# saifahmadgit/go2-sim2real-locomotion-rl

Hardware: AMD Instinct MI355X
Metric: env-steps/sec (all envs) Go2 walk 4096 envs; 1/2/4/8-GPU scaling (higher is better)
Workload: dtype f32

## Files before the change

### go2_sim2real_locomotion_rl_amd/csrc/go2sim.hip

```cpp

#include <hip/hip_runtime.h>

#include <algorithm>
#include <cstddef>
#include <cstdint>
#include <cstdio>
#include <cstdlib>
#include <cstring>
#include <new>
#include <vector>

#include "../../include/go2sim.h"
#include "../../include/go2sim_detmath.h"

#define DEV __device__ __forceinline__
#define DEVN __device__ __noinline__

namespace {

constexpr int NL = GO2SIM_NL, ND = GO2SIM_ND, NQ = GO2SIM_NQ, NG = GO2SIM_NG, NJ = GO2SIM_NJ;
constexpr int NPAIR = GO2SIM_NPAIR_MAX, MAXC = GO2SIM_MAX_CONTACTS, MAXB = GO2SIM_MAX_BROAD, MAXR = GO2SIM_MAX_ROWS;
constexpr int JOINT_FIXED = 0, JOINT_REVOLUTE = 1, JOINT_FREE = 4;
constexpr int GEOM_PLANE = 0, GEOM_SPHERE = 1, GEOM_CYLINDER = 3, GEOM_BOX = 5, GEOM_TERRAIN = 7;
constexpr int TERRAIN_CB = 4;
// ... 303 lines not shown
      depth[i] = (par < 0) ? 0 : depth[par] + 1;
      if (depth[i] > max_depth) max_depth = depth[i];
    }
    m.n_levels = max_depth + 1;
    int k = 0;
    for (int lev = 0; lev <= max_depth; ++lev) {
      m.level_start[lev] = k;
      for (int i = 0; i < NL; ++i) if (depth[i] == lev) m.level_links[k++] = i;
    }
    for (int lev = max_depth + 1; lev <= NL; ++lev) m.level_start[lev] = k;
    k = 0;
    for (int par = 0; par < NL; ++par) {
      m.child_start[par] = k;
      for (int i = NL - 1; i > par; --i) if (m.links[i].parent == par) m.child_list[k++] = i;
    }
    m.child_start[NL] = k;
    for (int d = 0; d < ND; ++d) m.dof_link[d] = -1;
    for (int i = 0; i < NL; ++i) for (int d = m.links[i].dof_start; d < m.links[i].dof_end; ++d) m.dof_link[d] = i;
    for (int d = 0; d < ND; ++d) if (m.dof_link[d] < 0) return false;
  }
  int g_next = 0;
  for (int i = 0; i < NL; ++i) { if (m.links[i].geom_start != g_next) return false; g_next = m.links[i].geom_end; }
  return g_next == NG;
}


struct LinkS {
  int parent, entity, is_fixed, joint_start, joint_end, dof_start, dof_end, q_start, q_end, n_dofs;
  V3 pos; Q4 quat; V3 inertial_pos; Q4 inertial_quat; M3 inertial_i; float mass; float invweight[2];
};
struct GeomS { int type, link; V3 pos; Q4 quat; };
struct JLim { int q_start, dof_start; float lo, hi; };
constexpr int NTRI = ND * (ND + 1) / 2;
constexpr int LEG_K = 4, LEG_D = 3;
struct alignas(16) ModelS {
  int n_levels, iterations, ls_iterations, arrow_mode;
  float substep_dt; V3 gravity; float eps, tolerance, ls_tolerance, meaninertia;
  LinkS links[NL];
  unsigned char tri_i[NTRI + 1], tri_j[NTRI + 1];
  JLim jlim[NJ];
  Joint joints[NJ]; Dof dofs[ND]; GeomS geoms[NG]; Entity entities[2];
  float qpos0[NQ]; unsigned mass_mask_bits[ND];
  int level_start[NL + 1], level_links[NL], child_start[NL + 1], child_list[NL], dof_link[ND];
  unsigned char leg_links[LEG_K * LEG_D], leg_root, leg_form;
};
constexpr int SOLVER_BLOCK_BYTES = (int)(sizeof(LinkS) * NL + 2 * (NTRI + 1) + sizeof(JLim) * NJ);
static_assert(sizeof(ModelS) % 16 == 0 && (2 * (NTRI + 1)) % 4 == 0 && offsetof(ModelS, links) % 16 == 0 && offsetof(ModelS, jlim) == offsetof(ModelS, links) + sizeof(LinkS) * NL + 2 * (NTRI + 1), "ModelS is copied in 16-byte granules");

static bool build_leg_form(const Model& m, ModelS& o) {
  if (getenv("GO2SIM_NO_LEG_FORM") && atoi(getenv("GO2SIM_NO_LEG_FORM")) != 0) return false;
  if (NL > 255) return false;
  auto n_children = [&](int i) { return m.child_start[i + 1] - m.child_start[i]; };
  auto one_revolute = [&](const Link& L) {
    if (L.joint_end - L.joint_start != 1) return false;
    const Joint& J = m.joints[L.joint_start];
    return J.type == JOINT_REVOLUTE && J.dof_end - J.dof_start == 1 && L.dof_start == J.dof_start && L.dof_end == J.dof_end &&
           L.q_end - L.q_start == 1 && J.q_start == L.q_start;
  };
  int root = -1, n_links = 0;
  for (int i = 0; i < NL; ++i) {
    const Link& L = m.links[i];
    if (L.parent != -1) continue;
    const bool free_root = !L.is_fixed && L.joint_end - L.joint_start == 1 && m.joints[L.joint_start].type == JOINT_FREE && L.n_dofs == 6;
    if (free_root) {
      if (root >= 0) return false;
      root = i;
    } else if (!(L.is_fixed && L.joint_end == L.joint_start && L.n_dofs == 0 && n_children(i) == 0)) {
      return false;
    } else {
      n_links++;
    }
  }
  if (root < 0 || n_children(root) != LEG_K) return false;
  n_links++;
  for (int l = 0; l < LEG_K; ++l) {
    int i = m.child_list[m.child_start[root] + l];
    for (int d = 0; d < LEG_D; ++d) {
      if (!one_revolute(m.links[i]) || n_children(i) != (d + 1 < LEG_D ? 1 : 0)) return false;
      o.leg_links[LEG_D * l + d] = (unsigned char)i;
      n_links++;
      if (d + 1 < LEG_D) i = m.child_list[m.child_start[i]];
    }
  }
  if (n_links != NL) return false;
  o.leg_root = (unsigned char)root;
  return true;
}
bool build_model_s(const Model& m, ModelS& o) {
  memset(&o, 0, sizeof(o));
  o.n_levels = m.n_levels; o.iterations = m.iterations; o.ls_iterations = m.ls_iterations; o.arrow_mode = m.arrow_mode;
  o.substep_dt = m.substep_dt; o.gravity = m.gravity; o.eps = m.eps; o.tolerance = m.tolerance; o.ls_tolerance = m.ls_tolerance; o.meaninertia = m.meaninertia;
  for (int i = 0; i < NL; ++i) {
    const Link& a = m.links[i]; LinkS& b = o.links[i];
    b.parent = a.parent; b.entity = a.entity; b.is_fixed = a.is_fixed; b.joint_start = a.joint_start; b.joint_end = a.joint_end; b.dof_start = a.dof_start;
    b.dof_end = a.dof_end; b.q_start = a.q_start; b.q_end = a.q_end; b.n_dofs = a.n_dofs; b.pos = a.pos; b.quat = a.quat; b.inertial_pos = a.inertial_pos;
    b.inertial_quat = a.inertial_quat; b.inertial_i = a.inertial_i; b.mass = a.mass; b.invweight[0] = a.invweight[0]; b.invweight[1] = a.invweight[1];
  }
  for (int i = 0; i < NJ; ++i) o.joints[i] = m.joints[i];
  for (int i = 0; i < ND; ++i) o.dofs[i] = m.dofs[i];
  for (int i = 0; i < NG; ++i) { o.geoms[i].type = m.geoms[i].type; o.geoms[i].link = m.geoms[i].link; o.geoms[i].pos = m.geoms[i].pos; o.geoms[i].quat = m.geoms[i].quat; }
  for (int i = 0; i < 2; ++i) o.entities[i] = m.entities[i];
  for (int i = 0; i < NQ; ++i) o.qpos0[i] = m.qpos0[i];
  for (int i = 0; i < ND; ++i) {
    unsigned bits = 0;
    for (int j = 0; j < ND; ++j) {
      float v = m.mass_parent_mask[i][j];
      if (v == 1.0f) bits |= 1u << j; else if (v != 0.0f) return false;
    }
    o.mass_mask_bits[i] = bits;
  }
  for (int i = 0; i <= NL; ++i) { o.level_start[i] = m.level_start[i]; o.child_start[i] = m.child_start[i]; }
  for (int i = 0; i < NL; ++i) { o.level_links[i] = m.level_links[i]; o.child_list[i] = m.child_list[i]; }
  for (int i = 0; i < ND; ++i) o.dof_link[i] = m.dof_link[i];
  int k = 0;
  for (int i = 0; i < ND; ++i) for (int j = 0; j <= i; ++j) { o.tri_i[k] = (unsigned char)i; o.tri_j[k] = (unsigned char)j; k++; }
  for (int i = 0; i < NJ; ++i) {
    const Joint& J = m.joints[i];
    bool rev = J.type == JOINT_REVOLUTE;
    o.jlim[i].q_start = rev ? J.q_start : -1; o.jlim[i].dof_start = J.dof_start;
    o.jlim[i].lo = rev ? m.dofs[J.dof_start].limit[0] : 0.0f; o.jlim[i].hi = rev ? m.dofs[J.dof_start].limit[1] : 0.0f;
  }
  o.leg_form = build_leg_form(m, o) ? 1 : 0;
  return true;
}
DEV float mass_mask(const ModelS& m, int i, int j) { return (float)((m.mass_mask_bits[i] >> j) & 1u); }
DEV void tri_index(const ModelS& m, int idx, int& i, int& j) { i = m.tri_i[idx]; j = m.tri_j[idx]; }

struct ModelView {
  int n_levels, iterations, ls_iterations, arrow_mode, leg_form; float substep_dt; V3 gravity; float eps, tolerance, ls_tolerance, meaninertia;
  const LinkS* links; const Joint* joints; const Dof* dofs; const GeomS* geoms; const Entity* entities; const float* qpos0;
  const unsigned* mass_mask_bits; const int *level_start, *level_links, *child_start, *child_list, *dof_link; const unsigned char *tri_i, *tri_j;
  const unsigned char* leg_links; int leg_root;
  DEV ModelView(const ModelS* t, const ModelS* __restrict__ g)
      : n_levels(g->n_levels), iterations(g->iterations), ls_iterations(g->ls_iterations), arrow_mode(g->arrow_mode), leg_form(g->leg_form), substep_dt(g->substep_dt), gravity(g->gravity), eps(g->eps),
        tolerance(g->tolerance), ls_tolerance(g->ls_tolerance), meaninertia(g->meaninertia), links(t->links), joints(t->joints), dofs(t->dofs),
        geoms(t->geoms), entities(t->entities), qpos0(t->qpos0), mass_mask_bits(t->mass_mask_bits), level_start(t->level_start),
        level_links(t->level_links), child_start(t->child_start), child_list(t->child_list), dof_link(t->dof_link), tri_i(t->tri_i), tri_j(t->tri_j),
        leg_links(t->leg_links), leg_root(g->leg_root) {}
  DEV ModelView(const LinkS* lds_links, const unsigned char* lds_tri_i, const unsigned char* lds_tri_j, const Model* __restrict__ g)
      : n_levels(g->n_levels), iterations(g->iterations), ls_iterations(g->ls_iterations), arrow_mode(g->arrow_mode), leg_form(0), substep_dt(g->substep_dt), gravity(g->gravity), eps(g->eps),
        tolerance(g->tolerance), ls_tolerance(g->ls_tolerance), meaninertia(g->meaninertia), links(lds_links), joints(g->joints), dofs(g->dofs),
        geoms(nullptr), entities(g->entities), qpos0(g->qpos0), mass_mask_bits(nullptr), level_start(nullptr), level_links(nullptr), child_start(nullptr),
        child_list(nullptr), dof_link(nullptr), tri_i(lds_tri_i), tri_j(lds_tri_j), leg_links(nullptr), leg_root(-1) {}
};
DEV float mass_mask(const ModelView& m, int i, int j) { return (float)((m.mass_mask_bits[i] >> j) & 1u); }
DEV void tri_index(const ModelView& m, int idx, int& i, int& j) { i = m.tri_i[idx]; j = m.tri_j[idx]; }
constexpr int lds_dma_bytes(int nbytes) { return (nbytes + 1023) / 1024 * 1024; }
template <int NBYTES>
DEV void wg_dma_to_lds(void* lds_dst, const void* __restrict__ src, int lane = (int)threadIdx.x) {
#pragma unroll
  for (int k = 0; k < lds_dma_bytes(NBYTES) / 1024; ++k)
    __builtin_amdgcn_global_load_lds((const __attribute__((address_space(1))) void*)((const char*)src + (k * 64 + lane) * 16),
                                     (__attribute__((address_space(3))) void*)((char*)lds_dst + k * 1024), 16, 0, 0);
}
constexpr int MODELS_LDS_BYTES = lds_dma_bytes((int)sizeof(ModelS));
constexpr int GEOMK_BYTES = NG * (int)sizeof(GeomK), GEOMK_LDS_BYTES = lds_dma_bytes(GEOMK_BYTES);

#define GO2SIM_FLOAT_FIELDS(X)                                                                                       \
  X(qpos, NQ) X(vel, ND) X(ctrl_force, ND) X(ext, NL * 6) X(mass_shift, NL) X(com_shift, NL * 3)                        \
  X(friction_ratio, NG) X(l_pos, NL * 3) X(l_quat, NL * 4) X(cd_vel, NL * 3) X(cd_ang, NL * 3) X(root_com, NL * 3)     \
  X(contact_force, NL * 3) X(geom_friction, NG) X(ctrl_pos, ND) X(ctrl_vel, ND) X(dof_pos, ND) \
                                                                                       \
  X(actions, NA) X(last_actions, NA) X(applied_actions, NA) X(action_history, GO2SIM_ACTION_RING_MAX * NA) X(target_dof_pos, NM)            \
  X(e_dof_pos, NM) X(e_dof_vel, NM) X(last_dof_vel, NM) X(torque, NM) X(base_pos, 3) X(base_quat, 4) X(base_lin_vel, 3) \
  X(base_ang_vel, 3) X(projected_gravity, 3) X(base_euler, 3) X(commands, 3) X(time_out, 1) X(kp_factors, NM)          \
  X(kd_factors, NM) X(motor_strength, NM) X(gravity_offset, 3) X(current_push_force, 3) X(push_stored_force, 3)       \
  X(feet_air_time, 4) X(base_vel_world, 3) X(last_base_pos_x, 1) X(episode_sums, NREW) X(rew_terms, NREW) X(rew, 1) X(obs, NOBS_MAX) X(priv, NPRIV_MAX) \
  X(base_kp, 1) X(base_kd, 1)

#define GO2SIM_INT_FIELDS(X)                                                                                         \
  X(n_contacts, 1) X(n_con, 1) X(err, 1) X(is_warmstart, 1) X(first_time, 1) X(n_broad, 1) X(solver_iters, 1) X(ctrl_mode, ND) \
  X(gjk_fallback, 1) X(delay_steps, 1) X(episode_length, 1) X(reset_buf, 1) X(push_remaining, 1) X(foot_contact, 4)    \
  X(last_foot_contact, 4) X(terrain_row, 1) X(terrain_key, 1)

#define GO2SIM_AOS_FLOAT_FIELDS(X)                                                                                   \
  X(acc, ND) X(qacc_ws, ND) X(force, ND) X(qf_smooth, ND) X(acc_smooth, ND) X(qfrc_constraint, ND) X(mass_mat, NTRI)  \
  X(cdof_ang, ND * 3) X(cdof_vel, ND * 3) X(cdofd_ang, ND * 3) X(cdofd_vel, ND * 3) X(cinr_inertial, NL * 9)            \
  X(cinr_pos, NL * 3) X(cinr_mass, NL) X(i_pos, NL * 3) X(i_quat, NL * 4) X(g_pos, NG * 3) X(g_quat, NG * 4)              \
  X(sort_value, 2 * NG) X(c_pos, MAXC * 3) X(c_normal, MAXC * 3) X(c_pen, MAXC) X(c_friction, MAXC) X(c_sol, MAXC * 7)    \
  X(c_force, MAXC * 3) X(efc_force, MAXR) X(normal_cache, NPAIR * 3)

constexpr int NCV = (NPAIR + 31) / 32;
#define GO2SIM_AOS_INT_FIELDS(X) X(sort_ig, 2 * NG) X(broad, MAXB * 2) X(c_geom, 2 * MAXC) X(c_link, 2 * MAXC) X(ncache_valid, NCV)

enum FOff : int {
#define X(n, c) FO_##n##_, FO_##n##_end = FO_##n##_ + (c) - 1,
  GO2SIM_FLOAT_FIELDS(X)
#undef X
  FO_TOTAL
};
enum IOff : int {
#define X(n, c) IO_##n##_, IO_##n##_end = IO_##n##_ + (c) - 1,
  GO2SIM_INT_FIELDS(X)
#undef X
  IO_TOTAL
};
enum AOff : int {
#define X(n, c) AO_##n##_, AO_##n##_end = AO_##n##_ + (c) - 1,
  GO2SIM_AOS_FLOAT_FIELDS(X)
#undef X
  AO_TOTAL
};
enum AIOff : int {
#define X(n, c) AIO_##n##_, AIO_##n##_end = AIO_##n##_ + (c) - 1,
  GO2SIM_AOS_INT_FIELDS(X)
#undef X
  AIO_TOTAL
};
#define FO(n) FO_##n##_
#define IO(n) IO_##n##_
#define AO(n) AO_##n##_
#define AIO(n) AIO_##n##_
constexpr int ASTRIDE = (AO_TOTAL + 15) / 16 * 16;
constexpr int AISTRIDE = (AIO_TOTAL + 15) / 16 * 16;

template <typename T>
struct Arr {
  T* p; int B;
  DEV T& operator[](int i) const { return p[(size_t)i * B]; }
};
struct V3Ref {
  float* p; int B;
  DEV operator V3() const { return v3(p[0], p[B], p[2 * (size_t)B]); }
  DEV const V3Ref& operator=(V3 v) const { p[0] = v.x; p[B] = v.y; p[2 * (size_t)B] = v.z; return *this; }
  DEV const V3Ref& operator=(const V3Ref& o) const { V3 v = o; return *this = v; }
};
struct Q4Ref {
  float* p; int B;
  DEV operator Q4() const { return q4(p[0], p[B], p[2 * (size_t)B], p[3 * (size_t)B]); }
  DEV const Q4Ref& operator=(Q4 q) const { p[0] = q.w; p[B] = q.x; p[2 * (size_t)B] = q.y; p[3 * (size_t)B] = q.z; return *this; }
  DEV const Q4Ref& operator=(const Q4Ref& o) const { Q4 v = o; return *this = v; }
};
struct M3Ref {
  float* p; int B;
  DEV operator M3() const { M3 r;
#pragma unroll
    for (int i = 0; i < 9; ++i) r.m[i / 3][i % 3] = p[(size_t)i * B];
    return r; }
  DEV const M3Ref& operator=(const M3& r) const {
#pragma unroll
    for (int i = 0; i < 9; ++i) p[(size_t)i * B] = r.m[i / 3][i % 3];
    return *this; }
  DEV const M3Ref& operator=(const M3Ref& o) const { M3 v = o; return *this = v; }
};
struct Arr3 { float* p; int B; DEV V3Ref operator[](int i) const { return V3Ref{p + (size_t)(3 * i) * B, B}; } };
struct Arr4 { float* p; int B; DEV Q4Ref operator[](int i) const { return Q4Ref{p + (size_t)(4 * i) * B, B}; } };
struct Arr9 { float* p; int B; DEV M3Ref operator[](int i) const { return M3Ref{p + (size_t)(9 * i) * B, B}; } };
template <int W>
struct Arr2 {
  float* p; int B;
  DEV Arr<float> operator[](int i) const { return Arr<float>{p + (size_t)(W * i) * B, B}; }
};

struct Pool { float* f; int* i; int B; float* fa; int* ia; };

struct E {
  float* f; int* i; int B; int b; float* fa; int* ia;
  DEV E(const Pool& P, int b_) : f(P.f + b_), i(P.i + b_), B(P.B), b(b_), fa(P.fa + (size_t)b_ * ASTRIDE), ia(P.ia + (size_t)b_ * AISTRIDE) {}
#define FA(name) DEV Arr<float> name() const { return Arr<float>{f + (size_t)FO(name) * B, B}; }
#define FA3(name) DEV Arr3 name() const { return Arr3{f + (size_t)FO(name) * B, B}; }
#define FA4(name) DEV Arr4 name() const { return Arr4{f + (size_t)FO(name) * B, B}; }
#define FA2(name, W) DEV Arr2<W> name() const { return Arr2<W>{f + (size_t)FO(name) * B, B}; }
#define IA(name) DEV Arr<int> name() const { return Arr<int>{i + (size_t)IO(name) * B, B}; }
#define AA(name) DEV Arr<float> name() const { return Arr<float>{fa + AO(name), 1}; }
#define AA3(name) DEV Arr3 name() const { return Arr3{fa + AO(name), 1}; }
#define AA4(name) DEV Arr4 name() const { return Arr4{fa + AO(name), 1}; }
#define AA9(name) DEV Arr9 name() const { return Arr9{fa + AO(name), 1}; }
#define AA2(name, W) DEV Arr2<W> name() const { return Arr2<W>{fa + AO(name), 1}; }
#define AIA(name) DEV Arr<int> name() const { return Arr<int>{ia + AIO(name), 1}; }
  FA(qpos) FA(vel) FA(ctrl_force) FA(ctrl_pos) FA(ctrl_vel) FA(ext) FA(mass_shift) FA3(com_shift) FA(friction_ratio)
  FA(geom_friction) FA3(l_pos) FA4(l_quat) FA3(root_com) FA(dof_pos) FA3(cd_vel) FA3(cd_ang) FA3(contact_force)
  FA(actions) FA(last_actions) FA(applied_actions) FA2(action_history, NA) FA(target_dof_pos) FA(e_dof_pos) FA(e_dof_vel) FA(last_dof_vel)
  FA(torque) FA(base_pos) FA(base_quat) FA(base_lin_vel) FA(base_ang_vel) FA(projected_gravity) FA(base_euler) FA(commands) FA(time_out)
  FA(kp_factors) FA(kd_factors) FA(motor_strength) FA(gravity_offset) FA(current_push_force) FA(push_stored_force) FA(feet_air_time) FA(base_vel_world) FA(last_base_pos_x)
  FA(episode_sums) FA(rew_terms) FA(rew) FA(obs) FA(priv) FA(base_kp) FA(base_kd)
  IA(n_contacts) IA(n_con) IA(err) IA(is_warmstart) IA(first_time) IA(n_broad) IA(solver_iters) IA(ctrl_mode)
  IA(gjk_fallback) IA(delay_steps) IA(episode_length) IA(reset_buf) IA(push_remaining) IA(foot_contact) IA(last_foot_contact) IA(terrain_row) IA(terrain_key)
  AA(acc) AA(qacc_ws) AA(force) AA(qf_smooth) AA(acc_smooth) AA(qfrc_constraint) AA3(cdof_ang) AA3(cdof_vel) AA3(cdofd_ang)
  AA3(cdofd_vel) AA9(cinr_inertial) AA3(cinr_pos) AA(cinr_mass) AA3(i_pos) AA4(i_quat) AA3(g_pos) AA4(g_quat) AA(sort_value) AA3(c_pos) AA3(c_normal)
  AA(c_pen) AA(c_friction) AA2(c_sol, 7) AA3(c_force) AA(efc_force) AA3(normal_cache)
  AIA(sort_ig) AIA(broad) AIA(c_geom) AIA(c_link) AIA(ncache_valid)
#undef FA
#undef FA3
#undef FA4
#undef FA2
#undef IA
#undef AA
#undef AA3
#undef AA4
#undef AA9
#undef AA2
#undef AIA
};
DEV void team_sync() {
  __builtin_amdgcn_fence(__ATOMIC_RELEASE, "workgroup");
  __builtin_amdgcn_wave_barrier();
  __builtin_amdgcn_fence(__ATOMIC_ACQUIRE, "workgroup");
}
DEV void team_sync_lds() {
  __builtin_amdgcn_fence(__ATOMIC_RELEASE, "workgroup", "local");
  __builtin_amdgcn_wave_barrier();
  __builtin_amdgcn_fence(__ATOMIC_ACQUIRE, "workgroup", "local");
}
DEV float gload(const E& e, int off, int k) { return e.f[(size_t)(off + k) * e.B]; }
DEV void gstore(const E& e, int off, int k, float v) { e.f[(size_t)(off + k) * e.B] = v; }
DEV float aload(const E& e, int off, int k) { return e.fa[off + k]; }
DEV void astore(const E& e, int off, int k, float v) { e.fa[off + k] = v; }


template <int N, int T, class F>
DEV void team_for(int tl, F f) {
#pragma unroll
  for (int k0 = 0; k0 < N; k0 += T) { int k = k0 + tl; if (k < N) f(k); }
}
template <int N, int STRIDE, int R, class FL, class FS>
DEV void team_stage_r(int k0, FL& ld, FS& st) {
  if constexpr (R * STRIDE < N) {
    int k = R * STRIDE + k0;
    k = k < N ? k : N - 1;
    const float v = ld(k);
    team_stage_r<N, STRIDE, R + 1>(k0, ld, st);
    st(k, v);
  }
}
template <int N, int T, class FL, class FS>
DEV void team_stage(int tl, FL ld, FS st) { team_stage_r<N, T, 0>(tl, ld, st); }
template <int EPW, int COUNT, class F>
DEV void wg_load(const Pool& P, int b0, int off, F put) {
  const int ev = threadIdx.x % EPW, k0 = threadIdx.x / EPW;
  const int b = (b0 + ev < P.B) ? b0 + ev : P.B - 1;
  auto ld = [&](int k) { return P.f[(size_t)(off + k) * P.B + b]; };
  auto st = [&](int k, float v) { put(ev, k, v); };
  team_stage_r<COUNT, 64 / EPW, 0>(k0, ld, st);
}

#ifdef GO2SIM_PHASE_PROFILE
constexpr int PH_MAX_WG = 8192;
__device__ unsigned long long g_phase_cycles[PH_MAX_WG * 64];
#define PH_BEGIN unsigned long long ph_t = __builtin_readcyclecounter();
#define PH(i) { __builtin_amdgcn_s_waitcnt(0); unsigned long long ph_n = __builtin_readcyclecounter(); if (threadIdx.x == 0 && blockIdx.x < PH_MAX_WG / 2) g_phase_cycles[blockIdx.x * 64 + (i)] += ph_n - ph_t; ph_t = __builtin_readcyclecounter(); }
#define PHD_BEGIN unsigned long long phd_t = __builtin_readcyclecounter();
#define PHD(i) { unsigned long long phd_n = __builtin_readcyclecounter(); const unsigned long long phd_a = __ballot(1); if ((int)threadIdx.x == __ffsll((long long)phd_a) - 1 && blockIdx.x < PH_MAX_WG / 2) { atomicAdd(&g_phase_cycles[blockIdx.x * 64 + (i)], phd_n - phd_t); atomicAdd(&g_phase_cycles[blockIdx.x * 64 + (i) + 1], 1ull); } phd_t = __builtin_readcyclecounter(); }
#define PHC(i, n) { if (threadIdx.x == 0 && blockIdx.x < PH_MAX_WG / 2) g_phase_cycles[blockIdx.x * 64 + (i)] += (unsigned long long)(n); }
#define PHB(i) { __builtin_amdgcn_s_waitcnt(0); unsigned long long ph_n = __builtin_readcyclecounter(); if (threadIdx.x == 0 && blockIdx.x < PH_MAX_WG / 2) g_phase_cycles[(PH_MAX_WG / 2 + blockIdx.x) * 64 + (i)] += ph_n - ph_t; ph_t = __builtin_readcyclecounter(); }
#else
#define PH_BEGIN
#define PH(i)
#define PHD_BEGIN
#define PHD(i)
#define PHC(i, n)
#define PHB(i)
#endif

#ifdef GO2SIM_STAMP
constexpr int ST_KINDS = 8, ST_MAX_WG = 4096, ST_DEPTH = 4;
__device__ unsigned long long g_stamp[ST_KINDS * ST_MAX_WG * ST_DEPTH * 2];
__device__ unsigned g_stamp_cnt[ST_KINDS * ST_MAX_WG];
struct StampScope {
  int kind; unsigned long long t0;
  DEV StampScope(int k) : kind(k) { t0 = __builtin_amdgcn_s_memrealtime(); }
  DEV ~StampScope() {
    __builtin_amdgcn_s_waitcnt(0);
    const unsigned long long t1 = __builtin_amdgcn_s_memrealtime();
    if (threadIdx.x == 0 && blockIdx.x < ST_MAX_WG) {
      const int w = kind * ST_MAX_WG + (int)blockIdx.x;
      const unsigned c = g_stamp_cnt[w];
      g_stamp[(w * ST_DEPTH + (int)(c % ST_DEPTH)) * 2] = t0; g_stamp[(w * ST_DEPTH + (int)(c % ST_DEPTH)) * 2 + 1] = t1;
      g_stamp_cnt[w] = c + 1;
    }
  }
};
#define STAMP(kind) StampScope stamp_scope_(kind);
#else
#define STAMP(kind)
#endif
enum { STK_PRE_DYN = 0, STK_COLLIDE, STK_SOLVE, STK_INT_FK_DYN, STK_INT_FK, STK_POST_A, STK_POST_B, STK_OTHER };

enum { SV_COST = 0, SV_PREV_COST, SV_GAUSS, SV_QG0, SV_QG1, SV_QG2, SV_GTOL };
enum { SI_LS_IT = 0, SI_LS_RESULT, SI_IMPROVED };

DEV V3 ld3(const float* p, int i) { return v3(p[3 * i], p[3 * i + 1], p[3 * i + 2]); }
DEV void st3(float* p, int i, V3 v) { p[3 * i] = v.x; p[3 * i + 1] = v.y; p[3 * i + 2] = v.z; }
DEV Q4 ld4(const float* p, int i) { return q4(p[4 * i], p[4 * i + 1], p[4 * i + 2], p[4 * i + 3]); }
DEV void st4(float* p, int i, Q4 q) { p[4 * i] = q.w; p[4 * i + 1] = q.x; p[4 * i + 2] = q.y; p[4 * i + 3] = q.z; }
DEV M3 ld9(const float* p, int i) { M3 r;
#pragma unroll
  for (int k = 0; k < 9; ++k) r.m[k / 3][k % 3] = p[9 * i + k];
  return r; }
DEV void st9(float* p, int i, const M3& r) {
#pragma unroll
  for (int k = 0; k < 9; ++k) p[9 * i + k] = r.m[k / 3][k % 3]; }

DEV int xcd_block() {
  const int n = (int)gridDim.x, q = n >> 3, r = n & 7, x = (int)blockIdx.x & 7, i = (int)blockIdx.x >> 3;
  return (x < r ? x * (q + 1) : r * (q + 1) + (x - r) * q) + i;
}

constexpr int LPT_CLS = 32;
DEV int lpt_solver_xcd(int b, int B, int epw_s) {
  const int n = (B + epw_s - 1) / epw_s, q = n >> 3, r = n & 7, L = b / epw_s;
  if (L < r * (q + 1)) return L / (q + 1);
  return r + (L - r * (q + 1)) / (q > 0 ? q : 1);
}
DEV void lpt_file(int* __restrict__ rec, int cap, int L, int B, int epw_s, int nc) {
  const int x = lpt_solver_xcd(L * epw_s, B, epw_s), cls = LPT_CLS - 1 - imn(LPT_CLS - 1, nc);
  const int pos = atomicAdd(&rec[x * LPT_CLS + cls], 1);
  if (pos < cap) rec[8 * LPT_CLS + (x * LPT_CLS + cls) * cap + pos] = L;
}
DEV int lpt_take(const int* __restrict__ rec, int cap, int B, int epw, int slot) {
  const int ident = xcd_block() * epw + slot;
  if (rec == nullptr) return ident;
  const int n = (int)gridDim.x, q = n >> 3, r = n & 7, x = (int)blockIdx.x & 7;
  const int expected = q + (x < r ? 1 : 0);
  const int local = (int)blockIdx.x >> 3;
  int total = 0, cls = -1, off = 0;
#pragma unroll
  for (int c = 0; c < LPT_CLS; ++c) {
    const int k = rec[x * LPT_CLS + c];
    if (cls < 0 && local < total + k) { cls = c; off = local - total; }
    total += k;
  }
  if (total != expected) return ident;
  if (cls < 0 || off >= cap) return B;
  return rec[8 * LPT_CLS + (x * LPT_CLS + cls) * cap + off] * epw + slot;
}

struct KinData {
  float qpos[NQ], vel[ND], qpos_next[NQ], vel_next[ND];
  float l_pos[NL * 3], l_quat[NL * 4], i_pos[NL * 3], i_quat[NL * 4];
  float xanchor[NJ * 3], xaxis[NJ * 3];
  float cdof_ang[ND * 3], cdof_vel[ND * 3];
  float cd_vel[NL * 3], cd_ang[NL * 3];
  float mass[NL];
  int valid;
};

#ifndef GO2SIM_FAST_ORDER
#define GO2SIM_FAST_ORDER 1
#endif
template <int CTRL>
DEV float dpp_perm(float x) { return __int_as_float(__builtin_amdgcn_update_dpp(0, __float_as_int(x), CTRL, 0xf, 0xf, true)); }
#if GO2SIM_FAST_ORDER
constexpr bool ARROW_SHAPE = (ND == 18);
DEV float leg_sum4(float x) {
  const auto r = __builtin_amdgcn_permlane16_swap(__float_as_uint(x), __float_as_uint(x), false, false);
  const float p = __uint_as_float(r[0]) + __uint_as_float(r[1]);
  return p + dpp_perm<0x128>(p);
}
DEV float4 lds4(const float* p) { return *(const float4*)p; }
template <int T, int STRIDE>
DEV void arrow_factor(const int mode, const float eps, const float* A, float* F, int tl) {
  static_assert(T == 32 || T == 64, "four groups of eight lanes");
  const int leg = (tl >> 3) & 3, u = tl & 7, ub = u < 6 ? u : 5;
  const int p0 = dm_arrow_dof(mode, leg, 0), p1 = dm_arrow_dof(mode, leg, 1), p2 = dm_arrow_dof(mode, leg, 2);
  const bool w_lane = tl < 32 && u < 6;
  const float a00 = A[p0 * STRIDE + p0], a10 = A[p1 * STRIDE + p0], a11 = A[p1 * STRIDE + p1];
  const float a20 = A[p2 * STRIDE + p0], a21 = A[p2 * STRIDE + p1], a22 = A[p2 * STRIDE + p2];
  const float c0 = A[p0 * STRIDE + ub], c1 = A[p1 * STRIDE + ub], c2 = A[p2 * STRIDE + ub];
  float br[6];
#pragma unroll
  for (int j = 0; j < 6; ++j) br[j] = A[ub * STRIDE + j];
  team_sync();
  const float e0 = fmx(a00, eps), i0 = dm_sqrt(e0) * (1.0f / e0);
  const float l10 = a10 * i0, l20 = a20 * i0;
  const float e1 = fmx(__builtin_fmaf(-l10, l10, a11), eps), i1 = dm_sqrt(e1) * (1.0f / e1);
  const float l21 = __builtin_fmaf(-l20, l10, a21) * i1;
  const float e2 = fmx(__builtin_fmaf(-l21, l21, __builtin_fmaf(-l20, l20, a22)), eps), i2 = dm_sqrt(e2) * (1.0f / e2);
  const float w0 = c0 * i0, w1 = __builtin_fmaf(-w0, l10, c1) * i1, w2 = __builtin_fmaf(-w1, l21, __builtin_fmaf(-w0, l20, c2)) * i2;
  if (w_lane) *(float4*)&F[32 * leg + 8 + 4 * u] = make_float4(w0, w1, w2, 0.0f);
  if (tl < 32 && u == 0) { *(float4*)&F[32 * leg] = make_float4(i0, i1, i2, 0.0f); *(float4*)&F[32 * leg + 4] = make_float4(l10, l20, l21, 0.0f); }
  team_sync();
  float sc[6];
#pragma unroll
  for (int j = 0; j < 6; ++j) {
    const float4 wj = lds4(&F[32 * leg + 8 + 4 * j]);
    sc[j] = __builtin_fmaf(w2, wj.z, __builtin_fmaf(w1, wj.y, w0 * wj.x));
  }
#pragma unroll
  for (int j = 0; j < 6; ++j) sc[j] = leg_sum4(sc[j]);
  const float bp[6] = {br[0] - sc[0], br[1] - sc[1], br[2] - sc[2], br[3] - sc[3], br[4] - sc[4], br[5] - sc[5]};
  if (tl < 6) { *(float4*)&F[128 + 8 * tl] = make_float4(bp[0], bp[1], bp[2], bp[3]); *(float4*)&F[128 + 8 * tl + 4] = make_float4(bp[4], bp[5], 0.0f, 0.0f); }
  team_sync();
  float a[6][6];
#pragma unroll
  for (int k = 0; k < 6; ++k) {
    const float4 lo = lds4(&F[128 + 8 * k]); const float2 hi = *(const float2*)&F[128 + 8 * k + 4];
    a[k][0] = lo.x; a[k][1] = lo.y; a[k][2] = lo.z; a[k][3] = lo.w; a[k][4] = hi.x; a[k][5] = hi.y;
  }
  team_sync();
#pragma unroll
  for (int k = 0; k < 6; ++k) {
    const float e = fmx(a[k][k], eps), ik = dm_sqrt(e) * (1.0f / e);
    a[k][k] = ik;
#pragma unroll
    for (int j = k + 1; j < 6; ++j) a[j][k] = a[j][k] * ik;
#pragma unroll
    for (int j = k + 1; j < 6; ++j)
#pragma unroll
      for (int i = k + 1; i <= j; ++i) a[j][i] = __builtin_fmaf(-a[j][k], a[i][k], a[j][i]);
  }
  if (tl == 0) {
#pragma unroll
    for (int k = 0; k < 6; ++k) {
      *(float4*)&F[128 + 8 * k] = make_float4(a[k][0], k >= 1 ? a[k][1] : 0.0f, k >= 2 ? a[k][2] : 0.0f, k >= 3 ? a[k][3] : 0.0f);
      *(float2*)&F[128 + 8 * k + 4] = make_float2(k >= 4 ? a[k][4] : 0.0f, k >= 5 ? a[k][5] : 0.0f);
    }
  }
  team_sync();
}
template <int T>
DEV void arrow_solve(const float* F, float gl0, float gl1, float gl2, float gb, float* x6, int tl, float (&xb)[6], float& xl0, float& xl1, float& xl2) {
  static_assert(T == 32 || T == 64, "four groups of eight lanes");
  const int leg = (tl >> 3) & 3, u = tl & 7, ub = u < 6 ? u : 5;
  const float4 iv = lds4(&F[32 * leg]), lv = lds4(&F[32 * leg + 4]), wo = lds4(&F[32 * leg + 8 + 4 * ub]);
  float4 W[6];
#pragma unroll
  for (int b = 0; b < 6; ++b) W[b] = lds4(&F[32 * leg + 8 + 4 * b]);
  float L[6][6];
#pragma unroll
  for (int k = 0; k < 6; ++k) {
    const float4 lo = lds4(&F[128 + 8 * k]); const float2 hi = *(const float2*)&F[128 + 8 * k + 4];
    L[k][0] = lo.x; L[k][1] = lo.y; L[k][2] = lo.z; L[k][3] = lo.w; L[k][4] = hi.x; L[k][5] = hi.y;
  }
  const float y0 = gl0 * iv.x, y1 = __builtin_fmaf(-lv.x, y0, gl1) * iv.y, y2 = __builtin_fmaf(-lv.z, y1, __builtin_fmaf(-lv.y, y0, gl2)) * iv.z;
  const float z = leg_sum4(__builtin_fmaf(wo.z, y2, __builtin_fmaf(wo.y, y1, wo.x * y0)));
  if (tl < 6) x6[tl] = gb - z;
  team_sync();
  const float2 r0 = *(const float2*)&x6[0], r1 = *(const float2*)&x6[2], r2 = *(const float2*)&x6[4];
  float x[6] = {r0.x, r0.y, r1.x, r1.y, r2.x, r2.y};
  team_sync();
#pragma unroll
  for (int k = 0; k < 6; ++k) {
    float acc = x[k];
#pragma unroll
    for (int j = 0; j < k; ++j) acc = __builtin_fmaf(-L[k][j], x[j], acc);
    x[k] = acc * L[k][k];
  }
#pragma unroll
  for (int k_ = 0; k_ < 6; ++k_) {
    const int k = 5 - k_;
    float acc = x[k];
#pragma unroll
    for (int j_ = 0; j_ < 5 - k; ++j_) { const int j = 5 - j_; acc = __builtin_fmaf(-L[j][k], x[j], acc); }
    x[k] = acc * L[k][k];
  }
  float v0 = y0, v1 = y1, v2 = y2;
#pragma unroll
  for (int b = 0; b < 6; ++b) { v0 = __builtin_fmaf(-W[b].x, x[b], v0); v1 = __builtin_fmaf(-W[b].y, x[b], v1); v2 = __builtin_fmaf(-W[b].z, x[b], v2); }
  xl2 = v2 * iv.z; xl1 = __builtin_fmaf(-lv.z, xl2, v1) * iv.y; xl0 = __builtin_fmaf(-lv.x, xl1, __builtin_fmaf(-lv.y, xl2, v0)) * iv.x;
#pragma unroll
  for (int k = 0; k < 6; ++k) xb[k] = x[k];
}
#endif
struct DynData {
  float cinr_I[NL * 9], cinr_pos[NL * 3], cinr_mass[NL];
  float crb_I[NL * 9], crb_pos[NL * 3], crb_mass[NL];
  float cdof_ang[ND * 3], cdof_vel[ND * 3], cdofd_ang[ND * 3], cdofd_vel[ND * 3];
  float cd_vel[NL * 3], cd_ang[NL * 3], cdd_vel[NL * 3], cdd_ang[NL * 3], cfrc_vel[NL * 3], cfrc_ang[NL * 3];
  float f_ang[ND * 3], f_vel[ND * 3];
  float vel[ND], qf_applied[ND], qf_passive[ND], force[ND], out[ND], Dinv[ND];
  float M[ND * ND], L[ND * ND];
  int ctrl_mode[ND];
};
#if GO2SIM_FAST_ORDER
static_assert(!ARROW_SHAPE || (offsetof(DynData, Dinv) % 8 == 0 && sizeof(DynData) % 8 == 0), "arrow_solve reads DynData::Dinv with 8-byte LDS loads");
#endif

template <int T>
DEV void tk_stage_links(const E& e, KinData* s, int tl) {
  team_for<NL, T>(tl, [&](int i_l) { st3(s->l_pos, i_l, e.l_pos()[i_l]); st4(s->l_quat, i_l, e.l_quat()[i_l]); });
}
template <int T, class MT>
DEV void tk_kinematics(const MT& m, const E& e, KinData* s, int tl, bool force_update_fixed, DynData* dk = nullptr) {
  PH_BEGIN
  const bool legs = (T == 32 || T == 64) && m.leg_form;
  if (legs) {
    const int r = m.leg_root;
    const int rq = m.joints[m.links[r].joint_start].q_start;
    const V3 rpos = v3(s->qpos[rq], s->qpos[rq + 1], s->qpos[rq + 2]);
    Q4 rquat = q4(s->qpos[rq + 3], s->qpos[rq + 4], s->qpos[rq + 5], s->qpos[rq + 6]);
    const float rn = dm_sqrt(norm_sqr(rquat));
    rquat = q4(rquat.w / rn, rquat.x / rn, rquat.y / rn, rquat.z / rn);
    if (tl == 0) {
      const auto& L = m.links[r];
      const int i_j = L.joint_start, ds = m.joints[i_j].dof_start;
      st3(s->xanchor, i_j, rpos);
      st3(s->xaxis, i_j, v3(0, 0, 1));
      gstore(e, FO(dof_pos), ds + 0, rpos.x); gstore(e, FO(dof_pos), ds + 1, rpos.y); gstore(e, FO(dof_pos), ds + 2, rpos.z);
      if (dk) { dk->out[ds] = rpos.x; dk->out[ds + 1] = rpos.y; dk->out[ds + 2] = rpos.z; }
      st3(s->l_pos, r, rpos); st4(s->l_quat, r, rquat); e.l_pos()[r] = rpos; e.l_quat()[r] = rquat;
    }
    Q4 ql = q4(0, 0, 0, 0);
    if (tl < LEG_K * LEG_D) {
      const Joint& J = m.joints[m.links[m.leg_links[tl]].joint_start];
      const float dp = s->qpos[J.q_start] - m.qpos0[J.q_start];
      gstore(e, FO(dof_pos), J.dof_start, dp);
      if (dk) dk->out[J.dof_start] = dp;
      ql = rotvec_to_quat(m.dofs[J.dof_start].motion_ang * dp, m.eps);
    }
    Q4 qloc[LEG_D];
#pragma unroll
    for (int d = 0; d < LEG_D; ++d) {
      const int src = tl < LEG_K ? LEG_D * tl + d : 0;
      qloc[d] = q4(__shfl(ql.w, src, T), __shfl(ql.x, src, T), __shfl(ql.y, src, T), __shfl(ql.z, src, T));
    }
    if (tl < LEG_K) {
      int lk[LEG_D], jk[LEG_D];
      V3 lpos[LEG_D], jpos[LEG_D], axis[LEG_D]; Q4 lquat[LEG_D];
#pragma unroll
      for (int d = 0; d < LEG_D; ++d) {
        lk[d] = m.leg_links[LEG_D * tl + d];
        const auto& L = m.links[lk[d]];
        jk[d] = L.joint_start;
        const Joint& J = m.joints[jk[d]];
        lpos[d] = L.pos; lquat[d] = L.quat; jpos[d] = J.pos; axis[d] = m.dofs[J.dof_start].motion_ang;
      }
      V3 pos = rpos; Q4 quat = rquat;
#pragma unroll
      for (int d = 0; d < LEG_D; ++d) {
        const Q4 pq = quat;
        pos = pos + transform_by_quat(lpos[d], pq);
        quat = transform_quat_by_quat(lquat[d], pq);
        const V3 anchor = transform_by_quat(jpos[d], quat) + pos;
        st3(s->xanchor, jk[d], anchor);
        st3(s->xaxis, jk[d], transform_by_quat(axis[d], quat));
        quat = transform_quat_by_quat(qloc[d], quat);
        pos = anchor - transform_by_quat(jpos[d], quat);
        st3(s->l_pos, lk[d], pos); st4(s->l_quat, lk[d], quat); e.l_pos()[lk[d]] = pos; e.l_quat()[lk[d]] = quat;
      }
    }
    team_sync();
  }
  for (int lev = 0; lev < (legs ? 0 : m.n_levels); ++lev) {
    for (int k = m.level_start[lev] + tl; k < m.level_start[lev + 1]; k += T) {
      int i_l = m.level_links[k];
      const auto& L = m.links[i_l];
      V3 pos = L.pos; Q4 quat = L.quat;
      if (L.parent != -1) {
        Q4 pq = ld4(s->l_quat, L.parent);
        pos = ld3(s->l_pos, L.parent) + transform_by_quat(L.pos, pq);
        quat = transform_quat_by_quat(L.quat, pq);
      }
      for (int i_j = L.joint_start; i_j < L.joint_end; ++i_j) {
        const Joint& J = m.joints[i_j];
        int q_start = J.q_start, dof_start = J.dof_start;
        if (J.type == JOINT_FREE) {
          V3 pos_ = v3(s->qpos[q_start], s->qpos[q_start + 1], s->qpos[q_start + 2]);
          st3(s->xanchor, i_j, pos_);
          st3(s->xaxis, i_j, v3(0, 0, 1));
          Q4 quat_ = q4(s->qpos[q_start + 3], s->qpos[q_start + 4], s->qpos[q_start + 5], s->qpos[q_start + 6]);
          float n = dm_sqrt(norm_sqr(quat_));
          quat_ = q4(quat_.w / n, quat_.x / n, quat_.y / n, quat_.z / n);
          pos = pos_; quat = quat_;
          gstore(e, FO(dof_pos), dof_start + 0, pos.x); gstore(e, FO(dof_pos), dof_start + 1, pos.y); gstore(e, FO(dof_pos), dof_start + 2, pos.z);
          if (dk) { dk->out[dof_start] = pos.x; dk->out[dof_start + 1] = pos.y; dk->out[dof_start + 2] = pos.z; }
        } else if (J.type == JOINT_REVOLUTE) {
          V3 axis = m.dofs[dof_start].motion_ang;
          V3 anchor = transform_by_quat(J.pos, quat) + pos;
          st3(s->xanchor, i_j, anchor);
          st3(s->xaxis, i_j, transform_by_quat(axis, quat));
          float dp = s->qpos[q_start] - m.qpos0[q_start];
          gstore(e, FO(dof_pos), dof_start, dp);
          if (dk) dk->out[dof_start] = dp;
          Q4 qloc = rotvec_to_quat(axis * dp, m.eps);
          quat = transform_quat_by_quat(qloc, quat);
          pos = anchor - transform_by_quat(J.pos, quat);
        }
      }
      if (!(L.parent == -1 && L.is_fixed)) { st3(s->l_pos, i_l, pos); st4(s->l_quat, i_l, quat); e.l_pos()[i_l] = pos; e.l_quat()[i_l] = quat; }
    }
    team_sync();
  }
  PH(18)
  for (int i_l = tl; i_l < NL; i_l += T) {
    const auto& L = m.links[i_l];
    s->mass[i_l] = L.mass + gload(e, FO(mass_shift), i_l);
    V3 ipbw; Q4 iq;
    transform_pos_quat_by_trans_quat(L.inertial_pos + (V3)e.com_shift()[i_l], L.inertial_quat, ld3(s->l_pos, i_l), ld4(s->l_quat, i_l), ipbw, iq);
    st3(s->i_pos, i_l, ipbw); st4(s->i_quat, i_l, iq);
  }
  team_sync();
  V3 rc[2];
#pragma unroll
  for (int i_e = 0; i_e < 2; ++i_e) {
    const Entity& en = m.entities[i_e];
    V3 root_com_bw = v3(0, 0, 0); float mass_sum = 0.0f;
    for (int i_l = en.link_start; i_l < en.link_end; ++i_l) {
      float mass = s->mass[i_l];
      mass_sum = mass_sum + mass;
      root_com_bw = root_com_bw + mass * ld3(s->i_pos, i_l);
    }
    rc[i_e] = root_com_bw / mass_sum;
  }
  team_sync();
  for (int i_l = tl; i_l < NL; i_l += T) {
    const auto& L = m.links[i_l];
    V3 r = (L.entity == 0) ? rc[0] : rc[1];
    e.root_com()[i_l] = r;
    V3 ip = ld3(s->i_pos, i_l) - r;
    Q4 iq = ld4(s->i_quat, i_l);
    if (!dk) e.i_pos()[i_l] = ip;
    e.i_quat()[i_l] = iq;
    float i_mass = s->mass[i_l];
    M3 oI; V3 op;
    transform_inertia_by_trans_quat(L.inertial_i, i_mass, ip, iq, m.eps, oI, op);
    if (!dk) { e.cinr_inertial()[i_l] = oI; e.cinr_pos()[i_l] = op; e.cinr_mass()[i_l] = i_mass; }
    if (dk) { st9(dk->cinr_I, i_l, oI); st9(dk->crb_I, i_l, oI); st3(dk->cinr_pos, i_l, op); st3(dk->crb_pos, i_l, op); dk->cinr_mass[i_l] = i_mass; dk->crb_mass[i_l] = i_mass; }
  }
  for (int i_j = tl; i_j < NJ; i_j += T) {
    const Joint& J = m.joints[i_j];
    const auto& L = m.links[J.link];
    if (L.n_dofs == 0) continue;
    V3 r = (L.entity == 0) ? rc[0] : rc[1];
    V3 offset_pos = r - ld3(s->xanchor, i_j);
    int ds = J.dof_start;
    if (J.type == JOINT_REVOLUTE) {
      V3 ax = ld3(s->xaxis, i_j);
      V3 cv = cross(ax, offset_pos);
      st3(s->cdof_ang, ds, ax); st3(s->cdof_vel, ds, cv);
      e.cdof_ang()[ds] = ax; e.cdof_vel()[ds] = cv;
      if (dk) { st3(dk->cdof_ang, ds, ax); st3(dk->cdof_vel, ds, cv); }
    } else if (J.type == JOINT_FREE) {
      for (int i = 0; i < 3; ++i) {
        V3 cv = v3(0, 0, 0);
        vset(cv, i, 1.0f);
        st3(s->cdof_ang, i + ds, v3(0, 0, 0)); st3(s->cdof_vel, i + ds, cv);
        e.cdof_ang()[i + ds] = v3(0, 0, 0); e.cdof_vel()[i + ds] = cv;
        if (dk) { st3(dk->cdof_ang, i + ds, v3(0, 0, 0)); st3(dk->cdof_vel, i + ds, cv); }
      }
      M3 xmat_T = transpose(quat_to_R(ld4(s->l_quat, J.link), m.eps));
#pragma unroll
      for (int i = 0; i < 3; ++i) {
        V3 row = v3(xmat_T.m[i][0], xmat_T.m[i][1], xmat_T.m[i][2]);
        V3 cv = cross(row, offset_pos);
        st3(s->cdof_ang, i + ds + 3, row); st3(s->cdof_vel, i + ds + 3, cv);
        e.cdof_ang()[i + ds + 3] = row; e.cdof_vel()[i + ds + 3] = cv;
        if (dk) { st3(dk->cdof_ang, i + ds + 3, row); st3(dk->cdof_vel, i + ds + 3, cv); }
      }
    }
  }
  for (int i_g = tl; i_g < NG; i_g += T) {
    const auto& G = m.geoms[i_g];
    bool is_fixed = m.links[G.link].is_fixed;
    if (force_update_fixed || !is_fixed) {
      V3 p; Q4 q;
      transform_pos_quat_by_trans_quat(G.pos, G.quat, ld3(s->l_pos, G.link), ld4(s->l_quat, G.link), p, q);
      e.g_pos()[i_g] = p; e.g_quat()[i_g] = q;
    }
  }
  team_sync();
  PH(19)
  if (legs) {
    const int r = m.leg_root, ds = m.links[r].dof_start;
    float v[6]; V3 ca[6], cv[6];
#pragma unroll
    for (int i = 0; i < 6; ++i) { v[i] = s->vel[ds + i]; ca[i] = ld3(s->cdof_ang, ds + i); cv[i] = ld3(s->cdof_vel, ds + i); }
    V3 cvel_vel = v3(0, 0, 0), cvel_ang = v3(0, 0, 0);
#pragma unroll
    for (int i = 0; i < 3; ++i) { cvel_vel = cvel_vel + cv[i] * v[i]; cvel_ang = cvel_ang + ca[i] * v[i]; }
    if (tl == 0) {
#pragma unroll
      for (int i = 0; i < 3; ++i) {
        if (!dk) { e.cdofd_ang()[ds + i] = v3(0, 0, 0); e.cdofd_vel()[ds + i] = v3(0, 0, 0); }
        if (dk) { st3(dk->cdofd_ang, ds + i, v3(0, 0, 0)); st3(dk->cdofd_vel, ds + i, v3(0, 0, 0)); }
        V3 oa, ov;
        motion_cross_motion(cvel_ang, cvel_vel, ca[i + 3], cv[i + 3], oa, ov);
        if (!dk) { e.cdofd_ang()[ds + i + 3] = oa; e.cdofd_vel()[ds + i + 3] = ov; }
        if (dk) { st3(dk->cdofd_ang, ds + i + 3, oa); st3(dk->cdofd_vel, ds + i + 3, ov); }
      }
    }
#pragma unroll
    for (int i = 0; i < 3; ++i) { cvel_vel = cvel_vel + cv[i + 3] * v[i + 3]; cvel_ang = cvel_ang + ca[i + 3] * v[i + 3]; }
    if (tl == 0) {
      st3(s->cd_vel, r, cvel_vel); st3(s->cd_ang, r, cvel_ang);
      if (!dk) { e.cd_vel()[r] = cvel_vel; e.cd_ang()[r] = cvel_ang; }
      if (dk) { st3(dk->cd_vel, r, cvel_vel); st3(dk->cd_ang, r, cvel_ang); }
    }
    for (int i_l = tl; i_l < NL; i_l += T) {
      if (m.links[i_l].parent != -1 || i_l == r) continue;
      st3(s->cd_vel, i_l, v3(0, 0, 0)); st3(s->cd_ang, i_l, v3(0, 0, 0));
      if (!dk) { e.cd_vel()[i_l] = v3(0, 0, 0); e.cd_ang()[i_l] = v3(0, 0, 0); }
      if (dk) { st3(dk->cd_vel, i_l, v3(0, 0, 0)); st3(dk->cd_ang, i_l, v3(0, 0, 0)); }
    }
    if (tl < LEG_K) {
      int lk[LEG_D], dd[LEG_D]; float lv[LEG_D]; V3 la[LEG_D], lc[LEG_D];
#pragma unroll
      for (int d = 0; d < LEG_D; ++d) {
        lk[d] = m.leg_links[LEG_D * tl + d];
        dd[d] = m.links[lk[d]].dof_start;
        lv[d] = s->vel[dd[d]]; la[d] = ld3(s->cdof_ang, dd[d]); lc[d] = ld3(s->cdof_vel, dd[d]);
      }
#pragma unroll
      for (int d = 0; d < LEG_D; ++d) {
        V3 oa, ov;
        motion_cross_motion(cvel_ang, cvel_vel, la[d], lc[d], oa, ov);
        if (!dk) { e.cdofd_ang()[dd[d]] = oa; e.cdofd_vel()[dd[d]] = ov; }
        if (dk) { st3(dk->cdofd_ang, dd[d], oa); st3(dk->cdofd_vel, dd[d], ov); }
        cvel_vel = cvel_vel + lc[d] * lv[d];
        cvel_ang = cvel_ang + la[d] * lv[d];
        st3(s->cd_vel, lk[d], cvel_vel); st3(s->cd_ang, lk[d], cvel_ang);
        if (!dk) { e.cd_vel()[lk[d]] = cvel_vel; e.cd_ang()[lk[d]] = cvel_ang; }
        if (dk) { st3(dk->cd_vel, lk[d], cvel_vel); st3(dk->cd_ang, lk[d], cvel_ang); }
      }
    }
    team_sync();
  }
  for (int lev = 0; lev < (legs ? 0 : m.n_levels); ++lev) {
    for (int k = m.level_start[lev] + tl; k < m.level_start[lev + 1]; k += T) {
      int i_l = m.level_links[k];
      const auto& L = m.links[i_l];
      V3 cvel_vel = v3(0, 0, 0), cvel_ang = v3(0, 0, 0);
      if (L.parent != -1) { cvel_vel = ld3(s->cd_vel, L.parent); cvel_ang = ld3(s->cd_ang, L.parent); }
      for (int i_j = L.joint_start; i_j < L.joint_end; ++i_j) {
        const Joint& J = m.joints[i_j];
        int ds = J.dof_start;
        if (J.type == JOINT_FREE) {
          for (int i = 0; i < 3; ++i) {
            float v = s->vel[ds + i];
            cvel_vel = cvel_vel + ld3(s->cdof_vel, ds + i) * v;
            cvel_ang = cvel_ang + ld3(s->cdof_ang, ds + i) * v;
          }
          for (int i = 0; i < 3; ++i) {
            if (!dk) { e.cdofd_ang()[ds + i] = v3(0, 0, 0); e.cdofd_vel()[ds + i] = v3(0, 0, 0); }
            if (dk) { st3(dk->cdofd_ang, ds + i, v3(0, 0, 0)); st3(dk->cdofd_vel, ds + i, v3(0, 0, 0)); }
            V3 oa, ov;
            motion_cross_motion(cvel_ang, cvel_vel, ld3(s->cdof_ang, ds + i + 3), ld3(s->cdof_vel, ds + i + 3), oa, ov);
            if (!dk) { e.cdofd_ang()[ds + i + 3] = oa; e.cdofd_vel()[ds + i + 3] = ov; }
            if (dk) { st3(dk->cdofd_ang, ds + i + 3, oa); st3(dk->cdofd_vel, ds + i + 3, ov); }
          }
          for (int i = 0; i < 3; ++i) {
            float v = s->vel[ds + i + 3];
            cvel_vel = cvel_vel + ld3(s->cdof_vel, ds + i + 3) * v;
            cvel_ang = cvel_ang + ld3(s->cdof_ang, ds + i + 3) * v;
          }
        } else {
          for (int i_d = ds; i_d < J.dof_end; ++i_d) {
            V3 oa, ov;
            motion_cross_motion(cvel_ang, cvel_vel, ld3(s->cdof_ang, i_d), ld3(s->cdof_vel, i_d), oa, ov);
            if (!dk) { e.cdofd_ang()[i_d] = oa; e.cdofd_vel()[i_d] = ov; }
            if (dk) { st3(dk->cdofd_ang, i_d, oa); st3(dk->cdofd_vel, i_d, ov); }
          }
          for (int i_d = ds; i_d < J.dof_end; ++i_d) {
            float v = s->vel[i_d];
            cvel_vel = cvel_vel + ld3(s->cdof_vel, i_d) * v;
            cvel_ang = cvel_ang + ld3(s->cdof_ang, i_d) * v;
          }
        }
      }
      st3(s->cd_vel, i_l, cvel_vel); st3(s->cd_ang, i_l, cvel_ang);
      if (!dk) { e.cd_vel()[i_l] = cvel_vel; e.cd_ang()[i_l] = cvel_ang; }
      if (dk) { st3(dk->cd_vel, i_l, cvel_vel); st3(dk->cd_ang, i_l, cvel_ang); }
    }
    team_sync();
  }
  PH(55)
}

template <int T, class MT>
DEV void tk_integrate(const MT& m, const E& e, KinData* s, int tl) {
  for (int i_l = tl; i_l < NL; i_l += T) {
    const auto& L = m.links[i_l];
    if (L.n_dofs == 0) continue;
    int ds = L.dof_start, qs = L.q_start;
    int joint_type = m.joints[L.joint_start].type;
    if (joint_type == JOINT_FREE) {
      V3 pos = v3(s->qpos[qs], s->qpos[qs + 1], s->qpos[qs + 2]);
      V3 v = v3(s->vel_next[ds], s->vel_next[ds + 1], s->vel_next[ds + 2]);
      pos = pos + v * m.substep_dt;
      s->qpos_next[qs] = pos.x; s->qpos_next[qs + 1] = pos.y; s->qpos_next[qs + 2] = pos.z;
      Q4 rot0 = q4(s->qpos[qs + 3], s->qpos[qs + 4], s->qpos[qs + 5], s->qpos[qs + 6]);
      V3 ang = v3(s->vel_next[ds + 3], s->vel_next[ds + 4], s->vel_next[ds + 5]) * m.substep_dt;
      Q4 qrot = rotvec_to_quat(ang, m.eps);
      Q4 rot = transform_quat_by_quat(qrot, rot0);
      s->qpos_next[qs + 3] = rot.w; s->qpos_next[qs + 4] = rot.x; s->qpos_next[qs + 5] = rot.y; s->qpos_next[qs + 6] = rot.z;
    } else {
      for (int j_ = 0; j_ < L.q_end - qs; ++j_) s->qpos_next[qs + j_] = s->qpos[qs + j_] + s->vel_next[ds + j_] * m.substep_dt;
    }
  }
  team_sync();
  bool bad = false;
  for (int d = tl; d < ND; d += T) bad |= isnan_(s->vel_next[d]);
  for (int q = tl; q < NQ; q += T) bad |= isnan_(s->qpos_next[q]);
  if (bad) s->valid = 0;
  team_sync();
  if (s->valid) {
    for (int d = tl; d < ND; d += T) { float v = s->vel_next[d]; s->vel[d] = v; gstore(e, FO(vel), d, v); }
    for (int q = tl; q < NQ; q += T) { float v = s->qpos_next[q]; s->qpos[q] = v; gstore(e, FO(qpos), q, v); }
  } else if (tl == 0) {
    atomicOr(&e.err()[0], GO2SIM_ERR_INVALID_ACC_NAN);
  }
  team_sync();
}

template <int T>
DEV void integrate_fk_body(const Pool& P, const ModelS* __restrict__ mp, int b, KinData* lds, char* ms_raw, bool pre, float pre_vel, float pre_acc) {
  const ModelS& ms = *(const ModelS*)ms_raw;
  wg_dma_to_lds<(int)sizeof(ModelS)>(ms_raw, mp);
  const int tl = threadIdx.x % T, slot = threadIdx.x / T;
  const ModelView m(&ms, mp);
  E e(P, b < P.B ? b : P.B - 1);
  KinData* s = &lds[slot];
  PH_BEGIN
  if (pre) { if (tl < ND) { s->vel[tl] = pre_vel; s->vel_next[tl] = pre_acc; } }
  else {
    team_stage<ND, T>(tl, [&](int d) { return gload(e, FO(vel), d); }, [&](int d, float v) { s->vel[d] = v; });
    team_stage<ND, T>(tl, [&](int d) { return aload(e, AO(acc), d); }, [&](int d, float a) { s->vel_next[d] = a; });
  }
  team_stage<NQ, T>(tl, [&](int q) { return gload(e, FO(qpos), q); }, [&](int q, float v) { s->qpos[q] = v; });
  team_for<ND, T>(tl, [&](int d) { s->vel_next[d] = s->vel[d] + s->vel_next[d] * m.substep_dt; });
  if (tl == 0) s->valid = 1;
  tk_stage_links<T>(e, s, tl);
  team_sync();
  if (b >= P.B) return;
  tk_integrate<T>(m, e, s, tl);
  PH(40)
  tk_kinematics<T>(m, e, s, tl, false);
  PH(41)
}
template <int T>
__global__ __launch_bounds__(64) void k_integrate_fk_team(Pool P, const ModelS* __restrict__ mp) {
  STAMP(STK_INT_FK)
  constexpr int EPW = 64 / T;
  __shared__ KinData lds[EPW];
  __shared__ alignas(16) char ms_raw[MODELS_LDS_BYTES];
  integrate_fk_body<T>(P, mp, xcd_block() * EPW + (int)threadIdx.x / T, lds, ms_raw, false, 0.0f, 0.0f);
}

template <int T>
__global__ __launch_bounds__(64) void k_fk_team(Pool P, const ModelS* __restrict__ mp, int force_update_fixed, const int* __restrict__ cond) {
  constexpr int EPW = 64 / T;
  __shared__ KinData lds[EPW];
  __shared__ alignas(16) char ms_raw[MODELS_LDS_BYTES];
  const ModelS& ms = *(const ModelS*)ms_raw;
  if (cond && *cond <= 0) return;
  wg_dma_to_lds<(int)sizeof(ModelS)>(ms_raw, mp);
  const int tl = threadIdx.x % T, slot = threadIdx.x / T;
  const int b = xcd_block() * EPW + slot;
  const ModelView m(&ms, mp);
  E e(P, b < P.B ? b : P.B - 1);
  KinData* s = &lds[slot];
  team_stage<ND, T>(tl, [&](int d) { return gload(e, FO(vel), d); }, [&](int d, float v) { s->vel[d] = v; });
  team_stage<NQ, T>(tl, [&](int q) { return gload(e, FO(qpos), q); }, [&](int q, float v) { s->qpos[q] = v; });
  tk_stage_links<T>(e, s, tl);
  team_sync();
  if (b >= P.B) return;
  tk_kinematics<T>(m, e, s, tl, force_update_fixed != 0);
}

template <int T, class MT>
DEV void tk_dynamics(const MT& m, const E& e, DynData* s, int tl, bool env_valid) {
  PH_BEGIN
  const bool legs = (T == 32 || T == 64) && m.leg_form;
  if (legs) {
    for (int c = tl; c < 13; c += T) {
      auto at = [&](int i_l) -> float* { return (c < 9) ? &s->crb_I[9 * i_l + c] : ((c < 12) ? &s->crb_pos[3 * i_l + c - 9] : &s->crb_mass[i_l]); };
      const int r = m.leg_root;
      float x[LEG_K][LEG_D];
#pragma unroll
      for (int l = 0; l < LEG_K; ++l)
#pragma unroll
        for (int d = 0; d < LEG_D; ++d) x[l][d] = *at(m.leg_links[LEG_D * l + d]);
      float a = *at(r);
#pragma unroll
      for (int l = 0; l < LEG_K; ++l) {
#pragma unroll
        for (int d = LEG_D - 2; d >= 0; --d) { x[l][d] = x[l][d] + x[l][d + 1]; *at(m.leg_links[LEG_D * l + d]) = x[l][d]; }
      }
#pragma unroll
      for (int l = 0; l < LEG_K; ++l) a = a + x[l][0];
      *at(r) = a;
    }
    team_sync();
  }
  for (int lev = (legs ? -1 : m.n_levels - 2); lev >= 0; --lev) {
    int n_par = m.level_start[lev + 1] - m.level_start[lev];
    for (int w = tl; w < n_par * 13; w += T) {
      int i_p = m.level_links[m.level_start[lev] + w / 13], comp = w % 13;
      float* dst = (comp < 9) ? &s->crb_I[9 * i_p + comp] : ((comp < 12) ? &s->crb_pos[3 * i_p + comp - 9] : &s->crb_mass[i_p]);
      float a = *dst;
      for (int c = m.child_start[i_p]; c < m.child_start[i_p + 1]; ++c) {
        int i_l = m.child_list[c];
        float v = (comp < 9) ? s->crb_I[9 * i_l + comp] : ((comp < 12) ? s->crb_pos[3 * i_l + comp - 9] : s->crb_mass[i_l]);
        a = a + v;
      }
      *dst = a;
    }
    team_sync();
  }
  PH(21)
  for (int i_d = tl; i_d < ND; i_d += T) {
    int i_l = m.dof_link[i_d];
    V3 oa, ov;
    inertial_mul(ld3(s->crb_pos, i_l), ld9(s->crb_I, i_l), s->crb_mass[i_l], ld3(s->cdof_vel, i_d), ld3(s->cdof_ang, i_d), oa, ov);
    st3(s->f_ang, i_d, oa); st3(s->f_vel, i_d, ov);
  }
  team_sync();
  for (int idx = tl; idx < ND * (ND + 1) / 2; idx += T) {
    int i_d, j_d;
    tri_index(m, idx, i_d, j_d);
    float v = (dot(ld3(s->f_ang, i_d), ld3(s->cdof_ang, j_d)) + dot(ld3(s->f_vel, i_d), ld3(s->cdof_vel, j_d))) * mass_mask(m, i_d, j_d);
    if (i_d == j_d) {
      v = v + m.dofs[i_d].armature;
      v = v + m.dofs[i_d].damping * m.substep_dt;
      int cm = s->ctrl_mode[i_d];
      if (cm == CTRL_POSITION || cm == CTRL_VELOCITY) v = v + m.dofs[i_d].kv * m.substep_dt;
    }
    s->M[i_d * ND + j_d] = v; s->M[j_d * ND + i_d] = v;
    s->L[i_d * ND + j_d] = v;
  }
  team_sync();
  PH(22)
#if GO2SIM_FAST_ORDER
  const bool arrow = ARROW_SHAPE && (T == 32 || T == 64) && m.arrow_mode != 0;
  float* const AF = (float*)(((uintptr_t)s->L + 15) & ~(uintptr_t)15);
#else
  const bool arrow = false;
#endif
  if constexpr (T == 32 || T == 64) {
#if GO2SIM_FAST_ORDER
    if (arrow) arrow_factor<T, ND>(m.arrow_mode, m.eps, s->M, AF, tl);
#endif
  }
  if (arrow) {
  } else if constexpr (T >= ND) {
    const int row = tl < ND ? tl : ND - 1;
    float Lr[ND];
#pragma unroll
    for (int k = 0; k < ND; ++k) Lr[k] = s->L[row * ND + k];
    float dinv_own = 0.0f;
#pragma unroll
    for (int i_d_ = 0; i_d_ < ND; ++i_d_) {
      const int i_d = ND - i_d_ - 1;
      if (i_d_ > 0) {
        if (tl == i_d) {
#pragma unroll
          for (int k = 0; k <= i_d; ++k) s->L[i_d * ND + k] = Lr[k];
        }
        team_sync();
      }
      float ri[ND];
#pragma unroll
      for (int k = 0; k <= i_d; ++k) ri[k] = s->L[i_d * ND + k];
      const float lij = s->L[i_d * ND + (row < i_d ? row : 0)];
      const float D_inv = 1.0f / ri[i_d];
      if (row == i_d) dinv_own = D_inv;
      const bool act = row < i_d;
      const float a = lij * D_inv;
#pragma unroll
      for (int k = 0; k < i_d; ++k) { const float nv = Lr[k] - a * ri[k]; Lr[k] = act ? nv : Lr[k]; }
    }
    team_sync();
    if (tl < ND) {
#pragma unroll
      for (int k = 0; k < ND; ++k) if (k < row) s->L[row * ND + k] = Lr[k] * dinv_own;
      s->L[row * ND + row] = 1.0f;
      s->Dinv[row] = dinv_own;
    }
    team_sync();
  } else {
#pragma unroll
    for (int i_d_ = 0; i_d_ < ND; ++i_d_) {
      const int i_d = ND - i_d_ - 1;
      float D_inv = 1.0f / s->L[i_d * ND + i_d];
      for (int idx = tl; idx < i_d * (i_d + 1) / 2; idx += T) {
        int j_d, k_d;
        tri_index(m, idx, j_d, k_d);
        float a = s->L[i_d * ND + j_d] * D_inv;
        s->L[j_d * ND + k_d] -= a * s->L[i_d * ND + k_d];
      }
      team_sync();
      for (int j_d = tl; j_d < i_d; j_d += T) s->L[i_d * ND + j_d] = s->L[i_d * ND + j_d] * D_inv;
      if (tl == 0) { s->Dinv[i_d] = D_inv; s->L[i_d * ND + i_d] = 1.0f; }
      team_sync();
    }
  }
  PH(23)
  for (int i_d = tl; i_d < ND; i_d += T) {
    const Dof& D = m.dofs[i_d];
    const auto& L = m.links[m.dof_link[i_d]];
    int joint_type = m.joints[L.joint_start].type;
    float force = 0.0f;
    int cm = s->ctrl_mode[i_d];
    const float in_ctrl_force = s->qf_applied[i_d], in_ctrl_pos = s->qf_passive[i_d], in_ctrl_vel = s->force[i_d], in_dof_pos = s->out[i_d];
    if (cm == CTRL_FORCE) force = in_ctrl_force;
    else if (cm == CTRL_VELOCITY) force = D.kv * (in_ctrl_vel - s->vel[i_d]);
    else if (cm == CTRL_POSITION && !(joint_type == JOINT_FREE && i_d >= L.dof_start + 3))
      force = D.kp * (in_ctrl_pos - in_dof_pos) + D.kv * (in_ctrl_vel - s->vel[i_d]);
    s->qf_applied[i_d] = clampf(force, D.force_range[0], D.force_range[1]);
    float qp = -D.damping * s->vel[i_d];
    if (joint_type != JOINT_FREE && joint_type != JOINT_FIXED) qp = qp + (-in_dof_pos * D.stiffness);
    s->qf_passive[i_d] = qp;
  }
  if (legs) {
    const int r = m.leg_root;
    if (tl < 6 * LEG_K) {
      const int l = tl / 6, c = tl % 6;
      const float* src = (c < 3) ? s->cdofd_vel : s->cdofd_ang;
      const int cc = (c < 3) ? c : c - 3;
      const V3 g0 = -m.gravity * (1.0f - 0.0f);
      const int ds = m.links[r].dof_start;
      float vr[6], xr[6], vl[LEG_D], xl[LEG_D]; int lk[LEG_D];
#pragma unroll
      for (int i = 0; i < 6; ++i) { vr[i] = s->vel[ds + i]; xr[i] = src[3 * (ds + i) + cc]; }
#pragma unroll
      for (int d = 0; d < LEG_D; ++d) {
        lk[d] = m.leg_links[LEG_D * l + d];
        const int i_d = m.links[lk[d]].dof_start;
        vl[d] = s->vel[i_d]; xl[d] = src[3 * i_d + cc];
      }
      float* dst = (c < 3) ? s->cdd_vel : s->cdd_ang;
      float a = (c < 3) ? ((cc == 0) ? g0.x : ((cc == 1) ? g0.y : g0.z)) : 0.0f;
#pragma unroll
      for (int i = 0; i < 6; ++i) a = a + xr[i] * vr[i];
      if (l == 0) dst[3 * r + cc] = a;
#pragma unroll
      for (int d = 0; d < LEG_D; ++d) { a = a + xl[d] * vl[d]; dst[3 * lk[d] + cc] = a; }
    }
    for (int i_l = tl; i_l < NL; i_l += T) {
      if (m.links[i_l].parent != -1 || i_l == r) continue;
      st3(s->cdd_vel, i_l, -m.gravity * (1.0f - 0.0f)); st3(s->cdd_ang, i_l, v3(0, 0, 0));
    }
    team_sync();
  }
  for (int lev = 0; lev < (legs ? 0 : m.n_levels); ++lev) {
    for (int k = m.level_start[lev] + tl; k < m.level_start[lev + 1]; k += T) {
      int i_l = m.level_links[k];
      const auto& L = m.links[i_l];
      V3 cv, ca;
      if (L.parent == -1) { cv = -m.gravity * (1.0f - 0.0f); ca = v3(0, 0, 0); }
      else { cv = ld3(s->cdd_vel, L.parent); ca = ld3(s->cdd_ang, L.parent); }
      for (int i_d = L.dof_start; i_d < L.dof_end; ++i_d) {
        float v = s->vel[i_d];
        V3 local_cdd_vel = ld3(s->cdofd_vel, i_d) * v;
        V3 local_cdd_ang = ld3(s->cdofd_ang, i_d) * v;
        cv = cv + local_cdd_vel;
        ca = ca + local_cdd_ang;
      }
      st3(s->cdd_vel, i_l, cv); st3(s->cdd_ang, i_l, ca);
    }
    team_sync();
  }
  for (int i_l = tl; i_l < NL; i_l += T) {
    V3 f1_ang, f1_vel, f2_ang, f2_vel, f3_ang, f3_vel;
    M3 I = ld9(s->cinr_I, i_l); V3 cp = ld3(s->cinr_pos, i_l); float cm = s->cinr_mass[i_l];
    V3 cdv = ld3(s->cd_vel, i_l), cda = ld3(s->cd_ang, i_l);
    inertial_mul(cp, I, cm, ld3(s->cdd_vel, i_l), ld3(s->cdd_ang, i_l), f1_ang, f1_vel);
    inertial_mul(cp, I, cm, cdv, cda, f2_ang, f2_vel);
    motion_cross_force(cda, cdv, f2_ang, f2_vel, f3_ang, f3_vel);
    V3 ext_ang = ld3(s->cfrc_ang, i_l), ext_vel = ld3(s->cfrc_vel, i_l);
    st3(s->cfrc_vel, i_l, f1_vel + f3_vel + ext_vel + v3(0, 0, 0));
    st3(s->cfrc_ang, i_l, f1_ang + f3_ang + ext_ang + v3(0, 0, 0));
  }
  team_sync();
  if (legs) {
    for (int c = tl; c < 6; c += T) {
      auto at = [&](int i_l) -> float* { return (c < 3) ? &s->cfrc_vel[3 * i_l + c] : &s->cfrc_ang[3 * i_l + c - 3]; };
      const int r = m.leg_root;
      float x[LEG_K][LEG_D];
#pragma unroll
      for (int l = 0; l < LEG_K; ++l)
#pragma unroll
        for (int d = 0; d < LEG_D; ++d) x[l][d] = *at(m.leg_links[LEG_D * l + d]);
      float a = *at(r);
#pragma unroll
      for (int l = 0; l < LEG_K; ++l) {
#pragma unroll
        for (int d = LEG_D - 2; d >= 0; --d) { x[l][d] = x[l][d] + x[l][d + 1]; *at(m.leg_links[LEG_D * l + d]) = x[l][d]; }
      }
#pragma unroll
      for (int l = 0; l < LEG_K; ++l) a = a + x[l][0];
      *at(r) = a;
    }
    team_sync();
  }
  for (int lev = (legs ? -1 : m.n_levels - 2); lev >= 0; --lev) {
    int n_par = m.level_start[lev + 1] - m.level_start[lev];
    for (int w = tl; w < n_par * 6; w += T) {
      int i_p = m.level_links[m.level_start[lev] + w / 6], comp = w % 6;
      float* dst = (comp < 3) ? &s->cfrc_vel[3 * i_p + comp] : &s->cfrc_ang[3 * i_p + comp - 3];
      float a = *dst;
      for (int c = m.child_start[i_p]; c < m.child_start[i_p + 1]; ++c) {
        int i_l = m.child_list[c];
        a = a + ((comp < 3) ? s->cfrc_vel[3 * i_l + comp] : s->cfrc_ang[3 * i_l + comp - 3]);
      }
      *dst = a;
    }
    team_sync();
  }
  for (int i_d = tl; i_d < ND; i_d += T) {
    int i_l = m.dof_link[i_d];
    float qf_bias = dot(ld3(s->cdof_ang, i_d), ld3(s->cfrc_ang, i_l)) + dot(ld3(s->cdof_vel, i_d), ld3(s->cfrc_vel, i_l));
    float f = s->qf_passive[i_d] - qf_bias + s->qf_applied[i_d];
    s->force[i_d] = f;
    if (env_valid) { astore(e, AO(force), i_d, f); astore(e, AO(qf_smooth), i_d, f); }
  }
  team_sync();
  PH(24)
  bool solved = false;
#if GO2SIM_FAST_ORDER
  if constexpr (T == 32 || T == 64) {
    if (arrow) {
      const int leg = (tl >> 3) & 3, u = tl & 7, ub = u < 6 ? u : 5;
      const int p0 = dm_arrow_dof(m.arrow_mode, leg, 0), p1 = dm_arrow_dof(m.arrow_mode, leg, 1), p2 = dm_arrow_dof(m.arrow_mode, leg, 2);
      float xb[6], x0, x1, x2;
      arrow_solve<T>(AF, s->force[p0], s->force[p1], s->force[p2], s->force[ub], s->Dinv, tl, xb, x0, x1, x2);
      if (tl == 0) {
#pragma unroll
        for (int k = 0; k < 6; ++k) s->out[k] = xb[k];
      }
      if (tl < 32 && u == 0) { s->out[p0] = x0; s->out[p1] = x1; s->out[p2] = x2; }
      solved = true;
    }
  }
#endif
  if (!solved) {
    float y[ND];
#pragma unroll
    for (int i_d_ = 0; i_d_ < ND; ++i_d_) {
      const int i_d = ND - i_d_ - 1;
      float cur = s->force[i_d];
#pragma unroll
      for (int j_d = i_d + 1; j_d < ND; ++j_d) cur = cur - s->L[j_d * ND + i_d] * y[j_d];
      y[i_d] = cur;
    }
#pragma unroll
    for (int i_d = 0; i_d < ND; ++i_d) y[i_d] = y[i_d] * s->Dinv[i_d];
#pragma unroll
    for (int i_d = 0; i_d < ND; ++i_d) {
      float cur = y[i_d];
#pragma unroll
      for (int j_d = 0; j_d < i_d; ++j_d) cur = cur - s->L[i_d * ND + j_d] * y[j_d];
      y[i_d] = cur;
    }
    if (tl == 0) {
#pragma unroll
      for (int i_d = 0; i_d < ND; ++i_d) s->out[i_d] = y[i_d];
    }
  }
  team_sync();
  if (env_valid) for (int i_d = tl; i_d < ND; i_d += T) { float a = s->out[i_d]; astore(e, AO(acc_smooth), i_d, a); astore(e, AO(acc), i_d, a); }
  if (env_valid) for (int idx = tl; idx < NTRI; idx += T) { int i, j; tri_index(m, idx, i, j); astore(e, AO(mass_mat), idx, s->M[i * ND + j]); }
  PH(25)
}

template <int T> DEV unsigned long long team_ballot(bool p) {
  const unsigned long long b = __ballot(p);
  if constexpr (T == 64) return b;
  else return (b >> (threadIdx.x & (64 - T))) & ((1ull << T) - 1ull);
}
template <int T>
struct BroadData {
  alignas(16) float amin[NG * 4], amax[NG * 4];
  alignas(16) unsigned long long skey[2 * NG];
  alignas(8) int rank_mm[NG * 2];
  int cand_key[MAXB], cand_pair[MAXB];
  unsigned pair_sorted[MAXB];
};
static_assert(NPAIR <= (1 << 16) && NG <= (1 << 8), "broad_word: 8 bits per geom, 16 bits of pair index");
DEV unsigned broad_word(int packed, int pidx) { return (unsigned)packed | ((unsigned)pidx << 16); }
constexpr int BROAD_PAD = 12;
template <int T> constexpr bool BROAD_OVERLAY = sizeof(BroadData<T>) + BROAD_PAD <= sizeof(DynData);
template <bool OVERLAY, int T> struct BroadSeparate { BroadData<T> k[64 / T]; DEV BroadData<T>* at(int slot, DynData*) { return &k[slot]; } };
template <int T> struct BroadSeparate<true, T> {
  DEV BroadData<T>* at(int slot, DynData* d) {
    static_assert(sizeof(BroadData<T>) + BROAD_PAD <= sizeof(DynData) && sizeof(DynData) % 4 == 0 && alignof(BroadData<T>) == 16, "BroadData overlay");
    return (BroadData<T>*)((char*)d + (16 - (slot * (int)sizeof(DynData)) % 16) % 16);
  }
};
static_assert((BROAD_OVERLAY<16> && BROAD_OVERLAY<32> && BROAD_OVERLAY<64>) || NG != 28 || ND != 18, "the Go2 shape keeps the dynamics kernels' LDS size");

template <int T>
DEV void tk_broadphase(const Model& m, const E& e, BroadData<T>* s, int tl) {
  const float inf = dm_bits2f(0x7f800000u);
  PH_BEGIN
  const int nc_old = e.n_contacts()[0];
  const bool first = e.first_time()[0] != 0;
  const unsigned ncv_old = (unsigned)e.ncache_valid()[tl < NCV ? tl : NCV - 1];
  constexpr int n2 = 2 * NG, NK = (2 * NG + T - 1) / T, NPI = (NPAIR + T - 1) / T, NGR = (NG + T - 1) / T;
  int sig_[NK];
#pragma unroll
  for (int q = 0; q < NK; ++q) { const int i = tl + q * T; sig_[q] = e.sort_ig()[i < n2 ? i : n2 - 1]; }
  int packed_[NPI];
  {
    const int n_pairs = m.n_pairs;
#pragma unroll
    for (int it = 0; it < NPI; ++it) { int pidx = it * T + tl; int v = m.pair_list[pidx < NPAIR ? pidx : NPAIR - 1]; packed_[it] = (pidx < n_pairs) ? v : -1; }
  }
  V3 lower_[NGR], upper_[NGR];
#pragma unroll
  for (int g = 0; g < NGR; ++g) {
    const int i_g = (g * T + tl < NG) ? g * T + tl : NG - 1;
    V3 lower = v3(inf, inf, inf), upper = v3(-inf, -inf, -inf);
    V3 gp = e.g_pos()[i_g]; Q4 gq = e.g_quat()[i_g];
#pragma unroll
    for (int c = 0; c < 8; ++c) {
      V3 corner = transform_by_trans_quat(m.geoms[i_g].aabb[c], gp, gq);
      lower = vmin(lower, corner); upper = vmax(upper, corner);
    }
    lower_[g] = lower; upper_[g] = upper;
  }
  team_sync();
#pragma unroll
  for (int g = 0; g < NGR; ++g) {
    const int i_g = (g * T + tl < NG) ? g * T + tl : NG - 1;
    *(float4*)&s->amin[4 * i_g] = make_float4(lower_[g].x, lower_[g].y, lower_[g].z, 0.0f);
    *(float4*)&s->amax[4 * i_g] = make_float4(upper_[g].x, upper_[g].y, upper_[g].z, 0.0f);
  }
  team_sync();
  PH(30)
  int r[NK]; float sorted_v[NK]; int sorted_sg[NK];
  unsigned long long key[NK];
#pragma unroll
  for (int q = 0; q < NK; ++q) {
    const int i = (tl + q * T < n2) ? tl + q * T : n2 - 1;
    const int sg = first ? ((i >> 1) | ((i & 1) ? 0x100 : 0)) : sig_[q];
    const int g = sg & 0xff;
    const float v = (sg & 0x100) ? s->amax[4 * g] : s->amin[4 * g];
    unsigned u = (unsigned)__float_as_int(v + 0.0f);
    u = (u & 0x80000000u) ? ~u : (u | 0x80000000u);
    key[q] = ((unsigned long long)u << 8) | (unsigned long long)i;
    s->skey[i] = key[q];
    sorted_v[q] = v; sorted_sg[q] = sg; r[q] = 0;
  }
  team_sync();
#pragma unroll
  for (int j = 0; j < 2 * NG; ++j) {
    const unsigned long long kj = s->skey[j];
#pragma unroll
    for (int q = 0; q < NK; ++q) r[q] += (kj < key[q]) ? 1 : 0;
  }
#pragma unroll
  for (int q = 0; q < NK; ++q)
    if (tl + q * T < n2) s->rank_mm[2 * (sorted_sg[q] & 0xff) + ((sorted_sg[q] & 0x100) ? 1 : 0)] = r[q];
  team_sync();
  PH(31)
  int n_cand = 0;
  unsigned ncv_clear = 0u;
  static_assert(NCV <= T, "one lane per word of the normal-cache mask");
#pragma unroll
  for (int it = 0; it < NPI; ++it) {
    const int packed = packed_[it];
    const int a = (packed < 0) ? 0 : (packed & 0xff), bg = (packed < 0) ? 0 : (packed >> 8);
    const int2 rka = *(const int2*)&s->rank_mm[2 * a], rkb = *(const int2*)&s->rank_mm[2 * bg];
    const float4 amn = *(const float4*)&s->amin[4 * a], amx = *(const float4*)&s->amax[4 * a], bmn = *(const float4*)&s->amin[4 * bg], bmx = *(const float4*)&s->amax[4 * bg];
    const int ra = rka.x, rb = rkb.x;
    const int rs = (ra < rb) ? rb : ra, rf = (ra < rb) ? ra : rb;
    const int rmax_first = (ra < rb) ? rka.y : rkb.y;
    const bool swept = packed >= 0 && rs < rmax_first;
    const bool any1 = (amx.x <= bmn.x) || (amx.y <= bmn.y) || (amx.z <= bmn.z);
    const bool any2 = (amn.x >= bmx.x) || (amn.y >= bmx.y) || (amn.z >= bmx.z);
    const bool cand = swept && !(any1 || any2);
    const unsigned long long cb = team_ballot<T>(cand);
    if (cand) {
      const int pos = n_cand + __popcll(cb & ((1ull << tl) - 1ull));
      if (pos < MAXB) { s->cand_key[pos] = rs * 64 + rf; s->cand_pair[pos] = (int)broad_word(packed, it * T + tl); }
    }
    n_cand += __popcll(cb);
    const unsigned long long sep = team_ballot<T>(swept && (any1 || any2));
    if constexpr (T < 32) { if (tl == ((it * T) >> 5)) ncv_clear |= (unsigned)(sep << ((it * T) & 31)); }
    else if constexpr (T == 32) { if (tl == it) ncv_clear |= (unsigned)sep; }
    else { if (tl == 2 * it) ncv_clear |= (unsigned)sep; if (tl == 2 * it + 1) ncv_clear |= (unsigned)(sep >> 32); }
  }
  const bool overflow = n_cand > m.max_broad_pairs;
  n_cand = imn(n_cand, MAXB);
  team_sync();
  for (int c = tl; c < n_cand; c += T) {
    const int ck = s->cand_key[c]; int cr = 0;
    for (int j = 0; j < n_cand; ++j) cr += s->cand_key[j] < ck;
    s->pair_sorted[cr] = (unsigned)s->cand_pair[c];
  }
  const int n_broad = imn(n_cand, m.max_broad_pairs);
  team_sync();
  for (int c = tl; c < n_broad; c += T) e.broad()[c] = (int)s->pair_sorted[c];
#pragma unroll
  for (int q = 0; q < NK; ++q) if (tl + q * T < n2) { e.sort_value()[r[q]] = sorted_v[q]; e.sort_ig()[r[q]] = sorted_sg[q]; }
  if (tl < NCV && ncv_clear != 0u) e.ncache_valid()[tl] = (int)(ncv_old & ~ncv_clear);
  if (tl == 0) {
    e.n_broad()[0] = n_broad;
    if (first) e.first_time()[0] = 0;
    if (overflow) atomicOr(&e.err()[0], GO2SIM_ERR_OVERFLOW_CANDIDATE_CONTACTS);
  }
  for (int i_c = tl; i_c < nc_old; i_c += T) {
    e.c_link()[i_c] = -1; e.c_link()[MAXC + i_c] = -1; e.c_geom()[i_c] = -1; e.c_geom()[MAXC + i_c] = -1;
    e.c_pen()[i_c] = 0.0f; e.c_pos()[i_c] = v3(0, 0, 0); e.c_normal()[i_c] = v3(0, 0, 0); e.c_force()[i_c] = v3(0, 0, 0);
  }
  PH(32)
}

template <int T>
__global__ __launch_bounds__(64) void k_dynamics_team(Pool P, const ModelS* __restrict__ mp, const Model* __restrict__ gm) {
  constexpr int EPW = 64 / T;
  __shared__ alignas(16) DynData lds[EPW];
  __shared__ alignas(16) char ms_raw[MODELS_LDS_BYTES];
  __shared__ BroadSeparate<BROAD_OVERLAY<T>, T> lds_b;
  const ModelS& ms = *(const ModelS*)ms_raw;
  wg_dma_to_lds<(int)sizeof(ModelS)>(ms_raw, mp);
  {
    const int b0 = xcd_block() * EPW;
    wg_load<EPW, NL * 3>(P, b0, FO(cd_vel), [&](int ev, int k, float v) { lds[ev].cd_vel[k] = v; });
    wg_load<EPW, NL * 3>(P, b0, FO(cd_ang), [&](int ev, int k, float v) { lds[ev].cd_ang[k] = v; });
    wg_load<EPW, ND>(P, b0, FO(vel), [&](int ev, int k, float v) { lds[ev].vel[k] = v; });
  }
  const int tl = threadIdx.x % T, slot = threadIdx.x / T;
  const int b = xcd_block() * EPW + slot;
  const bool env_valid = b < P.B;
  const ModelView m(&ms, mp);
  E e(P, env_valid ? b : P.B - 1);
  DynData* s = &lds[slot];
  PH_BEGIN
  team_stage<NL * 9, T>(tl, [&](int k) { return aload(e, AO(cinr_inertial), k); }, [&](int k, float v) { s->cinr_I[k] = v; s->crb_I[k] = v; });
  team_stage<NL * 3, T>(tl, [&](int k) { return aload(e, AO(cinr_pos), k); }, [&](int k, float v) { s->cinr_pos[k] = v; s->crb_pos[k] = v; });
  team_stage<NL, T>(tl, [&](int k) { return aload(e, AO(cinr_mass), k); }, [&](int k, float v) { s->cinr_mass[k] = v; s->crb_mass[k] = v; });
  team_stage<ND, T>(tl, [&](int d) { return __int_as_float((int)e.ctrl_mode()[d]); }, [&](int d, float v) { s->ctrl_mode[d] = __float_as_int(v); });
  team_stage<ND * 3, T>(tl, [&](int k) { return aload(e, AO(cdof_ang), k); }, [&](int k, float v) { s->cdof_ang[k] = v; });
  team_stage<ND * 3, T>(tl, [&](int k) { return aload(e, AO(cdof_vel), k); }, [&](int k, float v) { s->cdof_vel[k] = v; });
  team_stage<ND * 3, T>(tl, [&](int k) { return aload(e, AO(cdofd_ang), k); }, [&](int k, float v) { s->cdofd_ang[k] = v; });
  team_stage<ND * 3, T>(tl, [&](int k) { return aload(e, AO(cdofd_vel), k); }, [&](int k, float v) { s->cdofd_vel[k] = v; });
  team_stage<ND, T>(tl, [&](int d) { return gload(e, FO(ctrl_force), d); }, [&](int d, float v) { s->qf_applied[d] = v; });
  team_stage<ND, T>(tl, [&](int d) { return gload(e, FO(ctrl_pos), d); }, [&](int d, float v) { s->qf_passive[d] = v; });
  team_stage<ND, T>(tl, [&](int d) { return gload(e, FO(ctrl_vel), d); }, [&](int d, float v) { s->force[d] = v; });
  team_stage<ND, T>(tl, [&](int d) { return gload(e, FO(dof_pos), d); }, [&](int d, float v) { s->out[d] = v; });
  team_stage<NL * 6, T>(tl, [&](int k) { return gload(e, FO(ext), k); },
                        [&](int k, float v) { int i_l = k / 6, c = k % 6; if (c < 3) s->cfrc_ang[3 * i_l + c] = v; else s->cfrc_vel[3 * i_l + c - 3] = v; });
  team_sync();
  PH(20)
  tk_dynamics<T>(m, e, s, tl, env_valid);
  if (env_valid) tk_broadphase<T>(*gm, e, lds_b.at(slot, s), tl);
}


template <bool OVERLAY, int EPW> struct KinSeparate { KinData k[EPW]; DEV KinData* at(int slot, void*) { return &k[slot]; } };
template <int EPW> struct KinSeparate<true, EPW> { DEV KinData* at(int, void* overlay) { return (KinData*)overlay; } };
constexpr bool KIN_OVERLAY = sizeof(KinData) <= 2 * sizeof(float) * ND * ND;
template <int T>
DEV void integrate_fk_dynamics_body(const Pool& P, const ModelS* __restrict__ mp, const Model* __restrict__ gm, int b, DynData* lds_d, char* ms_raw,
                                    KinSeparate<KIN_OVERLAY, 64 / T>& lds_k, BroadSeparate<BROAD_OVERLAY<T>, T>& lds_b, bool pre, float pre_vel, float pre_acc) {
  const ModelS& ms = *(const ModelS*)ms_raw;
  wg_dma_to_lds<(int)sizeof(ModelS)>(ms_raw, mp);
  const int tl = threadIdx.x % T, slot = threadIdx.x / T;
  const ModelView m(&ms, mp);
  asm volatile("" : "+v"(b));
  E e(P, b < P.B ? b : P.B - 1);
  DynData* d = &lds_d[slot];
  static_assert(offsetof(DynData, L) == offsetof(DynData, M) + sizeof(float) * ND * ND, "KinData overlay");
  KinData* s = lds_k.at(slot, d->M);
  PH_BEGIN
  if (pre) { if (tl < ND) { s->vel[tl] = pre_vel; s->vel_next[tl] = pre_acc; } }
  else {
    team_stage<ND, T>(tl, [&](int i) { return gload(e, FO(vel), i); }, [&](int i, float v) { s->vel[i] = v; });
    team_stage<ND, T>(tl, [&](int i) { return aload(e, AO(acc), i); }, [&](int i, float a) { s->vel_next[i] = a; });
  }
  team_stage<NQ, T>(tl, [&](int q) { return gload(e, FO(qpos), q); }, [&](int q, float v) { s->qpos[q] = v; });
  team_stage<ND, T>(tl, [&](int i) { return __int_as_float((int)e.ctrl_mode()[i]); }, [&](int i, float v) { d->ctrl_mode[i] = __float_as_int(v); });
  team_stage<ND, T>(tl, [&](int i) { return gload(e, FO(ctrl_force), i); }, [&](int i, float v) { d->qf_applied[i] = v; });
  team_stage<ND, T>(tl, [&](int i) { return gload(e, FO(ctrl_pos), i); }, [&](int i, float v) { d->qf_passive[i] = v; });
  team_stage<ND, T>(tl, [&](int i) { return gload(e, FO(ctrl_vel), i); }, [&](int i, float v) { d->force[i] = v; });
  team_stage<NL * 6, T>(tl, [&](int k) { return gload(e, FO(ext), k); },
                        [&](int k, float v) { int i_l = k / 6, c = k % 6; if (c < 3) d->cfrc_ang[3 * i_l + c] = v; else d->cfrc_vel[3 * i_l + c - 3] = v; });
  team_for<ND, T>(tl, [&](int i) { s->vel_next[i] = s->vel[i] + s->vel_next[i] * m.substep_dt; });
  if (tl == 0) s->valid = 1;
  tk_stage_links<T>(e, s, tl);
  team_sync();
  if (b >= P.B) return;
  tk_integrate<T>(m, e, s, tl);
  PH(40)
  tk_kinematics<T>(m, e, s, tl, false, d);
  team_for<ND, T>(tl, [&](int i) { d->vel[i] = s->vel[i]; });
  team_sync();
  PH(41)
  tk_dynamics<T>(m, e, d, tl, true);
  tk_broadphase<T>(*gm, e, lds_b.at(slot, d), tl);
}
template <int T>
__global__ __launch_bounds__(64) void k_integrate_fk_dynamics_team(Pool P, const ModelS* __restrict__ mp, const Model* __restrict__ gm) {
  STAMP(STK_INT_FK_DYN)
  constexpr int EPW = 64 / T;
  __shared__ alignas(16) DynData lds_d[EPW];
  __shared__ alignas(16) char ms_raw[MODELS_LDS_BYTES];
  __shared__ KinSeparate<KIN_OVERLAY, EPW> lds_k;
  __shared__ BroadSeparate<BROAD_OVERLAY<T>, T> lds_b;
  integrate_fk_dynamics_body<T>(P, mp, gm, xcd_block() * EPW + (int)threadIdx.x / T, lds_d, ms_raw, lds_k, lds_b, false, 0.0f, 0.0f);
}

DEV int wrap180(float x) {
  if (!(x >= 0.0f)) return 0;
  int i = (x >= 180.0f) ? (int)(x - 180.0f) : (int)x;
  return (i > 179) ? 179 : i;
}
DEV int clampidx(float x) {
  if (!(x >= 0.0f)) return 0;
  return (x >= 179.0f) ? 179 : (int)x;
}
DEV V3 support_cylinder_local(const Model& m, const Geom& G, V3 d_mesh, int* vid_out = nullptr) {
  const float PI = 3.14159265358979323846f;
  float theta = dm_atan2(d_mesh.y, d_mesh.x);
  float phi = dm_acos(d_mesh.z);
  const float support_res = 180.0f;
  float ii = (theta + PI) / PI / 2.0f * support_res;
  float jj = phi / PI * support_res;
  const int i_lo = wrap180(dm_floor(ii)), i_hi = wrap180(dm_ceil(ii));
  int j_lo = clampidx(dm_floor(jj)); if (j_lo == 0) j_lo = 1;
  int j_hi = clampidx(dm_ceil(jj)); if (j_hi == 179) j_hi = 178;
  const int k_lo = m.theta_to_ring[i_lo], k_hi = m.theta_to_ring[i_hi];
  const float rx_lo = G.rim[k_lo][0], ry_lo = G.rim[k_lo][1], rx_hi = G.rim[k_hi][0], ry_hi = G.rim[k_hi][1];
  const float half = 0.5f * G.data[1];
  float dot_max = -1e20f;
  V3 v = v3(0, 0, 0);
  int vid = 0;
#pragma unroll
  for (int i4 = 0; i4 < 4; ++i4) {
    const bool hi_i = (i4 % 2) != 0, hi_j = (i4 / 2) > 0;
    const int j = hi_j ? j_hi : j_lo, k = hi_i ? k_hi : k_lo;
    V3 pos = v3(hi_i ? rx_hi : rx_lo, hi_i ? ry_hi : ry_lo, (j <= 90) ? half : -half);
    float d = dot(pos, d_mesh);
    if (d > dot_max) { v = pos; dot_max = d; vid = k + ((j <= 90) ? 0 : 32); }
  }
  if (vid_out) *vid_out = vid;
  return v;
}
DEV V3 vsel(bool c, V3 a, V3 b) { return v3(c ? a.x : b.x, c ? a.y : b.y, c ? a.z : b.z); }
DEV V3 support_prism(const V3* prism, V3 d) {
  const bool bottom = d.z < 0;
  const V3 p0 = vsel(bottom, prism[0], prism[3]), p1 = vsel(bottom, prism[1], prism[4]), p2 = vsel(bottom, prism[2], prism[5]);
  float best = dot(p0, d);
  V3 v = p0;
  const float dt1 = dot(p1, d);
  const bool b1 = dt1 > best;
  v = vsel(b1, p1, v); best = b1 ? dt1 : best;
  const float dt2 = dot(p2, d);
  v = vsel(dt2 > best, p2, v);
  return v;
}
struct GeomLite { int type; float d0, d1, d2; };
DEV GeomLite geom_lite(const GeomK* gk, int i_g) { const GeomK& G = gk[i_g]; GeomLite r = {G.type, G.data[0], G.data[1], G.data[2]}; return r; }
DEV V3 support_driver(const Model& m, V3 direction, int i_g, const GeomLite& gl, V3 pos, const Rot& rot, const V3* prism = nullptr) {
  if (gl.type == GEOM_TERRAIN) return support_prism(prism, direction);
  if (gl.type == GEOM_SPHERE) {
    return pos + direction * gl.d0;
  } else if (gl.type == GEOM_BOX) {
    V3 d_box = rot_apply_inv(rot, direction);
    V3 v_ = v3((d_box.x < 0.0f ? -1.0f : 1.0f) * gl.d0 * 0.5f, (d_box.y < 0.0f ? -1.0f : 1.0f) * gl.d1 * 0.5f,
               (d_box.z < 0.0f ? -1.0f : 1.0f) * gl.d2 * 0.5f);
    return rot_apply(rot, v_) + pos;
  } else if (gl.type == GEOM_CYLINDER) {
    V3 d_mesh = rot_apply_inv(rot, direction);
    V3 v_ = support_cylinder_local(m, m.geoms[i_g], d_mesh);
    return rot_apply(rot, v_) + pos;
  }
  return pos;
}
struct Pair { int i_ga, i_gb; V3 pos_a; Q4 quat_a; V3 pos_b; Q4 quat_b; const V3* prism; GeomLite ga, gb; Rot ra, rb; };
DEV void pair_set_rots(Pair& pr) { pr.ra = make_rot(pr.quat_a); pr.rb = make_rot(pr.quat_b); }
DEV void compute_support(const Model& m, V3 direction, const Pair& pr, V3& v, V3& v1, V3& v2) {
  v1 = support_driver(m, direction, pr.i_ga, pr.ga, pr.pos_a, pr.ra);
  v2 = support_driver(m, -direction, pr.i_gb, pr.gb, pr.pos_b, pr.rb, pr.prism);
  v = v1 - v2;
}


DEV V3 gjk_support_driver(const Model& m, V3 direction, int i_g, const GeomLite& gl, V3 pos, const Rot& rot, int& vid) {
  if (gl.type == GEOM_SPHERE) {
    vid = -1;
    return pos + direction * gl.d0;
  } else if (gl.type == GEOM_BOX) {
    V3 d_box = rot_apply_inv(rot, direction);
    V3 v_ = v3((d_box.x < 0.0f ? -1.0f : 1.0f) * gl.d0 * 0.5f, (d_box.y < 0.0f ? -1.0f : 1.0f) * gl.d1 * 0.5f,
               (d_box.z < 0.0f ? -1.0f : 1.0f) * gl.d2 * 0.5f);
    vid = (v_.x > 0.0f) * 1 + (v_.y > 0.0f) * 2 + (v_.z > 0.0f) * 4 + 64 * i_g;
    return rot_apply(rot, v_) + pos;
  } else if (gl.type == GEOM_CYLINDER) {
    V3 d_mesh = rot_apply_inv(rot, direction);
    int k = 0;
    V3 v_ = support_cylinder_local(m, m.geoms[i_g], d_mesh, &k);
    vid = k + 64 * i_g;
    return rot_apply(rot, v_) + pos;
  }
  vid = -1;
  return pos;
}
#include "go2sim_gjk_dev.h"

DEVN DgResult gjk_query_global(const DgPair& dp, GjkStoreFull* full, float eps) { return dg_contact(dp, *full, eps); }
DEV DgResult gjk_query(const DgPair& dp, GjkStoreLds* slots, unsigned* slot_mask, GjkStoreFull* full, float eps) {
  int slot = -1;
  if (slots) {
    for (int i = 0; i < GJK_SLOTS_MAX && slot < 0; ++i) {
      const unsigned bit = 1u << i;
      if (!(atomicOr(slot_mask, bit) & bit)) slot = i;
    }
  }
  DgResult r; r.is_col = false; r.overflow = true; r.penetration = 0.0f; r.normal = v3(0, 0, 0); r.pos = v3(0, 0, 0);
  if (slot >= 0) {
    r = dg_contact(dp, slots[slot], eps);
    atomicAnd(slot_mask, ~(1u << slot));
  }
  if (r.overflow) r = gjk_query_global(dp, full, eps);
  return r;
}

struct Simplex { V3 v[4], v1[4], v2[4]; };
DEV V3 mpr_portal_dir(const Simplex& s) { return normalized(cross(s.v[2] - s.v[1], s.v[3] - s.v[1])); }
DEV bool mpr_portal_reach_tolerance(const Model& m, const Simplex& s, V3 v, V3 direction) {
  float dv1 = dot(s.v[1], direction), dv2 = dot(s.v[2], direction), dv3 = dot(s.v[3], direction), dv4 = dot(v, direction);
  float dot1 = fmn(fmn(dv4 - dv1, dv4 - dv2), dv4 - dv3);
  return dot1 < m.ccd_tolerance + m.ccd_eps * fmx(1.0f, dot1);
}
DEV void simplex_set(Simplex& s, int i, V3 v, V3 v1, V3 v2) {
  const bool c1 = i == 1, c2 = i == 2, c3 = !(c1 || c2);
  s.v[1] = vsel(c1, v, s.v[1]); s.v1[1] = vsel(c1, v1, s.v1[1]); s.v2[1] = vsel(c1, v2, s.v2[1]);
  s.v[2] = vsel(c2, v, s.v[2]); s.v1[2] = vsel(c2, v1, s.v1[2]); s.v2[2] = vsel(c2, v2, s.v2[2]);
  s.v[3] = vsel(c3, v, s.v[3]); s.v1[3] = vsel(c3, v1, s.v1[3]); s.v2[3] = vsel(c3, v2, s.v2[3]);
}
DEV void mpr_expand_portal(Simplex& s, V3 v, V3 v1, V3 v2) {
  V3 v4v0 = cross(v, s.v[0]);
  float d = dot(s.v[1], v4v0);
  int i_s;
  if (d > 0) { d = dot(s.v[2], v4v0); i_s = (d > 0) ? 1 : 3; }
  else { d = dot(s.v[3], v4v0); i_s = (d > 0) ? 2 : 1; }
  simplex_set(s, i_s, v, v1, v2);
}
DEV bool mpr_first_support_separates(const Model& m, const Pair& pr, V3 center_a, V3 center_b) {
  const float EPSC = m.ccd_eps;
  V3 v0 = center_a - center_b;
  if (dm_abs(v0.x) < EPSC && dm_abs(v0.y) < EPSC && dm_abs(v0.z) < EPSC) v0.x += 10.0f * EPSC;
  const V3 direction = -normalized(v0);
  V3 v, v1, v2;
  compute_support(m, direction, pr, v, v1, v2);
  return dot(v, direction) < EPSC;
}
DEV int mpr_discover_portal(const Model& m, Simplex& s, const Pair& pr, V3 center_a, V3 center_b) {
  const float EPSC = m.ccd_eps;
  s.v1[0] = center_a; s.v2[0] = center_b; s.v[0] = center_a - center_b;
  int simplex_size = 1;
  if (dm_abs(s.v[0].x) < EPSC && dm_abs(s.v[0].y) < EPSC && dm_abs(s.v[0].z) < EPSC) s.v[0].x += 10.0f * EPSC;
  V3 direction = -normalized(s.v[0]);
  V3 v, v1, v2;
  compute_support(m, direction, pr, v, v1, v2);
  s.v1[1] = v1; s.v2[1] = v2; s.v[1] = v;
  simplex_size = 2;
  float d = dot(v, direction);
  int ret = 0;
  if (d < EPSC) {
    ret = -1;
  } else {
    direction = cross(s.v[0], s.v[1]);
    if (dot(direction, direction) < EPSC) {
      if (dm_abs(s.v[1].x) < EPSC && dm_abs(s.v[1].y) < EPSC && dm_abs(s.v[1].z) < EPSC) ret = 1; else ret = 2;
    } else {
      direction = normalized(direction);
      compute_support(m, direction, pr, v, v1, v2);
      d = dot(v, direction);
      if (d < EPSC) {
        ret = -1;
      } else {
        s.v1[2] = v1; s.v2[2] = v2; s.v[2] = v;
        simplex_size = 3;
        V3 va = s.v[1] - s.v[0], vb = s.v[2] - s.v[0];
        direction = normalized(cross(va, vb));
        d = dot(direction, s.v[0]);
        if (d > 0) {
          V3 t;
          t = s.v[1]; s.v[1] = s.v[2]; s.v[2] = t; t = s.v1[1]; s.v1[1] = s.v1[2]; s.v1[2] = t; t = s.v2[1]; s.v2[1] = s.v2[2]; s.v2[2] = t;
          direction = -direction;
        }
        int num_trials = 0;
        while (simplex_size < 4) {
          compute_support(m, direction, pr, v, v1, v2);
          d = dot(v, direction);
          if (d < EPSC) { ret = -1; break; }
          bool cont = false;
          va = cross(s.v[1], v);
          d = dot(va, s.v[0]);
          if (d < -EPSC) { s.v1[2] = v1; s.v2[2] = v2; s.v[2] = v; cont = true; }
          if (!cont) {
            va = cross(v, s.v[2]);
            d = dot(va, s.v[0]);
            if (d < -EPSC) { s.v1[1] = v1; s.v2[1] = v2; s.v[1] = v; cont = true; }
          }
          if (cont) {
            va = s.v[1] - s.v[0]; vb = s.v[2] - s.v[0];
            direction = normalized(cross(va, vb));
            num_trials++;
            if (num_trials == 15) { ret = -1; break; }
          } else {
            s.v1[3] = v1; s.v2[3] = v2; s.v[3] = v;
            simplex_size = 4;
          }
        }
      }
    }
  }
  return ret;
}
DEV int mpr_refine_portal(const Model& m, Simplex& s, const Pair& pr) {
  int ret = 1;
  while (true) {
    V3 direction = mpr_portal_dir(s);
    if (dot(s.v[1], direction) > -m.ccd_eps) { ret = 0; break; }
    V3 v, v1, v2;
    compute_support(m, direction, pr, v, v1, v2);
    if (!(dot(v, direction) > -m.ccd_eps) || mpr_portal_reach_tolerance(m, s, v, direction)) { ret = -1; break; }
    mpr_expand_portal(s, v, v1, v2);
  }
  return ret;
}
DEV V3 mpr_find_pos(const Model& m, const Simplex& s) {
  float b0 = 0.0f, b1 = 0.0f, b2 = 0.0f, b3 = 0.0f;
  float sum_ = ((b0 + b1) + b2) + b3;
  if (sum_ < m.ccd_eps) {
    V3 direction = mpr_portal_dir(s);
    b0 = 0.0f;
    b1 = dot(cross(s.v[2], s.v[3]), direction);
    b2 = dot(cross(s.v[3], s.v[1]), direction);
    b3 = dot(cross(s.v[1], s.v[2]), direction);
    sum_ = ((b0 + b1) + b2) + b3;
  }
  V3 p1 = v3(0, 0, 0), p2 = v3(0, 0, 0);
  p1 = p1 + b0 * s.v1[0]; p2 = p2 + b0 * s.v2[0];
  p1 = p1 + b1 * s.v1[1]; p2 = p2 + b1 * s.v2[1];
  p1 = p1 + b2 * s.v1[2]; p2 = p2 + b2 * s.v2[2];
  p1 = p1 + b3 * s.v1[3]; p2 = p2 + b3 * s.v2[3];
  return (0.5f / sum_) * (p1 + p2);
}
DEV void mpr_find_penetration(const Model& m, Simplex& s, const Pair& pr, bool& is_col, V3& normal, float& penetration, V3& pos) {
  int iterations = 0;
  while (true) {
    V3 direction = mpr_portal_dir(s);
    V3 v, v1, v2;
    compute_support(m, direction, pr, v, v1, v2);
    if (mpr_portal_reach_tolerance(m, s, v, direction) || iterations > m.ccd_iterations) {
      penetration = dot(direction, s.v[1]);
      normal = -direction;
      is_col = true;
      pos = mpr_find_pos(m, s);
      break;
    }
    mpr_expand_portal(s, v, v1, v2);
    iterations++;
  }
}
DEV void guess_geoms_center(const Model& m, const GeomK* gk, const Pair& pr, V3 normal_ws, V3& center_a, V3& center_b) {
  const GeomK& A = gk[pr.i_ga]; const GeomK& Bg = gk[pr.i_gb];
  center_a = transform_by_trans_quat(A.center, pr.pos_a, pr.quat_a);
  center_b = transform_by_trans_quat(Bg.center, pr.pos_b, pr.quat_b);
  if (dm_abs(normal_ws.x) > m.ccd_eps || dm_abs(normal_ws.y) > m.ccd_eps || dm_abs(normal_ws.z) > m.ccd_eps) {
    V3 center_a_local = A.aabb_mid;
    center_a = transform_by_trans_quat(center_a_local, pr.pos_a, pr.quat_a);
    V3 center_b_local = Bg.aabb_mid;
    center_b = transform_by_trans_quat(center_b_local, pr.pos_b, pr.quat_b);
    V3 delta = center_a - center_b;
    V3 normal = normalized(delta);
    if (norm(cross(normal_ws, normal)) > 0.01f) {
      V3 offset = dot(delta, normal_ws) * normal_ws - delta;
      float offset_norm = norm(offset);
      if (offset_norm > m.eps) {
        V3 dir_offset = offset / offset_norm;
        V3 dla = inv_transform_by_quat(dir_offset, pr.quat_a), dlb = inv_transform_by_quat(dir_offset, pr.quat_b);
        V3 box_size_a = A.aabb_size, box_size_b = Bg.aabb_size;
        float length_a = dot(box_size_a, v3(dm_abs(dla.x), dm_abs(dla.y), dm_abs(dla.z)));
        float length_b = dot(box_size_b, v3(dm_abs(dlb.x), dm_abs(dlb.y), dm_abs(dlb.z)));
        float offset_ratio = fmn(offset_norm / (length_a + length_b), 0.5f);
        center_a = center_a + dir_offset * length_a * offset_ratio;
        center_b = center_b - dir_offset * length_b * offset_ratio;
      }
    }
  }
}
DEV void mpr_contact_from_centers(const Model& m, const Pair& pr, V3 center_a, V3 center_b, bool& is_col, V3& normal, float& penetration, V3& pos) {
  Simplex s;
  int res = mpr_discover_portal(m, s, pr, center_a, center_b);
  is_col = false; pos = v3(0, 0, 0); normal = v3(0, 0, 0); penetration = 0.0f;
  if (res == 1) {
    is_col = true; penetration = 0.0f; normal = -normalized(s.v[0]); pos = (s.v1[1] + s.v2[1]) * 0.5f;
  } else if (res == 2) {
// ... 2015 lines not shown
    dp.ga = geom_lite(m.gk, i_ga); dp.gb = geom_lite(m.gk, i_gb); dp.ra = make_rot(qa); dp.rb = make_rot(qb);
    dp.discrete = m.geoms[i_ga].type == GEOM_BOX && m.geoms[i_gb].type == GEOM_BOX;
    const DgResult r = (which == 1) ? gjk_query(dp, slots, &mask, full, m.eps) : gjk_query(dp, nullptr, &mask, full, m.eps);
    is_col = r.is_col; pen = r.penetration; normal = r.normal; pos = r.pos;
  }
  out8[0] = is_col ? 1.0f : 0.0f; out8[1] = pen; out8[2] = normal.x; out8[3] = normal.y; out8[4] = normal.z; out8[5] = pos.x; out8[6] = pos.y; out8[7] = pos.z;
}

__global__ __launch_bounds__(64) void k_build_geomk(const Model* __restrict__ mp, GeomK* __restrict__ gk) {
  for (int i_g = (int)threadIdx.x; i_g < NG; i_g += 64) {
    const Geom& G = mp->geoms[i_g];
    GeomK k;
    k.type = G.type; k.link = G.link;
    for (int q = 0; q < 3; ++q) k.data[q] = G.data[q];
    for (int q = 0; q < 7; ++q) k.sol_params[q] = G.sol_params[q];
    k.center = G.center; k.aabb7 = G.aabb[7];
    k.aabb_mid = 0.5f * (G.aabb[7] + G.aabb[0]);
    k.aabb_size = G.aabb[7] - G.aabb[0];
    k.aabb_diag = norm(G.aabb[7] - G.aabb[0]);
    gk[i_g] = k;
  }
}

__global__ __launch_bounds__(WG) void k_clear_ext(Pool P) {
  int b = blockIdx.x * WG + threadIdx.x;
  if (b >= P.B) return;
  E e(P, b);
  auto ext = e.ext();
  for (int i = 0; i < NL * 6; ++i) ext[i] = 0.0f;
}

struct DCfg { double d[GO2SIM_FC_N_HOST]; float f[GO2SIM_FC_COUNT]; int i[GO2SIM_IC_COUNT]; };
struct Acc { double timeouts, tracking, ep[NREW]; int n_reset_now; int done; };
typedef go2sim_env_globals_t Glob;

enum { RNG_ACTION_NOISE = 1, RNG_PUSH = 2, RNG_CMD = 3, RNG_OBS_NOISE = 4, RNG_RESET_DR = 5, RNG_GLOBAL_DR = 6, RNG_RESET_CMD = 7, RNG_RESET_POSE = 8, RNG_TERRAIN_ROW = 9, RNG_TERRAIN_PERM = 10, RNG_RESET_KPKD = 11 };
__host__ __device__ inline dm_u4 rng4(uint64_t seed, uint32_t purpose, uint32_t env, uint32_t step, uint32_t idx) {
#ifdef GO2SIM_RNG_CONST
  dm_u4 o; o.v[0] = o.v[1] = o.v[2] = o.v[3] = step; (void)purpose; (void)env; (void)idx; (void)seed; return o;
#else
  return dm_philox(env, step, purpose, idx, (uint32_t)seed, (uint32_t)(seed >> 32));
#endif
}
__host__ __device__ inline float rand_float(double lower, double upper, uint32_t r) { return (float)(upper - lower) * dm_u01(r) + (float)lower; }
#ifdef GO2SIM_RNG_CONST
DEV int rand_int(int lower, int upper, uint32_t r) { return lower + (int)(dm_rng_const_u(r) * (float)(upper - lower + 1)); }
#else
DEV int rand_int(int lower, int upper, uint32_t r) { return lower + (int)(r % (uint32_t)(upper - lower + 1)); }
#endif
__host__ __device__ inline double clamp01d(double x) { return x < 0.0 ? 0.0 : (x > 1.0 ? 1.0 : x); }
__host__ __device__ inline double lerpd(double a, double b, double t) { t = clamp01d(t); return a + (b - a) * t; }
__host__ __device__ inline double lerp_lo(const DCfg& c, int easy_lo, double t) { return lerpd(c.d[easy_lo], c.d[easy_lo + 2], t); }
__host__ __device__ inline double lerp_hi(const DCfg& c, int easy_lo, double t) { return lerpd(c.d[easy_lo + 1], c.d[easy_lo + 3], t); }
DEV void sample_commands(const DCfg& c, const Glob& g, const dm_u4& r, int b, float& cx, float& cy, float& cz) {
  cx = rand_float(g.cmd_x_lo, g.cmd_x_hi, r.v[0]); cy = rand_float(g.cmd_y_lo, g.cmd_y_hi, r.v[1]); cz = rand_float(g.cmd_yaw_lo, g.cmd_yaw_hi, r.v[2]);
  if (!c.i[GO2SIM_IC_COMPOUND_COMMANDS]) {
    const int choice = rand_int(0, 2, r.v[3]);
    if (choice != 0) cx = 0.0f;
    if (choice != 1) cy = 0.0f;
    if (choice != 2) cz = 0.0f;
  }
  if (b < c.i[GO2SIM_IC_N_STANDING]) { cx = 0.0f; cy = 0.0f; cz = 0.0f; }
}

DEV Q4 tc_quat_mul(Q4 u, Q4 v) {
  float w1 = u.w, x1 = u.x, y1 = u.y, z1 = u.z, w2 = v.w, x2 = v.x, y2 = v.y, z2 = v.z;
  float ww = (z1 + x1) * (x2 + y2), yy = (w1 - y1) * (w2 + z2), zz = (w1 + y1) * (w2 - z2);
  float xx = ww + yy + zz;
  float qq = 0.5f * (xx + (z1 - x1) * (x2 - y2));
  Q4 o = q4(qq - ww + (z1 - y1) * (y2 - z2), qq - xx + (x1 + w1) * (x2 + w2), qq - yy + (w1 - x1) * (y2 + z2), qq - zz + (z1 + y1) * (w2 - x2));
  float n = dm_sqrt(norm_sqr(o));
  return q4(o.w / n, o.x / n, o.y / n, o.z / n);
}
DEV V3 tc_transform_by_quat(V3 v, Q4 q) {
  float q_ww = q.w * q.w, q_wx = q.w * q.x, q_wy = q.w * q.y, q_wz = q.w * q.z;
  float q_xx = q.x * q.x, q_xy = q.x * q.y, q_xz = q.x * q.z, q_yy = q.y * q.y, q_yz = q.y * q.z, q_zz = q.z * q.z;
  float den = q_ww + q_xx + q_yy + q_zz;
  float vx = v.x / den, vy = v.y / den, vz = v.z / den;
  return v3(vx * (q_xx + q_ww - q_yy - q_zz) + vy * (2.0f * q_xy - 2.0f * q_wz) + vz * (2.0f * q_xz + 2.0f * q_wy),
            vx * (2.0f * q_wz + 2.0f * q_xy) + vy * (q_ww - q_xx + q_yy - q_zz) + vz * (2.0f * q_yz - 2.0f * q_wx),
            vx * (2.0f * q_xz - 2.0f * q_wy) + vy * (2.0f * q_wx + 2.0f * q_yz) + vz * (q_ww - q_xx - q_yy + q_zz));
}
DEV V3 tc_quat_to_xyz_rpy_deg(Q4 q, float eps) {
  float q_ww = q.w * q.w, q_wx = q.w * q.x, q_wy = q.w * q.y, q_wz = q.w * q.z;
  float q_xx = q.x * q.x, q_xy = q.x * q.y, q_xz = q.x * q.z, q_yy = q.y * q.y, q_yz = q.y * q.z, q_zz = q.z * q.z;
  float sinp = q_wy - q_xz, sinrcosp = q_wx + q_yz, sinycosp = q_wz + q_xy;
  float cosrcosp = (q_ww - q_xx - q_yy + q_zz) / 2.0f, cosycosp = (q_ww + q_xx - q_yy - q_zz) / 2.0f;
  float cosp = dm_sqrt(cosycosp * cosycosp + sinycosp * sinycosp);
  float x = dm_atan2(sinrcosp, cosrcosp), y = dm_atan2(sinp, cosp), z = dm_atan2(sinycosp, cosycosp);
  if (cosp < eps) { x = 0.0f; z = dm_atan2(q_wz - q_xy, (q_ww - q_xx + q_yy - q_zz) / 2.0f); }
  const float R2D = 57.29577951308232f;
  return v3(x * R2D, y * R2D, z * R2D);
}

__host__ __device__ inline double dr_level(const DCfg& c, double terrain_level) {
  if (!c.i[GO2SIM_IC_DR_SCHEDULE]) return terrain_level;
  double gate = c.d[GO2SIM_FC_DR_TERRAIN_GATE], p1 = c.d[GO2SIM_FC_DR_PHASE1_LEVEL];
  if (terrain_level < gate) return p1;
  double den = 1.0 - gate; if (den < 1e-6) den = 1e-6;
  double progress = clamp01d((terrain_level - gate) / den);
  return lerpd(p1, 1.0, progress);
}
DEV float terrain_height(const Model& m, const DCfg& c, float x, float y) {
  if (!c.i[GO2SIM_IC_USE_TERRAIN] || !m.terrain_enabled) return 0.0f;
  long long col = (long long)((x - c.f[GO2SIM_FC_TERRAIN_ORIGIN_X]) / c.f[GO2SIM_FC_TERRAIN_H_SCALE]);
  long long row = (long long)((y - c.f[GO2SIM_FC_TERRAIN_ORIGIN_Y]) / c.f[GO2SIM_FC_TERRAIN_H_SCALE]);
  col = col < 0 ? 0 : (col > m.terrain_rows - 1 ? m.terrain_rows - 1 : col);
  row = row < 0 ? 0 : (row > m.terrain_cols - 1 ? m.terrain_cols - 1 : row);
  return m.terrain_hf[(size_t)col * m.terrain_cols + row];
}
__host__ __device__ inline void apply_curriculum_level(const DCfg& c, Glob& g) {
  double lvl_terrain = c.i[GO2SIM_IC_CURR_ENABLED] ? g.level : 1.0;
  double lvl = dr_level(c, lvl_terrain);
  g.obs_noise_level_cur = lerpd(0.0, c.i[GO2SIM_IC_HAS_OBS_NOISE] ? c.d[GO2SIM_FC_OBS_NOISE_LEVEL_MAX] : 0.0, lvl);
  g.action_noise_std_cur = lerpd(0.0, c.d[GO2SIM_FC_ACTION_NOISE_STD_MAX], lvl);
  double dt = c.d[GO2SIM_FC_DT];
  if (!c.i[GO2SIM_IC_HAS_PUSH]) {
    g.push_enable = 0; g.push_force_lo = g.push_force_hi = 0.0; g.push_interval = 1000000000;
  } else {
    double push_start = c.d[GO2SIM_FC_PUSH_START];
    if (lvl < push_start) {
      g.push_enable = 0; g.push_force_lo = g.push_force_hi = 0.0;
      g.push_interval = (int)(c.d[GO2SIM_FC_PUSH_INTERVAL_S_EASY] / dt);
    } else {
      double den = 1.0 - push_start; if (den < 1e-6) den = 1e-6;
      double s = clamp01d((lvl - push_start) / den);
      g.push_force_lo = c.d[GO2SIM_FC_PUSH_FORCE_LO] * s;
      g.push_force_hi = c.d[GO2SIM_FC_PUSH_FORCE_HI] * s;
      double interval_s = lerpd(c.d[GO2SIM_FC_PUSH_INTERVAL_S_EASY], c.d[GO2SIM_FC_PUSH_INTERVAL_S_HARD], s);
      int iv = (int)(interval_s / dt);
      g.push_interval = iv < 1 ? 1 : iv;
      g.push_enable = 1;
    }
  }
  g.delay_max_cur = (int)rint(lerpd((double)c.i[GO2SIM_IC_DELAY_EASY_MAX], (double)c.i[GO2SIM_IC_MAX_DELAY], lvl));
  double frac = c.i[GO2SIM_IC_CMD_CURRICULUM] ? lerpd(c.d[GO2SIM_FC_CMD_START_FRAC], 1.0, lvl_terrain) : 1.0;
  {
    double lo = c.d[GO2SIM_FC_CMD_X_LO], hi = c.d[GO2SIM_FC_CMD_X_HI], center = (lo + hi) / 2.0, half = (hi - lo) / 2.0;
    g.cmd_x_lo = center - half * frac; g.cmd_x_hi = center + half * frac;
    lo = c.d[GO2SIM_FC_CMD_Y_LO]; hi = c.d[GO2SIM_FC_CMD_Y_HI]; center = (lo + hi) / 2.0; half = (hi - lo) / 2.0;
    g.cmd_y_lo = center - half * frac; g.cmd_y_hi = center + half * frac;
    lo = c.d[GO2SIM_FC_CMD_YAW_LO]; hi = c.d[GO2SIM_FC_CMD_YAW_HI]; center = (lo + hi) / 2.0; half = (hi - lo) / 2.0;
    g.cmd_yaw_lo = center - half * frac; g.cmd_yaw_hi = center + half * frac;
  }
}

__host__ __device__ inline bool curriculum_update(const DCfg& c, Glob& g, double timeout_rate, double tracking_per_sec, double fall_rate) {
  double a = c.d[GO2SIM_FC_CURR_EMA_ALPHA];
  if (!g.ema_valid) { g.timeout_rate_ema = timeout_rate; g.tracking_ema = tracking_per_sec; g.fall_rate_ema = fall_rate; g.ema_valid = 1; }
  else {
    g.timeout_rate_ema = (1.0 - a) * g.timeout_rate_ema + a * timeout_rate;
    g.tracking_ema = (1.0 - a) * g.tracking_ema + a * tracking_per_sec;
    g.fall_rate_ema = (1.0 - a) * g.fall_rate_ema + a * fall_rate;
  }
  if (g.cooldown > 0) g.cooldown -= 1;
  bool ready = g.timeout_rate_ema >= c.d[GO2SIM_FC_CURR_READY_TIMEOUT_RATE] && g.tracking_ema >= c.d[GO2SIM_FC_CURR_READY_TRACKING] &&
               g.fall_rate_ema <= c.d[GO2SIM_FC_CURR_READY_FALL_RATE];
  bool hard = g.fall_rate_ema >= c.d[GO2SIM_FC_CURR_HARD_FALL_RATE];
  g.ready_streak = ready ? g.ready_streak + 1 : 0;
  g.hard_streak = hard ? g.hard_streak + 1 : 0;
  double old_level = g.level;
  if (g.hard_streak >= c.i[GO2SIM_IC_CURR_HARD_STREAK]) {
    { double lo = c.d[GO2SIM_FC_CURR_LEVEL_MIN], v = g.level - c.d[GO2SIM_FC_CURR_STEP_DOWN]; g.level = (lo < v) ? v : lo; }
    g.hard_streak = 0; g.ready_streak = 0; g.cooldown = c.i[GO2SIM_IC_CURR_COOLDOWN];
  } else if (g.ready_streak >= c.i[GO2SIM_IC_CURR_READY_STREAK] && g.cooldown == 0) {
    { double hi = c.d[GO2SIM_FC_CURR_LEVEL_MAX], v = g.level + c.d[GO2SIM_FC_CURR_STEP_UP]; g.level = (v < hi) ? v : hi; }
    g.ready_streak = 0; g.cooldown = c.i[GO2SIM_IC_CURR_COOLDOWN];
  }
  g.level = clamp01d(g.level);
  return g.level != old_level;
}

__global__ __launch_bounds__(WG) void k_env_pre(Pool P, const Model* __restrict__ mp, const DCfg cv, const Glob* __restrict__ gp,
                                                const float* __restrict__ actions_in, uint64_t seed, uint32_t step_count, int write_idx) {
  int b = blockIdx.x * WG + threadIdx.x;
  if (b >= P.B) return;
  const DCfg& c = cv;  const Glob& g = *gp;
  E e(P, b);
  const int na = c.i[GO2SIM_IC_NUM_ACTIONS];
  float clip = c.f[GO2SIM_FC_CLIP_ACTIONS];
  auto actions = e.actions(); auto hist = e.action_history(); auto applied = e.applied_actions();
  auto target_dof_pos = e.target_dof_pos(); auto kp_factors = e.kp_factors(); auto kd_factors = e.kd_factors(); auto motor_strength = e.motor_strength();
  auto dof_pos = e.e_dof_pos(); auto dof_vel = e.e_dof_vel(); auto torque_ = e.torque(); auto ctrl_mode = e.ctrl_mode(); auto ctrl_force = e.ctrl_force();
  auto cpf = e.current_push_force(); auto psf = e.push_stored_force(); auto prem = e.push_remaining(); auto ext = e.ext();
  const bool manual_pd = c.i[GO2SIM_IC_MANUAL_PD] != 0, pls = c.i[GO2SIM_IC_PLS_ENABLE] != 0;
  const bool push_on = c.i[GO2SIM_IC_HAS_PUSH] && g.push_enable;
  const int pl = c.i[GO2SIM_IC_PUSH_LINK];
  int delay = e.delay_steps()[0];
  const bool base_env = c.i[GO2SIM_IC_ENV_KIND] == 1;
  const int depth = c.i[GO2SIM_IC_MAX_DELAY] + 1;
  const int read_idx = (((write_idx - delay) % depth) + depth) % depth;
  auto last_a = e.last_actions();
  float a_in[NA], h_[NA];
#pragma unroll
  for (int i = 0; i < NA; ++i) {
    a_in[i] = (i < na) ? actions_in[(size_t)b * na + i] : 0.0f;
    h_[i] = base_env ? last_a[i] : hist[read_idx][i];
  }
  float kpf[NM], kdf[NM], mst[NM], dp[NM], dv[NM];
#pragma unroll
  for (int i = 0; i < NM; ++i) { kpf[i] = kp_factors[i]; kdf[i] = kd_factors[i]; mst[i] = motor_strength[i]; dp[i] = dof_pos[i]; dv[i] = dof_vel[i]; }
  float bkp = c.f[GO2SIM_FC_KP], bkd = c.f[GO2SIM_FC_KD];
  if (manual_pd && !pls && c.i[GO2SIM_IC_HAS_KP_RANGE]) { bkp = e.base_kp()[0]; bkd = e.base_kd()[0]; }
  float psf_[3] = {psf[0], psf[1], psf[2]}; int rem0 = prem[0];
  V3 pl_pos = e.l_pos()[pl], pl_com = e.root_com()[pl];
  float ext_[6];
#pragma unroll
  for (int k = 0; k < 6; ++k) ext_[k] = ext[6 * pl + k];
  float delayed[NA];
#pragma unroll
  for (int i = 0; i < NA; ++i) {
    if (i < na) {
      float a = fmn(fmx(a_in[i], -clip), clip);
      actions[i] = a;
      float d;
      if (base_env) d = (depth > 1) ? h_[i] : a;
      else { hist[write_idx][i] = a; d = (read_idx == write_idx) ? a : h_[i]; }
      delayed[i] = d; applied[i] = d;
    } else {
      delayed[i] = 0.0f;
    }
  }
  float target[NM];
#pragma unroll
  for (int i = 0; i < NM; ++i) target[i] = delayed[i] * c.f[GO2SIM_FC_ACTION_SCALE] + c.f[GO2SIM_FC_DEFAULT_DOF_POS0 + i];
  if (g.action_noise_std_cur > 0.0) {
#pragma unroll
    for (int blk = 0; blk < 3; ++blk) {
      dm_u4 r = rng4(seed, RNG_ACTION_NOISE, b, step_count, blk);
      float n0, n1, n2, n3;
      dm_normal2(r.v[0], r.v[1], &n0, &n1); dm_normal2(r.v[2], r.v[3], &n2, &n3);
      target[4 * blk + 0] = target[4 * blk + 0] + n0 * (float)g.action_noise_std_cur;
      target[4 * blk + 1] = target[4 * blk + 1] + n1 * (float)g.action_noise_std_cur;
      target[4 * blk + 2] = target[4 * blk + 2] + n2 * (float)g.action_noise_std_cur;
      target[4 * blk + 3] = target[4 * blk + 3] + n3 * (float)g.action_noise_std_cur;
    }
  }
  if (!manual_pd) {
    auto ctrl_pos = e.ctrl_pos(); auto ctrl_vel = e.ctrl_vel();
#pragma unroll
    for (int i = 0; i < NM; ++i) {
      target_dof_pos[i] = target[i];
      int d = c.i[GO2SIM_IC_MOTOR_DOF0 + i];
      ctrl_mode[d] = CTRL_POSITION; ctrl_pos[d] = target[i]; ctrl_vel[d] = 0.0f; ctrl_force[d] = 0.0f;
      torque_[i] = 0.0f;
    }
  } else
#pragma unroll
  for (int i = 0; i < NM; ++i) {
    target_dof_pos[i] = target[i];
    float eff_kp, eff_kd;
    if (pls) {
      int leg = i / 3;
      float kp_leg = c.f[GO2SIM_FC_PLS_KP_DEFAULT] + delayed[NM + leg] * c.f[GO2SIM_FC_PLS_KP_ACTION_SCALE];
      kp_leg = fmn(fmx(kp_leg, c.f[GO2SIM_FC_PLS_KP_MIN]), c.f[GO2SIM_FC_PLS_KP_MAX]);
      float kd_j = 0.2f * dm_sqrt(kp_leg);
      eff_kp = kp_leg * kpf[i] * mst[i];
      eff_kd = kd_j * kdf[i];
    } else {
      eff_kp = bkp * kpf[i]; eff_kd = bkd * kdf[i];
    }
    float pos_error = target[i] - dp[i];
    float torque = eff_kp * pos_error - eff_kd * dv[i];
    float lim = c.f[GO2SIM_FC_TORQUE_LIMIT0 + i];
    torque = fmn(fmx(torque, -lim), lim);
    torque_[i] = torque;
    int d = c.i[GO2SIM_IC_MOTOR_DOF0 + i];
    ctrl_mode[d] = CTRL_FORCE; ctrl_force[d] = torque;
  }
  if (!push_on) {
    cpf[0] = 0.0f; cpf[1] = 0.0f; cpf[2] = 0.0f;
  } else {
    if (g.push_counter % g.push_interval == 0) {
      dm_u4 r = rng4(seed, RNG_PUSH, b, step_count, 0);
      psf_[0] = rand_float(g.push_force_lo, g.push_force_hi, r.v[0]);
      psf_[1] = rand_float(g.push_force_lo, g.push_force_hi, r.v[1]);
      psf_[2] = 0.0f;
      psf[0] = psf_[0]; psf[1] = psf_[1]; psf[2] = psf_[2];
      rem0 = rand_int(c.i[GO2SIM_IC_PUSH_DUR_LO], c.i[GO2SIM_IC_PUSH_DUR_HI], r.v[2]);
    }
    int rem = rem0;
    float active = (rem > 0) ? 1.0f : 0.0f;
    V3 force = v3(psf_[0] * active, psf_[1] * active, psf_[2] * active);
    cpf[0] = force.x; cpf[1] = force.y; cpf[2] = force.z;
    prem[0] = imx(rem - 1, 0);
    V3 tq = cross(pl_pos - pl_com, force);
    ext[6 * pl + 0] = ext_[0] - tq.x; ext[6 * pl + 1] = ext_[1] - tq.y; ext[6 * pl + 2] = ext_[2] - tq.z;
    ext[6 * pl + 3] = ext_[3] - force.x; ext[6 * pl + 4] = ext_[4] - force.y; ext[6 * pl + 5] = ext_[5] - force.z;
  }
}

template <int T>
__global__ __launch_bounds__(64) void k_pre_dynamics_team(Pool P, const ModelS* __restrict__ mp, const DCfg cv, const Glob* __restrict__ gp,
                                                          const float* __restrict__ actions_in, uint64_t seed, uint32_t step_count, int write_idx,
                                                          const Model* __restrict__ gm) {
  STAMP(STK_PRE_DYN)
  static_assert(T >= NA, "one lane per action");
  constexpr int EPW = 64 / T;
  __shared__ alignas(16) DynData lds[EPW];
  __shared__ alignas(16) char ms_raw[MODELS_LDS_BYTES];
  __shared__ BroadSeparate<BROAD_OVERLAY<T>, T> lds_b;
  const ModelS& ms = *(const ModelS*)ms_raw;
  wg_dma_to_lds<(int)sizeof(ModelS)>(ms_raw, mp);
  {
    const int b0 = xcd_block() * EPW;
    wg_load<EPW, NL * 3>(P, b0, FO(cd_vel), [&](int ev, int k, float v) { lds[ev].cd_vel[k] = v; });
    wg_load<EPW, NL * 3>(P, b0, FO(cd_ang), [&](int ev, int k, float v) { lds[ev].cd_ang[k] = v; });
    wg_load<EPW, ND>(P, b0, FO(vel), [&](int ev, int k, float v) { lds[ev].vel[k] = v; });
  }
  const int tl = threadIdx.x % T, slot = threadIdx.x / T;
  const int b = xcd_block() * EPW + slot;
  const bool env_valid = b < P.B;
  const ModelView m(&ms, mp);
  E e(P, env_valid ? b : P.B - 1);
  DynData* s = &lds[slot];
  const DCfg& c = cv; const Glob& g = *gp;
  PH_BEGIN
  const int na = c.i[GO2SIM_IC_NUM_ACTIONS];
  const int ia = tl < NA ? tl : NA - 1, im = tl < NM ? tl : NM - 1;
  const int eb = env_valid ? b : P.B - 1;
  auto hist = e.action_history();
  const int delay = e.delay_steps()[0];
  const float a_in = (ia < na) ? actions_in[(size_t)eb * na + ia] : 0.0f;
  const bool base_env = c.i[GO2SIM_IC_ENV_KIND] == 1;
  const int depth = c.i[GO2SIM_IC_MAX_DELAY] + 1;
  const int read_idx = (((write_idx - delay) % depth) + depth) % depth;
  const float h_ = base_env ? e.last_actions()[ia] : hist[read_idx][ia];
  const float kpf = e.kp_factors()[im], kdf = e.kd_factors()[im], mst = e.motor_strength()[im], dp = e.e_dof_pos()[im], dv = e.e_dof_vel()[im];
  const bool manual_pd = c.i[GO2SIM_IC_MANUAL_PD] != 0, pls = c.i[GO2SIM_IC_PLS_ENABLE] != 0;
  const bool base_gains = manual_pd && !pls && c.i[GO2SIM_IC_HAS_KP_RANGE];
  const float bkp = base_gains ? e.base_kp()[0] : c.f[GO2SIM_FC_KP], bkd = base_gains ? e.base_kd()[0] : c.f[GO2SIM_FC_KD];
  const bool push_on = c.i[GO2SIM_IC_HAS_PUSH] && g.push_enable;
  const int pl = c.i[GO2SIM_IC_PUSH_LINK];
  auto psf = e.push_stored_force(); auto prem = e.push_remaining(); auto cpf = e.current_push_force(); auto ext = e.ext();
  float psf_[3] = {psf[0], psf[1], psf[2]}; int rem0 = prem[0];
  const V3 pl_pos = e.l_pos()[pl], pl_com = e.root_com()[pl];
  float ext_[6];
#pragma unroll
  for (int k = 0; k < 6; ++k) ext_[k] = ext[6 * pl + k];
  team_stage<NL * 9, T>(tl, [&](int k) { return aload(e, AO(cinr_inertial), k); }, [&](int k, float v) { s->cinr_I[k] = v; s->crb_I[k] = v; });
  team_stage<NL * 3, T>(tl, [&](int k) { return aload(e, AO(cinr_pos), k); }, [&](int k, float v) { s->cinr_pos[k] = v; s->crb_pos[k] = v; });
  team_stage<NL, T>(tl, [&](int k) { return aload(e, AO(cinr_mass), k); }, [&](int k, float v) { s->cinr_mass[k] = v; s->crb_mass[k] = v; });
  team_stage<ND, T>(tl, [&](int d) { return __int_as_float((int)e.ctrl_mode()[d]); }, [&](int d, float v) { s->ctrl_mode[d] = __float_as_int(v); });
  team_stage<ND * 3, T>(tl, [&](int k) { return aload(e, AO(cdof_ang), k); }, [&](int k, float v) { s->cdof_ang[k] = v; });
  team_stage<ND * 3, T>(tl, [&](int k) { return aload(e, AO(cdof_vel), k); }, [&](int k, float v) { s->cdof_vel[k] = v; });
  team_stage<ND * 3, T>(tl, [&](int k) { return aload(e, AO(cdofd_ang), k); }, [&](int k, float v) { s->cdofd_ang[k] = v; });
  team_stage<ND * 3, T>(tl, [&](int k) { return aload(e, AO(cdofd_vel), k); }, [&](int k, float v) { s->cdofd_vel[k] = v; });
  team_stage<ND, T>(tl, [&](int d) { return gload(e, FO(ctrl_force), d); }, [&](int d, float v) { s->qf_applied[d] = v; });
  team_stage<ND, T>(tl, [&](int d) { return gload(e, FO(ctrl_pos), d); }, [&](int d, float v) { s->qf_passive[d] = v; });
  team_stage<ND, T>(tl, [&](int d) { return gload(e, FO(ctrl_vel), d); }, [&](int d, float v) { s->force[d] = v; });
  team_stage<ND, T>(tl, [&](int d) { return gload(e, FO(dof_pos), d); }, [&](int d, float v) { s->out[d] = v; });
  team_stage<NL * 6, T>(tl, [&](int k) { return gload(e, FO(ext), k); },
                        [&](int k, float v) { int i_l = k / 6, cc = k % 6; if (cc < 3) s->cfrc_ang[3 * i_l + cc] = v; else s->cfrc_vel[3 * i_l + cc - 3] = v; });
  team_sync();
  if (env_valid) {
    const float clip = c.f[GO2SIM_FC_CLIP_ACTIONS];
    float delayed = 0.0f;
    if (tl < NA && tl < na) {
      const float a = fmn(fmx(a_in, -clip), clip);
      e.actions()[tl] = a;
      if (base_env) delayed = (depth > 1) ? h_ : a;
      else { hist[write_idx][tl] = a; delayed = (read_idx == write_idx) ? a : h_; }
      e.applied_actions()[tl] = delayed;
    }
    const float delayed_leg = __shfl(delayed, NM + im / 3, T);
    if (tl < NM) {
      float target = delayed * c.f[GO2SIM_FC_ACTION_SCALE] + c.f[GO2SIM_FC_DEFAULT_DOF_POS0 + tl];
      if (g.action_noise_std_cur > 0.0) {
        dm_u4 r = rng4(seed, RNG_ACTION_NOISE, b, step_count, tl / 4);
        float n0, n1;
        if ((tl & 2) == 0) dm_normal2(r.v[0], r.v[1], &n0, &n1); else dm_normal2(r.v[2], r.v[3], &n0, &n1);
        target = target + ((tl & 1) ? n1 : n0) * (float)g.action_noise_std_cur;
      }
      e.target_dof_pos()[tl] = target;
      const int d = c.i[GO2SIM_IC_MOTOR_DOF0 + tl];
      if (!manual_pd) {
        e.ctrl_mode()[d] = CTRL_POSITION; e.ctrl_pos()[d] = target; e.ctrl_vel()[d] = 0.0f; e.ctrl_force()[d] = 0.0f;
        e.torque()[tl] = 0.0f;
        s->ctrl_mode[d] = CTRL_POSITION; s->qf_passive[d] = target; s->force[d] = 0.0f; s->qf_applied[d] = 0.0f;
      } else {
        float eff_kp, eff_kd;
        if (pls) {
          float kp_leg = c.f[GO2SIM_FC_PLS_KP_DEFAULT] + delayed_leg * c.f[GO2SIM_FC_PLS_KP_ACTION_SCALE];
          kp_leg = fmn(fmx(kp_leg, c.f[GO2SIM_FC_PLS_KP_MIN]), c.f[GO2SIM_FC_PLS_KP_MAX]);
          const float kd_j = 0.2f * dm_sqrt(kp_leg);
          eff_kp = kp_leg * kpf * mst;
          eff_kd = kd_j * kdf;
        } else {
          eff_kp = bkp * kpf; eff_kd = bkd * kdf;
        }
        const float pos_error = target - dp;
        float torque = eff_kp * pos_error - eff_kd * dv;
        const float lim = c.f[GO2SIM_FC_TORQUE_LIMIT0 + tl];
        torque = fmn(fmx(torque, -lim), lim);
        e.torque()[tl] = torque;
        e.ctrl_mode()[d] = CTRL_FORCE; e.ctrl_force()[d] = torque;
        s->ctrl_mode[d] = CTRL_FORCE; s->qf_applied[d] = torque;
      }
    }
    if (tl == T - 1) {
      if (!push_on) {
        cpf[0] = 0.0f; cpf[1] = 0.0f; cpf[2] = 0.0f;
      } else {
        if (g.push_counter % g.push_interval == 0) {
          dm_u4 r = rng4(seed, RNG_PUSH, b, step_count, 0);
          psf_[0] = rand_float(g.push_force_lo, g.push_force_hi, r.v[0]);
          psf_[1] = rand_float(g.push_force_lo, g.push_force_hi, r.v[1]);
          psf_[2] = 0.0f;
          psf[0] = psf_[0]; psf[1] = psf_[1]; psf[2] = psf_[2];
          rem0 = rand_int(c.i[GO2SIM_IC_PUSH_DUR_LO], c.i[GO2SIM_IC_PUSH_DUR_HI], r.v[2]);
        }
        const float active = (rem0 > 0) ? 1.0f : 0.0f;
        const V3 force = v3(psf_[0] * active, psf_[1] * active, psf_[2] * active);
        cpf[0] = force.x; cpf[1] = force.y; cpf[2] = force.z;
        prem[0] = imx(rem0 - 1, 0);
        const V3 tq = cross(pl_pos - pl_com, force);
        const float x0 = ext_[0] - tq.x, x1 = ext_[1] - tq.y, x2 = ext_[2] - tq.z, x3 = ext_[3] - force.x, x4 = ext_[4] - force.y, x5 = ext_[5] - force.z;
        ext[6 * pl + 0] = x0; ext[6 * pl + 1] = x1; ext[6 * pl + 2] = x2; ext[6 * pl + 3] = x3; ext[6 * pl + 4] = x4; ext[6 * pl + 5] = x5;
        s->cfrc_ang[3 * pl + 0] = x0; s->cfrc_ang[3 * pl + 1] = x1; s->cfrc_ang[3 * pl + 2] = x2;
        s->cfrc_vel[3 * pl + 0] = x3; s->cfrc_vel[3 * pl + 1] = x4; s->cfrc_vel[3 * pl + 2] = x5;
      }
    }
  }
  team_sync();
  PH(20)
  tk_dynamics<T>(m, e, s, tl, env_valid);
  if (env_valid) tk_broadphase<T>(*gm, e, lds_b.at(slot, s), tl);
}

struct RewCtx { float link_vel_xy[8], foot_z[4], foot_xy[8]; float vel_world[3]; int was_reset; };
struct RewState {
  float cmd[3], blv[3], bav[3], pg[3], base_pos[3];
  float dof_pos[NM], dof_vel[NM], last_dof_vel[NM], target[NM], ctrl_force[NM];
  float actions[NA], last_actions[NA];
  float fat[4]; int fc[4];
  float last_x;
  float ctrl_pos[NM], ctrl_vel[NM], s_vel[NM], s_dof_pos[NM]; int ctrl_mode[NM];
};
DEV void load_rew_state(const DCfg& c, const E& e, RewState& rs) {
  auto cmd = e.commands(); auto ldv = e.last_dof_vel(); auto t = e.target_dof_pos(); auto cf = e.ctrl_force(); auto a = e.actions(); auto la = e.last_actions();
  auto fat = e.feet_air_time();
#pragma unroll
  for (int i = 0; i < 3; ++i) rs.cmd[i] = cmd[i];
#pragma unroll
  for (int i = 0; i < NM; ++i) { rs.last_dof_vel[i] = ldv[i]; rs.target[i] = t[i]; rs.ctrl_force[i] = cf[c.i[GO2SIM_IC_MOTOR_DOF0 + i]]; }
#pragma unroll
  for (int i = 0; i < NA; ++i) { rs.actions[i] = a[i]; rs.last_actions[i] = la[i]; }
#pragma unroll
  for (int i = 0; i < 4; ++i) rs.fat[i] = fat[i];
  rs.last_x = e.last_base_pos_x()[0];
  if (c.i[GO2SIM_IC_ENV_KIND] == 1) {
    auto ctrl_mode = e.ctrl_mode(); auto cp = e.ctrl_pos(); auto cv = e.ctrl_vel(); auto vel = e.vel(); auto sdp = e.dof_pos();
#pragma unroll
    for (int i = 0; i < NM; ++i) {
      int d = c.i[GO2SIM_IC_MOTOR_DOF0 + i];
      rs.ctrl_mode[i] = ctrl_mode[d]; rs.ctrl_pos[i] = cp[d]; rs.ctrl_vel[i] = cv[d]; rs.s_vel[i] = vel[d]; rs.s_dof_pos[i] = sdp[d];
    }
  }
}
struct RewGates { float still, moving; };
DEV RewGates reward_gates(const RewState& rs) {
  const float c0 = rs.cmd[0], c1 = rs.cmd[1], c2 = rs.cmd[2];
  const float cmd_norm = dm_sqrt(c0 * c0 + c1 * c1 + c2 * c2);
  RewGates g;
  g.still = (cmd_norm < 0.1f) ? 1.0f : 0.0f;
  g.moving = (dm_sqrt(c0 * c0 + c1 * c1) > 0.1f) ? 1.0f : 0.0f;
  return g;
}
struct RewK { float dt, sigma, lin_vel_z_deadzone, base_height_target, feet_air_time_target, feet_height_target; float def[NM], force_lo[NM], force_hi[NM]; int na, use_terrain; };
DEV RewK load_rew_k(const Model& m, const DCfg& c) {
  RewK K;
  K.dt = c.f[GO2SIM_FC_DT]; K.sigma = c.f[GO2SIM_FC_TRACKING_SIGMA]; K.lin_vel_z_deadzone = c.f[GO2SIM_FC_LIN_VEL_Z_DEADZONE];
  K.base_height_target = c.f[GO2SIM_FC_BASE_HEIGHT_TARGET]; K.feet_air_time_target = c.f[GO2SIM_FC_FEET_AIR_TIME_TARGET]; K.feet_height_target = c.f[GO2SIM_FC_FEET_HEIGHT_TARGET];
  K.na = c.i[GO2SIM_IC_NUM_ACTIONS]; K.use_terrain = c.i[GO2SIM_IC_USE_TERRAIN];
#pragma unroll
  for (int i = 0; i < NM; ++i) {
    const int d = c.i[GO2SIM_IC_MOTOR_DOF0 + i];
    K.def[i] = c.f[GO2SIM_FC_DEFAULT_DOF_POS0 + i]; K.force_lo[i] = m.dofs[d].force_range[0]; K.force_hi[i] = m.dofs[d].force_range[1];
  }
  return K;
}
DEV float reward_term(const Model& m, const DCfg& c, const RewK& K, RewState& rs, int id, const RewCtx& rc, const RewGates& gt) {
  const float dt = K.dt;
  const float* cmd = rs.cmd; const float* blv = rs.blv; const float* bav = rs.bav; const float* dof_pos = rs.dof_pos; const float* dof_vel = rs.dof_vel;
  float c0 = cmd[0], c1 = cmd[1], c2 = cmd[2];
  const float still = gt.still, moving = gt.moving;
  switch (id) {
    case GO2SIM_R_TRACKING_LIN_VEL: { float d0 = c0 - blv[0], d1 = c1 - blv[1]; return dm_exp(-(d0 * d0 + d1 * d1) / K.sigma); }
    case GO2SIM_R_TRACKING_ANG_VEL: { float d = c2 - bav[2]; return dm_exp(-(d * d) / K.sigma); }
    case GO2SIM_R_LIN_VEL_Z: {
      float v = blv[2], dz = K.lin_vel_z_deadzone;
      if (dz > 0.0f) { float ex = fmx(dm_abs(v) - dz, 0.0f); return ex * ex; }
      return v * v;
    }
    case GO2SIM_R_ACTION_RATE: {
      float s = 0.0f; const int na = K.na;
#pragma unroll
      for (int i = 0; i < NA; ++i) if (i < na) { float d = rs.last_actions[i] - rs.actions[i]; s = s + d * d; }
      return s;
    }
    case GO2SIM_R_SIMILAR_TO_DEFAULT: {
      float s = 0.0f;
#pragma unroll
      for (int i = 0; i < NM; ++i) s = s + dm_abs(dof_pos[i] - K.def[i]);
      return s;
    }
    case GO2SIM_R_BASE_HEIGHT: {
      float hgt = rs.base_pos[2];
      if (K.use_terrain) hgt = rs.base_pos[2] - terrain_height(m, c, rs.base_pos[0], rs.base_pos[1]);
      float d = hgt - K.base_height_target; return d * d;
    }
    case GO2SIM_R_DOF_ACC: {
      float s = 0.0f;
#pragma unroll
      for (int i = 0; i < NM; ++i) { float a = (dof_vel[i] - rs.last_dof_vel[i]) / dt; s = s + a * a; }
      return s;
    }
    case GO2SIM_R_DOF_VEL: {
      float s = 0.0f;
#pragma unroll
      for (int i = 0; i < NM; ++i) { float v = dof_vel[i]; s = s + v * v; }
      return s;
    }
    case GO2SIM_R_ORIENTATION_PENALTY: { float a = rs.pg[0], b2 = rs.pg[1]; return a * a + b2 * b2; }
    case GO2SIM_R_ANG_VEL_XY: { float a = bav[0], b2 = bav[1]; return a * a + b2 * b2; }
    case GO2SIM_R_STAND_STILL: {
      float s = 0.0f;
#pragma unroll
      for (int i = 0; i < NM; ++i) s = s + dm_abs(dof_pos[i] - K.def[i]);
      return s * still;
    }
    case GO2SIM_R_STAND_STILL_VEL: { float a = blv[0], b2 = blv[1], w = bav[2]; float lin = a * a + b2 * b2; float ang = w * w; return (lin + 0.5f * ang) * still; }
    case GO2SIM_R_FEET_STANCE: {
      float sa = 0.0f, sn = 0.0f;
#pragma unroll
      for (int i = 0; i < 4; ++i) { sa = sa + rs.fat[i]; sn = sn + (rs.fc[i] ? 0.0f : 1.0f); }
      return (sa + sn) * still;
    }
    case GO2SIM_R_FEET_AIR_TIME: {
      float first[4], at[4];
#pragma unroll
      for (int i = 0; i < 4; ++i) { float a = rs.fat[i]; int ct = rs.fc[i]; first[i] = (a > 0.0f && ct) ? 1.0f : 0.0f; a = a + dt; a = a * (ct ? 0.0f : 1.0f); rs.fat[i] = a; at[i] = a; }
      float s = 0.0f;
#pragma unroll
      for (int i = 0; i < 4; ++i) s = s + (at[i] - K.feet_air_time_target) * first[i];
      return s * moving;
    }
    case GO2SIM_R_FOOT_SLIP: {
      float slip = 0.0f;
#pragma unroll
      for (int i = 0; i < 4; ++i) { float vx = rc.link_vel_xy[2 * i], vy = rc.link_vel_xy[2 * i + 1]; slip = slip + (rs.fc[i] ? 1.0f : 0.0f) * (vx * vx + vy * vy); }
      return slip;
    }
    case GO2SIM_R_FOOT_CLEARANCE: {
      float pen = 0.0f;
#pragma unroll
      for (int i = 0; i < 4; ++i) {
        float vx = rc.link_vel_xy[2 * i], vy = rc.link_vel_xy[2 * i + 1];
        float vn = dm_sqrt(vx * vx + vy * vy);
        float fz = rc.foot_z[i];
        if (K.use_terrain) fz = rc.foot_z[i] - terrain_height(m, c, rc.foot_xy[2 * i], rc.foot_xy[2 * i + 1]);
        float he = K.feet_height_target - fz; he = he * he;
        pen = pen + (rs.fc[i] ? 0.0f : 1.0f) * he * vn;
      }
      return pen * moving;
    }
    case GO2SIM_R_JOINT_TRACKING: {
      float s = 0.0f;
#pragma unroll
      for (int i = 0; i < NM; ++i) { float d = rs.target[i] - dof_pos[i]; s = s + d * d; }
      return s;
    }
    case GO2SIM_R_ENERGY: case GO2SIM_R_TORQUE_LOAD: {
      float s = 0.0f;
#pragma unroll
      for (int i = 0; i < NM; ++i) {
        float tau = clampf(rs.ctrl_force[i], K.force_lo[i], K.force_hi[i]);
        s = s + ((id == GO2SIM_R_ENERGY) ? dm_abs(tau * dof_vel[i]) : dm_abs(tau));
      }
      return s;
    }
    case GO2SIM_R_JUMP_IMPULSE: { float gate = (rs.base_pos[2] < 0.50f) ? 1.0f : 0.0f; return gate * fmx(blv[2], 0.0f); }
    case GO2SIM_R_JUMP_APEX: { float q = (rs.base_pos[2] - c.f[GO2SIM_FC_JUMP_APEX_HEIGHT]) / c.f[GO2SIM_FC_JUMP_APEX_SIGMA]; return dm_exp(-(q * q)); }
    case GO2SIM_R_XY_STABILITY: { float vx = rc.vel_world[0], vy = rc.vel_world[1]; return -(vx * vx + vy * vy); }
    case GO2SIM_R_ORIENTATION: return -rs.pg[2];
    case GO2SIM_R_NO_SHAKE: { float a = bav[0], b2 = bav[1], c3 = bav[2]; return -((a * a + b2 * b2) + c3 * c3) / 1.0f; }
    case GO2SIM_R_CROUCH: return (rs.base_pos[2] < 0.25f) ? 1.0f : 0.0f;
    case GO2SIM_R_CROUCH_2: { float z = rs.base_pos[2]; return (z <= 0.30f && z >= 0.20f) ? 1.0f : 0.0f; }
    case GO2SIM_R_GROUND_PENALTY: { float v = (0.15f - rs.base_pos[2]) / 0.1f; v = fmn(fmx(v, 0.0f), 1.0f); return -(v * v); }
    case GO2SIM_R_CROUCH_TARGET: { float q = (rs.base_pos[2] - 0.15f) / 0.03f; return dm_exp(-(q * q)); }
    case GO2SIM_R_NO_FALL: { float dn = fmx(-blv[2] - 0.5f, 0.0f); return -(dn * dn); }
    case GO2SIM_R_Y_STABILITY: { float vy = rc.vel_world[1]; return -(vy * vy); }
    case GO2SIM_R_TORQUE_LOAD_BASE: {
      float s = 0.0f;
#pragma unroll
      for (int i = 0; i < NM; ++i) {
        int d = c.i[GO2SIM_IC_MOTOR_DOF0 + i];
        const Dof& D = m.dofs[d];
        float pos_d = rc.was_reset ? ((m.qpos0[d + 1] + dof_pos[i]) - m.qpos0[d + 1]) : rs.s_dof_pos[i];
        float vel_d = rc.was_reset ? 0.0f : rs.s_vel[i];
        float force = 0.0f;
        int cm = rs.ctrl_mode[i];
        if (cm == CTRL_FORCE) force = rs.ctrl_force[i];
        else if (cm == CTRL_VELOCITY) force = D.kv * (rs.ctrl_vel[i] - vel_d);
        else if (cm == CTRL_POSITION) force = D.kp * (rs.ctrl_pos[i] - pos_d) + D.kv * (rs.ctrl_vel[i] - vel_d);
        s = s + dm_abs(clampf(force, D.force_range[0], D.force_range[1]));
      }
      return -0.001f * s;
    }
    case GO2SIM_R_CROUCH_PROGRESS: return fmx(0.35f - rs.base_pos[2], 0.0f);
    case GO2SIM_R_CROUCH_SPEED: return -(blv[2] * blv[2]);
    case GO2SIM_R_ORIENTATION_ROLL_ONLY: { float gy = rs.pg[1]; return gy * gy; }
    case GO2SIM_R_FORWARD_PROGRESS: { float bx = rs.base_pos[0]; float dx = bx - rs.last_x; rs.last_x = bx; return dx; }
  }
  return 0.0f;
}

DEV void env_globals_body(const DCfg& c, Glob& g, Acc* acc, uint64_t seed, int count_push);
constexpr int POST_A_NWAVES = 4;
struct TermDeal { uint32_t w[NREW / 8]; uint32_t tracking; };
static_assert(NREW == 32 && POST_A_NWAVES >= 2 && POST_A_NWAVES <= 16, "TermDeal holds four bits per term");
__global__ __launch_bounds__(WG * POST_A_NWAVES) void k_env_post_a(Pool P, const Model* __restrict__ mp, const DCfg cv, Glob* gp,
                                                   Acc* acc, uint64_t seed, uint32_t step_count, const TermDeal deal) {
  STAMP(STK_POST_A)
  __shared__ float s_es[NREW][WG], s_r[NREW][WG];
  const int ln = threadIdx.x % WG, wv = threadIdx.x / WG;
  const bool w0 = wv == 0;
  int b = blockIdx.x * WG + ln;
  if (b >= P.B) return;
  const Model& m = *mp; const DCfg& c = cv;  const Glob& g = *gp;
  E e(P, b);
  const int nrew = c.i[GO2SIM_IC_N_REWARDS];
  const bool base_env = c.i[GO2SIM_IC_ENV_KIND] == 1;
  PH_BEGIN
  int ep_len = e.episode_length()[0] + 1;
  int bl = c.i[GO2SIM_IC_BASE_LINK];
  V3 bp = e.l_pos()[bl]; Q4 bq = e.l_quat()[bl];
  V3 rcom = e.root_com()[bl];
  V3 cda = e.cd_ang()[bl], cdv = e.cd_vel()[bl];
  V3 f_cf[4], f_lp[4], f_cdv[4], f_cda[4]; int fc_old[4];
  {
    auto fc = e.foot_contact();
#pragma unroll
    for (int i = 0; i < 4; ++i) {
      int l = c.i[GO2SIM_IC_FOOT_LINK0 + i];
      fc_old[i] = fc[i];
      f_cf[i] = e.contact_force()[l]; f_lp[i] = e.l_pos()[l]; f_cdv[i] = e.cd_vel()[l]; f_cda[i] = e.cd_ang()[l];
    }
  }
  RewState rs;
  {
    auto sdof_pos = e.dof_pos(); auto vel = e.vel();
#pragma unroll
    for (int i = 0; i < NM; ++i) { int d = c.i[GO2SIM_IC_MOTOR_DOF0 + i]; rs.dof_pos[i] = sdof_pos[d]; rs.dof_vel[i] = vel[d]; }
  }
  if (!base_env) load_rew_state(c, e, rs);
  else { auto cmd = e.commands(); for (int i = 0; i < 3; ++i) rs.cmd[i] = cmd[i]; }
  {
    auto episode_sums = e.episode_sums();
    float es_[NREW];
#pragma unroll
    for (int k = 0; k < NREW; ++k) es_[k] = episode_sums[k];
    if (w0) {
#pragma unroll
      for (int k = 0; k < NREW; ++k) s_es[k][ln] = es_[k];
    }
  }
  PH(12)
  if (w0) {
    { auto ext = e.ext(); for (int i = 0; i < NL * 6; ++i) ext[i] = 0.0f; }
    e.episode_length()[0] = ep_len;
    auto base_pos = e.base_pos(); auto base_quat = e.base_quat();
    base_pos[0] = bp.x; base_pos[1] = bp.y; base_pos[2] = bp.z;
    base_quat[0] = bq.w; base_quat[1] = bq.x; base_quat[2] = bq.y; base_quat[3] = bq.z;
  }
  Q4 inv_init = inv_quat(q4(c.f[GO2SIM_FC_BASE_INIT_QUAT0], c.f[GO2SIM_FC_BASE_INIT_QUAT0 + 1], c.f[GO2SIM_FC_BASE_INIT_QUAT0 + 2], c.f[GO2SIM_FC_BASE_INIT_QUAT0 + 3]));
  V3 eul = tc_quat_to_xyz_rpy_deg(tc_quat_mul(bq, inv_init), m.eps);
  Q4 inv_bq = inv_quat(bq);
  V3 velw = cdv + cross(cda, bp - rcom);
  V3 blv = tc_transform_by_quat(velw, inv_bq), bav = tc_transform_by_quat(cda, inv_bq);
  V3 pg = tc_transform_by_quat(v3(0.0f, 0.0f, -1.0f), inv_bq);
  if (w0) {
    auto base_euler = e.base_euler();
    base_euler[0] = eul.x; base_euler[1] = eul.y; base_euler[2] = eul.z;
    { auto bvw = e.base_vel_world(); bvw[0] = velw.x; bvw[1] = velw.y; bvw[2] = velw.z; }
    auto o_blv = e.base_lin_vel(); auto o_bav = e.base_ang_vel(); auto o_pg = e.projected_gravity();
    o_blv[0] = blv.x; o_blv[1] = blv.y; o_blv[2] = blv.z;
    o_bav[0] = bav.x; o_bav[1] = bav.y; o_bav[2] = bav.z;
    o_pg[0] = pg.x; o_pg[1] = pg.y; o_pg[2] = pg.z;
  }
  rs.blv[0] = blv.x; rs.blv[1] = blv.y; rs.blv[2] = blv.z; rs.bav[0] = bav.x; rs.bav[1] = bav.y; rs.bav[2] = bav.z;
  rs.pg[0] = pg.x; rs.pg[1] = pg.y; rs.pg[2] = pg.z; rs.base_pos[0] = bp.x; rs.base_pos[1] = bp.y; rs.base_pos[2] = bp.z;
  if (w0) {
    auto dof_pos = e.e_dof_pos(); auto dof_vel = e.e_dof_vel();
#pragma unroll
    for (int i = 0; i < NM; ++i) { dof_pos[i] = rs.dof_pos[i]; dof_vel[i] = rs.dof_vel[i]; }
  }
  RewCtx rc; rc.was_reset = 0; rc.vel_world[0] = velw.x; rc.vel_world[1] = velw.y; rc.vel_world[2] = velw.z;
  auto fc = e.foot_contact(); auto lfc = e.last_foot_contact();
#pragma unroll
  for (int i = 0; i < 4; ++i) {
    int ct = dm_abs(f_cf[i].z) > c.f[GO2SIM_FC_FOOT_CONTACT_THRESHOLD];
    if (w0) { lfc[i] = fc_old[i]; fc[i] = ct; }
    rs.fc[i] = ct;
    V3 lp = f_lp[i];
    V3 lv = f_cdv[i] + cross(f_cda[i], lp - rcom);
    rc.link_vel_xy[2 * i] = lv.x; rc.link_vel_xy[2 * i + 1] = lv.y; rc.foot_z[i] = lp.z; rc.foot_xy[2 * i] = lp.x; rc.foot_xy[2 * i + 1] = lp.y;
  }
  if (ep_len % c.i[GO2SIM_IC_RESAMPLE_STEPS] == 0) {
    auto cmd = e.commands();
    dm_u4 r = rng4(seed, RNG_CMD, b, step_count, 0);
    float cx, cy, cz;
    sample_commands(c, g, r, b, cx, cy, cz);
    if (w0) { cmd[0] = cx; cmd[1] = cy; cmd[2] = cz; }
    rs.cmd[0] = cx; rs.cmd[1] = cy; rs.cmd[2] = cz;
  }
  int maxlen = c.i[GO2SIM_IC_MAX_EPISODE_LENGTH];
  int rst = ep_len > maxlen;
  rst |= dm_abs(eul.y) > c.f[GO2SIM_FC_TERM_PITCH_DEG];
  rst |= dm_abs(eul.x) > c.f[GO2SIM_FC_TERM_ROLL_DEG];
  rst |= dm_abs(blv.z) > c.f[GO2SIM_FC_TERM_ZVEL];
  rst |= dm_abs(blv.y) > c.f[GO2SIM_FC_TERM_YVEL];
  float time_out = (ep_len > maxlen) ? 1.0f : 0.0f;
  if (w0) { e.reset_buf()[0] = rst; e.time_out()[0] = time_out; }
  float rew = 0.0f;
  float tracking_int = 0.0f;
  PH(13)
  const float fat0[4] = {rs.fat[0], rs.fat[1], rs.fat[2], rs.fat[3]};
  const float last_x0 = rs.last_x;
  const RewGates gates = reward_gates(rs);
// ... 1697 lines not shown
```

Before: 18.25 million.

## Use LDS-only team syncs, keep geom poses in registers, defer dynamics stores into broadphase

Most team_sync calls between LDS-only phases become team_sync_lds, which fences only local memory so outstanding global stores need not drain at every barrier. Geom poses computed in kinematics are passed to the broadphase in registers instead of being re-read from global memory. Per-link mass and COM shifts are prefetched before the first barrier. The acc and mass-matrix global stores are moved into the broadphase so they overlap AABB computation. The control kernel hoists its global loads (action ring, gains) ahead of staging, with asm pins forcing early issue. The price is more register pressure and a subtle memory-ordering risk if any phase actually depends on global data that the narrower fence no longer orders.

```diff
diff --git a/go2_sim2real_locomotion_rl_amd/csrc/go2sim.hip b/go2_sim2real_locomotion_rl_amd/csrc/go2sim.hip
--- a/go2_sim2real_locomotion_rl_amd/csrc/go2sim.hip
+++ b/go2_sim2real_locomotion_rl_amd/csrc/go2sim.hip
@@ -629,6 +629,7 @@
   __builtin_amdgcn_wave_barrier();
   __builtin_amdgcn_fence(__ATOMIC_ACQUIRE, "workgroup", "local");
 }
+DEV void issued(float x) { asm volatile("" ::"v"(x)); }
 DEV float gload(const E& e, int off, int k) { return e.f[(size_t)(off + k) * e.B]; }
 DEV void gstore(const E& e, int off, int k, float v) { e.f[(size_t)(off + k) * e.B] = v; }
 DEV float aload(const E& e, int off, int k) { return e.fa[off + k]; }
@@ -893,12 +894,21 @@
 static_assert(!ARROW_SHAPE || (offsetof(DynData, Dinv) % 8 == 0 && sizeof(DynData) % 8 == 0), "arrow_solve reads DynData::Dinv with 8-byte LDS loads");
 #endif
 
+struct LinkShift { float mass; V3 com; };
+template <int T>
+DEV LinkShift tk_load_shift(const E& e, int tl) {
+  const int i_l = tl < NL ? tl : NL - 1;
+  LinkShift r; r.mass = gload(e, FO(mass_shift), i_l); r.com = e.com_shift()[i_l];
+  return r;
+}
+template <int T> struct GeomPose { V3 p[(NG + T - 1) / T]; Q4 q[(NG + T - 1) / T]; };
 template <int T>
 DEV void tk_stage_links(const E& e, KinData* s, int tl) {
   team_for<NL, T>(tl, [&](int i_l) { st3(s->l_pos, i_l, e.l_pos()[i_l]); st4(s->l_quat, i_l, e.l_quat()[i_l]); });
 }
 template <int T, class MT>
-DEV void tk_kinematics(const MT& m, const E& e, KinData* s, int tl, bool force_update_fixed, DynData* dk = nullptr) {
+DEV void tk_kinematics(const MT& m, const E& e, KinData* s, int tl, bool force_update_fixed, DynData* dk = nullptr, const LinkShift* ls = nullptr,
+                       GeomPose<T>* gout = nullptr) {
   PH_BEGIN
   const bool legs = (T == 32 || T == 64) && m.leg_form;
   if (legs) {
@@ -956,7 +966,7 @@
         st3(s->l_pos, lk[d], pos); st4(s->l_quat, lk[d], quat); e.l_pos()[lk[d]] = pos; e.l_quat()[lk[d]] = quat;
       }
     }
-    team_sync();
+    team_sync_lds();
   }
   for (int lev = 0; lev < (legs ? 0 : m.n_levels); ++lev) {
     for (int k = m.level_start[lev] + tl; k < m.level_start[lev + 1]; k += T) {
@@ -996,17 +1006,20 @@
       }
       if (!(L.parent == -1 && L.is_fixed)) { st3(s->l_pos, i_l, pos); st4(s->l_quat, i_l, quat); e.l_pos()[i_l] = pos; e.l_quat()[i_l] = quat; }
     }
-    team_sync();
+    team_sync_lds();
   }
   PH(18)
   for (int i_l = tl; i_l < NL; i_l += T) {
     const auto& L = m.links[i_l];
-    s->mass[i_l] = L.mass + gload(e, FO(mass_shift), i_l);
+    float mass_shift; V3 com_shift;
+    if (T >= NL && ls) { mass_shift = ls->mass; com_shift = ls->com; }
+    else { mass_shift = gload(e, FO(mass_shift), i_l); com_shift = e.com_shift()[i_l]; }
+    s->mass[i_l] = L.mass + mass_shift;
     V3 ipbw; Q4 iq;
-    transform_pos_quat_by_trans_quat(L.inertial_pos + (V3)e.com_shift()[i_l], L.inertial_quat, ld3(s->l_pos, i_l), ld4(s->l_quat, i_l), ipbw, iq);
+    transform_pos_quat_by_trans_quat(L.inertial_pos + com_shift, L.inertial_quat, ld3(s->l_pos, i_l), ld4(s->l_quat, i_l), ipbw, iq);
     st3(s->i_pos, i_l, ipbw); st4(s->i_quat, i_l, iq);
   }
-  team_sync();
+  team_sync_lds();
   V3 rc[2];
 #pragma unroll
   for (int i_e = 0; i_e < 2; ++i_e) {
@@ -1019,7 +1032,7 @@
     }
     rc[i_e] = root_com_bw / mass_sum;
   }
-  team_sync();
+  team_sync_lds();
   for (int i_l = tl; i_l < NL; i_l += T) {
     const auto& L = m.links[i_l];
     V3 r = (L.entity == 0) ? rc[0] : rc[1];
@@ -1066,7 +1079,22 @@
       }
     }
   }
-  for (int i_g = tl; i_g < NG; i_g += T) {
+  if (gout) {
+#pragma unroll
+    for (int g = 0; g < (NG + T - 1) / T; ++g) {
+      const bool mine = g * T + tl < NG;
+      const int i_g = mine ? g * T + tl : NG - 1;
+      const auto& G = m.geoms[i_g];
+      bool is_fixed = m.links[G.link].is_fixed;
+      V3 p; Q4 q;
+      if (force_update_fixed || !is_fixed) {
+        transform_pos_quat_by_trans_quat(G.pos, G.quat, ld3(s->l_pos, G.link), ld4(s->l_quat, G.link), p, q);
+        if (mine) { e.g_pos()[i_g] = p; e.g_quat()[i_g] = q; }
+      } else { p = e.g_pos()[i_g]; q = e.g_quat()[i_g]; }
+      gout->p[g] = p; gout->q[g] = q;
+    }
+  }
+  for (int i_g = tl; i_g < (gout ? 0 : NG); i_g += T) {
     const auto& G = m.geoms[i_g];
     bool is_fixed = m.links[G.link].is_fixed;
     if (force_update_fixed || !is_fixed) {
@@ -1075,7 +1103,7 @@
       e.g_pos()[i_g] = p; e.g_quat()[i_g] = q;
     }
   }
-  team_sync();
+  team_sync_lds();
   PH(19)
   if (legs) {
     const int r = m.leg_root, ds = m.links[r].dof_start;
@@ -1130,7 +1158,7 @@
         if (dk) { st3(dk->cd_vel, lk[d], cvel_vel); st3(dk->cd_ang, lk[d], cvel_ang); }
       }
     }
-    team_sync();
+    team_sync_lds();
   }
   for (int lev = 0; lev < (legs ? 0 : m.n_levels); ++lev) {
     for (int k = m.level_start[lev] + tl; k < m.level_start[lev + 1]; k += T) {
@@ -1178,7 +1206,7 @@
       if (!dk) { e.cd_vel()[i_l] = cvel_vel; e.cd_ang()[i_l] = cvel_ang; }
       if (dk) { st3(dk->cd_vel, i_l, cvel_vel); st3(dk->cd_ang, i_l, cvel_ang); }
     }
-    team_sync();
+    team_sync_lds();
   }
   PH(55)
 }
@@ -1204,19 +1232,19 @@
       for (int j_ = 0; j_ < L.q_end - qs; ++j_) s->qpos_next[qs + j_] = s->qpos[qs + j_] + s->vel_next[ds + j_] * m.substep_dt;
     }
   }
-  team_sync();
+  team_sync_lds();
   bool bad = false;
   for (int d = tl; d < ND; d += T) bad |= isnan_(s->vel_next[d]);
   for (int q = tl; q < NQ; q += T) bad |= isnan_(s->qpos_next[q]);
   if (bad) s->valid = 0;
-  team_sync();
+  team_sync_lds();
   if (s->valid) {
     for (int d = tl; d < ND; d += T) { float v = s->vel_next[d]; s->vel[d] = v; gstore(e, FO(vel), d, v); }
     for (int q = tl; q < NQ; q += T) { float v = s->qpos_next[q]; s->qpos[q] = v; gstore(e, FO(qpos), q, v); }
   } else if (tl == 0) {
     atomicOr(&e.err()[0], GO2SIM_ERR_INVALID_ACC_NAN);
   }
-  team_sync();
+  team_sync_lds();
 }
 
 template <int T>
@@ -1225,6 +1253,7 @@
   wg_dma_to_lds<(int)sizeof(ModelS)>(ms_raw, mp);
   const int tl = threadIdx.x % T, slot = threadIdx.x / T;
   const ModelView m(&ms, mp);
+  asm volatile("" : "+v"(b));
   E e(P, b < P.B ? b : P.B - 1);
   KinData* s = &lds[slot];
   PH_BEGIN
@@ -1237,11 +1266,12 @@
   team_for<ND, T>(tl, [&](int d) { s->vel_next[d] = s->vel[d] + s->vel_next[d] * m.substep_dt; });
   if (tl == 0) s->valid = 1;
   tk_stage_links<T>(e, s, tl);
+  const LinkShift ls = tk_load_shift<T>(e, tl);
   team_sync();
   if (b >= P.B) return;
   tk_integrate<T>(m, e, s, tl);
   PH(40)
-  tk_kinematics<T>(m, e, s, tl, false);
+  tk_kinematics<T>(m, e, s, tl, false, nullptr, &ls);
   PH(41)
 }
 template <int T>
@@ -1275,6 +1305,11 @@
 }
 
 template <int T, class MT>
+DEV void tk_dynamics_out(const MT& m, const E& e, const DynData* s, int tl) {
+  for (int i_d = tl; i_d < ND; i_d += T) { float a = s->out[i_d]; astore(e, AO(acc_smooth), i_d, a); astore(e, AO(acc), i_d, a); }
+  team_for<NTRI, T>(tl, [&](int idx) { int i, j; tri_index(m, idx, i, j); astore(e, AO(mass_mat), idx, s->M[i * ND + j]); });
+}
+template <int T, class MT>
 DEV void tk_dynamics(const MT& m, const E& e, DynData* s, int tl, bool env_valid) {
   PH_BEGIN
   const bool legs = (T == 32 || T == 64) && m.leg_form;
@@ -1297,7 +1332,7 @@
       for (int l = 0; l < LEG_K; ++l) a = a + x[l][0];
       *at(r) = a;
     }
-    team_sync();
+    team_sync_lds();
   }
   for (int lev = (legs ? -1 : m.n_levels - 2); lev >= 0; --lev) {
     int n_par = m.level_start[lev + 1] - m.level_start[lev];
@@ -1312,7 +1347,7 @@
       }
       *dst = a;
     }
-    team_sync();
+    team_sync_lds();
   }
   PH(21)
   for (int i_d = tl; i_d < ND; i_d += T) {
@@ -1321,7 +1356,7 @@
     inertial_mul(ld3(s->crb_pos, i_l), ld9(s->crb_I, i_l), s->crb_mass[i_l], ld3(s->cdof_vel, i_d), ld3(s->cdof_ang, i_d), oa, ov);
     st3(s->f_ang, i_d, oa); st3(s->f_vel, i_d, ov);
   }
-  team_sync();
+  team_sync_lds();
   for (int idx = tl; idx < ND * (ND + 1) / 2; idx += T) {
     int i_d, j_d;
     tri_index(m, idx, i_d, j_d);
@@ -1335,7 +1370,7 @@
     s->M[i_d * ND + j_d] = v; s->M[j_d * ND + i_d] = v;
     s->L[i_d * ND + j_d] = v;
   }
-  team_sync();
+  team_sync_lds();
   PH(22)
 #if GO2SIM_FAST_ORDER
   const bool arrow = ARROW_SHAPE && (T == 32 || T == 64) && m.arrow_mode != 0;
@@ -1363,7 +1398,7 @@
 #pragma unroll
           for (int k = 0; k <= i_d; ++k) s->L[i_d * ND + k] = Lr[k];
         }
-        team_sync();
+        team_sync_lds();
       }
       float ri[ND];
 #pragma unroll
@@ -1376,14 +1411,14 @@
 #pragma unroll
       for (int k = 0; k < i_d; ++k) { const float nv = Lr[k] - a * ri[k]; Lr[k] = act ? nv : Lr[k]; }
     }
-    team_sync();
+    team_sync_lds();
     if (tl < ND) {
 #pragma unroll
       for (int k = 0; k < ND; ++k) if (k < row) s->L[row * ND + k] = Lr[k] * dinv_own;
       s->L[row * ND + row] = 1.0f;
       s->Dinv[row] = dinv_own;
     }
-    team_sync();
+    team_sync_lds();
   } else {
 #pragma unroll
     for (int i_d_ = 0; i_d_ < ND; ++i_d_) {
@@ -1395,10 +1430,10 @@
         float a = s->L[i_d * ND + j_d] * D_inv;
         s->L[j_d * ND + k_d] -= a * s->L[i_d * ND + k_d];
       }
-      team_sync();
+      team_sync_lds();
       for (int j_d = tl; j_d < i_d; j_d += T) s->L[i_d * ND + j_d] = s->L[i_d * ND + j_d] * D_inv;
       if (tl == 0) { s->Dinv[i_d] = D_inv; s->L[i_d * ND + i_d] = 1.0f; }
-      team_sync();
+      team_sync_lds();
     }
   }
   PH(23)
@@ -1447,7 +1482,7 @@
       if (m.links[i_l].parent != -1 || i_l == r) continue;
       st3(s->cdd_vel, i_l, -m.gravity * (1.0f - 0.0f)); st3(s->cdd_ang, i_l, v3(0, 0, 0));
     }
-    team_sync();
+    team_sync_lds();
   }
   for (int lev = 0; lev < (legs ? 0 : m.n_levels); ++lev) {
     for (int k = m.level_start[lev] + tl; k < m.level_start[lev + 1]; k += T) {
@@ -1465,7 +1500,7 @@
       }
       st3(s->cdd_vel, i_l, cv); st3(s->cdd_ang, i_l, ca);
     }
-    team_sync();
+    team_sync_lds();
   }
   for (int i_l = tl; i_l < NL; i_l += T) {
     V3 f1_ang, f1_vel, f2_ang, f2_vel, f3_ang, f3_vel;
@@ -1478,7 +1513,7 @@
     st3(s->cfrc_vel, i_l, f1_vel + f3_vel + ext_vel + v3(0, 0, 0));
     st3(s->cfrc_ang, i_l, f1_ang + f3_ang + ext_ang + v3(0, 0, 0));
   }
-  team_sync();
+  team_sync_lds();
   if (legs) {
     for (int c = tl; c < 6; c += T) {
       auto at = [&](int i_l) -> float* { return (c < 3) ? &s->cfrc_vel[3 * i_l + c] : &s->cfrc_ang[3 * i_l + c - 3]; };
@@ -1498,7 +1533,7 @@
       for (int l = 0; l < LEG_K; ++l) a = a + x[l][0];
       *at(r) = a;
     }
-    team_sync();
+    team_sync_lds();
   }
   for (int lev = (legs ? -1 : m.n_levels - 2); lev >= 0; --lev) {
     int n_par = m.level_start[lev + 1] - m.level_start[lev];
@@ -1512,7 +1547,7 @@
       }
       *dst = a;
     }
-    team_sync();
+    team_sync_lds();
   }
   for (int i_d = tl; i_d < ND; i_d += T) {
     int i_l = m.dof_link[i_d];
@@ -1521,7 +1556,7 @@
     s->force[i_d] = f;
     if (env_valid) { astore(e, AO(force), i_d, f); astore(e, AO(qf_smooth), i_d, f); }
   }
-  team_sync();
+  team_sync_lds();
   PH(24)
   bool solved = false;
 #if GO2SIM_FAST_ORDER
@@ -1564,9 +1599,7 @@
       for (int i_d = 0; i_d < ND; ++i_d) s->out[i_d] = y[i_d];
     }
   }
-  team_sync();
-  if (env_valid) for (int i_d = tl; i_d < ND; i_d += T) { float a = s->out[i_d]; astore(e, AO(acc_smooth), i_d, a); astore(e, AO(acc), i_d, a); }
-  if (env_valid) for (int idx = tl; idx < NTRI; idx += T) { int i, j; tri_index(m, idx, i, j); astore(e, AO(mass_mat), idx, s->M[i * ND + j]); }
+  team_sync_lds();
   PH(25)
 }
 
@@ -1596,8 +1629,8 @@
 };
 static_assert((BROAD_OVERLAY<16> && BROAD_OVERLAY<32> && BROAD_OVERLAY<64>) || NG != 28 || ND != 18, "the Go2 shape keeps the dynamics kernels' LDS size");
 
-template <int T>
-DEV void tk_broadphase(const Model& m, const E& e, BroadData<T>* s, int tl) {
+template <int T, class TAIL>
+DEV void tk_broadphase(const Model& m, const E& e, BroadData<T>* s, int tl, const GeomPose<T>* gin, TAIL tail) {
   const float inf = dm_bits2f(0x7f800000u);
   PH_BEGIN
   const int nc_old = e.n_contacts()[0];
@@ -1618,7 +1651,8 @@
   for (int g = 0; g < NGR; ++g) {
     const int i_g = (g * T + tl < NG) ? g * T + tl : NG - 1;
     V3 lower = v3(inf, inf, inf), upper = v3(-inf, -inf, -inf);
-    V3 gp = e.g_pos()[i_g]; Q4 gq = e.g_quat()[i_g];
+    V3 gp; Q4 gq;
+    if (gin) { gp = gin->p[g]; gq = gin->q[g]; } else { gp = e.g_pos()[i_g]; gq = e.g_quat()[i_g]; }
 #pragma unroll
     for (int c = 0; c < 8; ++c) {
       V3 corner = transform_by_trans_quat(m.geoms[i_g].aabb[c], gp, gq);
@@ -1626,14 +1660,15 @@
     }
     lower_[g] = lower; upper_[g] = upper;
   }
-  team_sync();
+  tail();
+  team_sync_lds();
 #pragma unroll
   for (int g = 0; g < NGR; ++g) {
     const int i_g = (g * T + tl < NG) ? g * T + tl : NG - 1;
     *(float4*)&s->amin[4 * i_g] = make_float4(lower_[g].x, lower_[g].y, lower_[g].z, 0.0f);
     *(float4*)&s->amax[4 * i_g] = make_float4(upper_[g].x, upper_[g].y, upper_[g].z, 0.0f);
   }
-  team_sync();
+  team_sync_lds();
   PH(30)
   int r[NK]; float sorted_v[NK]; int sorted_sg[NK];
   unsigned long long key[NK];
@@ -1649,7 +1684,7 @@
     s->skey[i] = key[q];
     sorted_v[q] = v; sorted_sg[q] = sg; r[q] = 0;
   }
-  team_sync();
+  team_sync_lds();
 #pragma unroll
   for (int j = 0; j < 2 * NG; ++j) {
     const unsigned long long kj = s->skey[j];
@@ -1659,7 +1694,7 @@
 #pragma unroll
   for (int q = 0; q < NK; ++q)
     if (tl + q * T < n2) s->rank_mm[2 * (sorted_sg[q] & 0xff) + ((sorted_sg[q] & 0x100) ? 1 : 0)] = r[q];
-  team_sync();
+  team_sync_lds();
   PH(31)
   int n_cand = 0;
   unsigned ncv_clear = 0u;
@@ -1690,14 +1725,14 @@
   }
   const bool overflow = n_cand > m.max_broad_pairs;
   n_cand = imn(n_cand, MAXB);
-  team_sync();
+  team_sync_lds();
   for (int c = tl; c < n_cand; c += T) {
     const int ck = s->cand_key[c]; int cr = 0;
     for (int j = 0; j < n_cand; ++j) cr += s->cand_key[j] < ck;
     s->pair_sorted[cr] = (unsigned)s->cand_pair[c];
   }
   const int n_broad = imn(n_cand, m.max_broad_pairs);
-  team_sync();
+  team_sync_lds();
   for (int c = tl; c < n_broad; c += T) e.broad()[c] = (int)s->pair_sorted[c];
 #pragma unroll
   for (int q = 0; q < NK; ++q) if (tl + q * T < n2) { e.sort_value()[r[q]] = sorted_v[q]; e.sort_ig()[r[q]] = sorted_sg[q]; }
@@ -1752,7 +1787,7 @@
   team_sync();
   PH(20)
   tk_dynamics<T>(m, e, s, tl, env_valid);
-  if (env_valid) tk_broadphase<T>(*gm, e, lds_b.at(slot, s), tl);
+  if (env_valid) tk_broadphase<T>(*gm, e, lds_b.at(slot, s), tl, nullptr, [&]() { tk_dynamics_out<T>(m, e, s, tl); });
 }
 
 
@@ -1763,7 +1798,9 @@
 DEV void integrate_fk_dynamics_body(const Pool& P, const ModelS* __restrict__ mp, const Model* __restrict__ gm, int b, DynData* lds_d, char* ms_raw,
                                     KinSeparate<KIN_OVERLAY, 64 / T>& lds_k, BroadSeparate<BROAD_OVERLAY<T>, T>& lds_b, bool pre, float pre_vel, float pre_acc) {
   const ModelS& ms = *(const ModelS*)ms_raw;
-  wg_dma_to_lds<(int)sizeof(ModelS)>(ms_raw, mp);
+  int lane = (int)threadIdx.x;
+  asm volatile("" : "+v"(lane));
+  wg_dma_to_lds<(int)sizeof(ModelS)>(ms_raw, mp, lane);
   const int tl = threadIdx.x % T, slot = threadIdx.x / T;
   const ModelView m(&ms, mp);
   asm volatile("" : "+v"(b));
@@ -1787,16 +1824,18 @@
   team_for<ND, T>(tl, [&](int i) { s->vel_next[i] = s->vel[i] + s->vel_next[i] * m.substep_dt; });
   if (tl == 0) s->valid = 1;
   tk_stage_links<T>(e, s, tl);
+  const LinkShift ls = tk_load_shift<T>(e, tl);
   team_sync();
   if (b >= P.B) return;
   tk_integrate<T>(m, e, s, tl);
   PH(40)
-  tk_kinematics<T>(m, e, s, tl, false, d);
+  GeomPose<T> gp;
+  tk_kinematics<T>(m, e, s, tl, false, d, &ls, &gp);
   team_for<ND, T>(tl, [&](int i) { d->vel[i] = s->vel[i]; });
-  team_sync();
+  team_sync_lds();
   PH(41)
   tk_dynamics<T>(m, e, d, tl, true);
-  tk_broadphase<T>(*gm, e, lds_b.at(slot, d), tl);
+  tk_broadphase<T>(*gm, e, lds_b.at(slot, d), tl, &gp, [&]() { tk_dynamics_out<T>(m, e, d, tl); });
 }
 template <int T>
 __global__ __launch_bounds__(64) void k_integrate_fk_dynamics_team(Pool P, const ModelS* __restrict__ mp, const Model* __restrict__ gm) {
@@ -4418,14 +4457,15 @@
   __shared__ BroadSeparate<BROAD_OVERLAY<T>, T> lds_b;
   const ModelS& ms = *(const ModelS*)ms_raw;
   wg_dma_to_lds<(int)sizeof(ModelS)>(ms_raw, mp);
+  const int blk = xcd_block();
   {
-    const int b0 = xcd_block() * EPW;
+    const int b0 = blk * EPW;
     wg_load<EPW, NL * 3>(P, b0, FO(cd_vel), [&](int ev, int k, float v) { lds[ev].cd_vel[k] = v; });
     wg_load<EPW, NL * 3>(P, b0, FO(cd_ang), [&](int ev, int k, float v) { lds[ev].cd_ang[k] = v; });
     wg_load<EPW, ND>(P, b0, FO(vel), [&](int ev, int k, float v) { lds[ev].vel[k] = v; });
   }
   const int tl = threadIdx.x % T, slot = threadIdx.x / T;
-  const int b = xcd_block() * EPW + slot;
+  const int b = blk * EPW + slot;
   const bool env_valid = b < P.B;
   const ModelView m(&ms, mp);
   E e(P, env_valid ? b : P.B - 1);
@@ -4437,16 +4477,20 @@
   const int eb = env_valid ? b : P.B - 1;
   auto hist = e.action_history();
   const int delay = e.delay_steps()[0];
-  const float a_in = (ia < na) ? actions_in[(size_t)eb * na + ia] : 0.0f;
+  const float a_ld = actions_in[(size_t)eb * na + (ia < na ? ia : 0)];
+  const float a_in = (ia < na) ? a_ld : 0.0f;
   const bool base_env = c.i[GO2SIM_IC_ENV_KIND] == 1;
   const int depth = c.i[GO2SIM_IC_MAX_DELAY] + 1;
-  const int read_idx = (((write_idx - delay) % depth) + depth) % depth;
-  const float h_ = base_env ? e.last_actions()[ia] : hist[read_idx][ia];
+  const float la_ = e.last_actions()[ia];
+  float ring_[GO2SIM_ACTION_RING_MAX];
+#pragma unroll
+  for (int k = 0; k < GO2SIM_ACTION_RING_MAX; ++k) ring_[k] = hist[k][ia];
   const float kpf = e.kp_factors()[im], kdf = e.kd_factors()[im], mst = e.motor_strength()[im], dp = e.e_dof_pos()[im], dv = e.e_dof_vel()[im];
   const bool manual_pd = c.i[GO2SIM_IC_MANUAL_PD] != 0, pls = c.i[GO2SIM_IC_PLS_ENABLE] != 0;
   const bool base_gains = manual_pd && !pls && c.i[GO2SIM_IC_HAS_KP_RANGE];
-  const float bkp = base_gains ? e.base_kp()[0] : c.f[GO2SIM_FC_KP], bkd = base_gains ? e.base_kd()[0] : c.f[GO2SIM_FC_KD];
-  const bool push_on = c.i[GO2SIM_IC_HAS_PUSH] && g.push_enable;
+  const float bkp_ = e.base_kp()[0], bkd_ = e.base_kd()[0];
+  const float bkp = base_gains ? bkp_ : c.f[GO2SIM_FC_KP], bkd = base_gains ? bkd_ : c.f[GO2SIM_FC_KD];
+  const bool push_on = (c.i[GO2SIM_IC_HAS_PUSH] != 0) & (g.push_enable != 0);
   const int pl = c.i[GO2SIM_IC_PUSH_LINK];
   auto psf = e.push_stored_force(); auto prem = e.push_remaining(); auto cpf = e.current_push_force(); auto ext = e.ext();
   float psf_[3] = {psf[0], psf[1], psf[2]}; int rem0 = prem[0];
@@ -4468,6 +4512,15 @@
   team_stage<ND, T>(tl, [&](int d) { return gload(e, FO(dof_pos), d); }, [&](int d, float v) { s->out[d] = v; });
   team_stage<NL * 6, T>(tl, [&](int k) { return gload(e, FO(ext), k); },
                         [&](int k, float v) { int i_l = k / 6, cc = k % 6; if (cc < 3) s->cfrc_ang[3 * i_l + cc] = v; else s->cfrc_vel[3 * i_l + cc - 3] = v; });
+  const int read_idx = (((write_idx - delay) % depth) + depth) % depth;
+  float h_ = base_env ? la_ : ring_[0];
+#pragma unroll
+  for (int k = 1; k < GO2SIM_ACTION_RING_MAX; ++k) h_ = (!base_env && read_idx == k) ? ring_[k] : h_;
+  issued(h_); issued(a_in); issued(kpf); issued(kdf); issued(mst); issued(dp); issued(dv); issued(bkp); issued(bkd);
+  issued(psf_[0]); issued(psf_[1]); issued(psf_[2]); issued(__int_as_float(rem0)); issued(pl_pos.x); issued(pl_pos.y); issued(pl_pos.z);
+  issued(pl_com.x); issued(pl_com.y); issued(pl_com.z);
+#pragma unroll
+  for (int k = 0; k < 6; ++k) issued(ext_[k]);
   team_sync();
   if (env_valid) {
     const float clip = c.f[GO2SIM_FC_CLIP_ACTIONS];
@@ -4538,10 +4591,10 @@
       }
     }
   }
-  team_sync();
+  team_sync_lds();
   PH(20)
   tk_dynamics<T>(m, e, s, tl, env_valid);
-  if (env_valid) tk_broadphase<T>(*gm, e, lds_b.at(slot, s), tl);
+  if (env_valid) tk_broadphase<T>(*gm, e, lds_b.at(slot, s), tl, nullptr, [&]() { tk_dynamics_out<T>(m, e, s, tl); });
 }
 
 struct RewCtx { float link_vel_xy[8], foot_z[4], foot_xy[8]; float vel_world[3]; int was_reset; };
```

New measurement: 18.05 million. -1.1%, worse.
